# microsoft/GenerativeImage2Text

Measured on AMD Instinct MI355X. Metric: captions/sec whole-node (GIT_BASE 224px bs=64/GPU greedy len=20), higher is better.
Workload: dtype f16; 1 GPU; GIT_BASE 224px bs=64/GPU greedy max_len=20 frames=1; global_batch=64, parallelism=dp1, decode_steps_per_caption=19, seq_len_returned=20, hip_graph=True, contexts_in_flight=4, layernorm_folded=True, library=libgitmi_f16.so, encoder_chains=2, schedule=mixed

## Files before the change

generativeimage2text_amd/csrc/engine.hip:

```cpp
#include "../../include/gitmi.h"
#include "engine_state.h"

#include <algorithm>
#include <cmath>
#include <cstdarg>
#include <cstdio>
#include <cstring>

using namespace gitmi;

#ifdef GITMI_EXPERIMENT
#include "../../include/gitmi_experiment.h"
#define GITMI_EXP_EXPORT extern "C"
#else
#define GITMI_EXP_EXPORT [[maybe_unused]] static
#endif

static thread_local char g_err[1024] = "";
int gitmi::fail(const char* fmt, ...) {
    va_list ap;
    va_start(ap, fmt);
    vsnprintf(g_err, sizeof(g_err), fmt, ap);
    va_end(ap);
    return 1;
// ... 22 lines not shown
static bool gemm_tall_tiles(const gitmi_engine* e, int N) {
    if (!e->pol.shared_device) return false;
    return e->pol.gemm_tall == 1 || (e->pol.gemm_tall == 2 && N >= 2048) || (e->pol.gemm_tall == 3 && N < 2048);
}

static double gemm_flops(int M, int N, int K) { return 2.0 * (double)M * (double)N * (double)K; }
static GemmArgs gemm_args(const void* A, int lda, const void* W, const float* bias, const void* res, int ldr, void* C, int ldc,
                          int M, int N, int K, int act) {
    GemmArgs g{};
    g.A = A; g.W = W; g.bias = bias; g.res = (const float*)res; g.C = C;
    g.M = M; g.N = N; g.K = K; g.lda = lda; g.ldc = ldc; g.ldr = ldr; g.act = act;
    return g;
}
static int gemm_run(gitmi_engine* e, hipStream_t s, GemmArgs g, bool in_f32, bool out_f32, int tag) {
    g.shared = gemm_tall_tiles(e, g.N) ? 1 : 0;
    SpanGuard sp(e, s, tag, gemm_flops(g.M, g.N, g.K));
    HIPCK(launch_gemm(g, in_f32, out_f32, s));
    return 0;
}
static int gemm(gitmi_engine* e, hipStream_t s, const void* A, int lda, const void* W, const float* bias,
                const float* res, int ldr, void* C, int ldc, bool out_f32, int M, int N, int K, int act, int tag) {
    return gemm_run(e, s, gemm_args(A, lda, W, bias, res, ldr, C, ldc, M, N, K, act), e->pol.f32, out_f32, tag);
}
static bool on_p8(const void* A, int lda, const void* W, const void* C, int ldc, int M, int N, int K, bool stream_out) {
    GemmArgs g = gemm_args(A, lda, W, nullptr, nullptr, 0, const_cast<void*>(C), ldc, M, N, K, 0);
    g.out_f16 = stream_out ? 1 : 0;
    return gemm_uses_p8(g, false, false);
}
struct Stream {
    void* x = nullptr; int M = 0, D = 0, tag = 0;
    bool fold = false;
    void* t = nullptr;
    float* xn = nullptr;
    float2* parts[2] = {nullptr, nullptr};
    const float2* part = nullptr; const float* gamma = nullptr; const float* beta = nullptr; float eps = 0.f;
};
static float2* stream_part_out(const Stream& st) { return st.part == st.parts[0] ? st.parts[1] : st.parts[0]; }
static void stream_written(Stream& st, const float2* part, const float* gamma, const float* beta, float eps) {
    st.part = part; st.gamma = gamma; st.beta = beta; st.eps = eps;
}
static int ln_gemm(gitmi_engine* e, hipStream_t s, const Stream& st, const Folded& f, const void* W, const float* bias, void* C,
                   int ldc, int col0, int N, int act) {
    const int D = st.D;
    const size_t woff = (size_t)col0 * D * e->pol.esz;
    C = (char*)C + (size_t)col0 * e->pol.esz;
    if (st.fold) {
        GemmArgs g = gemm_args(st.x, D, (const char*)f.w + woff, f.bias + col0, nullptr, 0, C, ldc, st.M, N, D, act);
        g.ln_part = st.part; g.ln_nparts = D / 256; g.ln_colsum = f.colsum + col0; g.ln_inv_d = 1.0f / (float)D; g.ln_eps = st.eps;
        return gemm_run(e, s, g, false, false, st.tag);
    }
    if (e->pol.stream_f16)
        HIPCK(launch_layernorm_s16(st.x, D, st.gamma, st.beta, st.eps, nullptr, st.t, D, false, st.xn, st.xn ? D : 0, st.M, D, 0, 0, 0, s));
    else
        HIPCK(launch_layernorm((const float*)st.x, D, st.gamma, st.beta, st.eps, nullptr, st.t, D, e->pol.f32, st.xn, st.xn ? D : 0, st.M,
                               D, 0, 0, 0, s));
    return gemm(e, s, st.t, D, (const char*)W + woff, bias + col0, nullptr, 0, C, ldc, e->pol.f32, st.M, N, D, act, st.tag);
}
static int gemm_to_stream(gitmi_engine* e, hipStream_t s, Stream& st, const void* A, int lda, const void* W, const float* bias, int K,
                          bool residual, const float* gamma, const float* beta, float eps) {
    const int D = st.D;
    float2* part = gamma ? stream_part_out(st) : nullptr;
    const void* res = !residual ? nullptr : st.xn && !st.fold ? st.xn : st.x;
    GemmArgs g = gemm_args(A, lda, W, bias, res, residual ? D : 0, st.x, D, st.M, D, K, 0);
    g.out_f16 = e->pol.stream_f16 ? 1 : 0;
    if (st.fold) {
        g.part_out = part;
        if (residual && st.xn) {
            g.res_part = st.part; g.res_nparts = D / 256; g.res_gamma = st.gamma; g.res_beta = st.beta;
            g.res_inv_d = 1.0f / (float)D; g.res_eps = st.eps;
        }
    }
    RCK(gemm_run(e, s, g, e->pol.f32, !e->pol.stream_f16, st.tag));
    stream_written(st, part, gamma, beta, eps);
    return 0;
}
static int attn_full_packed(gitmi_engine* e, const void* qkv, void* out, int width, int heads, int N, int batch, const int* ntok,
                            hipStream_t s) {
    AttnFullArgs a{};
    a.q = qkv;
    a.k = (const char*)qkv + (size_t)width * e->pol.esz;
    a.v = (const char*)qkv + (size_t)2 * width * e->pol.esz;
    a.out = out;
    a.ldq = a.ldk = a.ldv = 3 * width;
    a.ldo = width;
    a.N = N; a.H = heads; a.scale = 0.125f;
    a.ntok = ntok;
    HIPCK(launch_attn_full(a, batch, e->pol.f32, e->pol.attn_impl, s));
    return 0;
}
static int dec_layer_tail(gitmi_engine* e, hipStream_t s, const DecLayerW& L, const void* ctx, float* hf, void* ht, float* y, void* u,
                          int M) {
    const int d = e->cfg.dec_hidden, ffn = e->cfg.dec_ffn;
    RCK(gemm(e, s, ctx, d, L.wo, L.bo, hf, d, y, d, true, M, d, d, 0, TAG_GEMM_OTHER));
    HIPCK(launch_layernorm(y, d, L.lnag, L.lnab, 1e-12f, nullptr, ht, d, e->pol.f32, hf, d, M, d, 0, 0, 0, s));
    RCK(gemm(e, s, ht, d, L.w1, L.b1, nullptr, 0, u, ffn, e->pol.f32, M, ffn, d, 2, TAG_GEMM_OTHER));
    RCK(gemm(e, s, u, ffn, L.w2, L.b2, hf, d, y, d, true, M, d, ffn, 0, TAG_GEMM_OTHER));
    HIPCK(launch_layernorm(y, d, L.lnog, L.lnob, 1e-12f, nullptr, ht, d, e->pol.f32, hf, d, M, d, 0, 0, 0, s));
    return 0;
}

extern "C" int gitmi_abi_version(void) { return GITMI_ABI_VERSION; }
extern "C" int gitmi_operand_dtype(void) {
#ifdef GITMI_OPS_F16
    return GITMI_DTYPE_F16;
#else
    return GITMI_DTYPE_BF16;
#endif
}
extern "C" const char* gitmi_last_error(void) { return g_err; }

extern "C" int gitmi_create(const gitmi_config* cfg, int device, gitmi_engine** out) {
    if (!cfg || !out) return fail("gitmi_create: null argument");
    int ndev = 0;
    if (hipGetDeviceCount(&ndev) != hipSuccess || ndev <= 0)
        return fail("gitmi_create: no HIP device available (this engine has no CPU fallback)");
    if (device < 0 || device >= ndev) return fail("gitmi_create: device %d out of range (%d devices)", device, ndev);
    HIPCK(hipSetDevice(device));
    hipDeviceProp_t prop;
    HIPCK(hipGetDeviceProperties(&prop, device));
    if (strncmp(prop.gcnArchName, "gfx950", 6) != 0)
        return fail("gitmi_create: device %d is %s; this library is built for gfx950 (MI355X) only", device,
                    prop.gcnArchName);
    const gitmi_config& c = *cfg;
    if (c.vit_width % c.vit_heads || c.vit_width / c.vit_heads != 64) return fail("ViT head_dim must be 64");
    if (c.dec_hidden % c.dec_heads || c.dec_hidden / c.dec_heads != 64) return fail("decoder head_dim must be 64");
    if (c.image_size % c.patch) return fail("image_size must be a multiple of patch");
    if (c.max_image_pixels < 0 || c.max_image_tokens < 0) return fail("negative image capacity");
    if (c.vit_width > 1024 || c.dec_hidden > 1024) return fail("hidden sizes above 1024 are not supported");
    if (c.vit_width % 64 || c.dec_hidden % 64 || c.dec_ffn % 64) return fail("hidden sizes must be multiples of 64");
    if (c.max_batch < 1 || c.max_beams < 1 || c.max_beams > 8 || c.max_frames < 1 || c.max_text_len < 2)
        return fail("bad capacity (max_batch>=1, 1<=max_beams<=8, max_frames>=1, max_text_len>=2)");
    if (c.max_text_len > c.max_pos) return fail("max_text_len exceeds max_pos");
    if (c.precision != GITMI_PREC_BF16 && c.precision != GITMI_PREC_F32) return fail("bad precision");

    gitmi_engine* e = new gitmi_engine();
    e->cfg = c;
    e->device = device;
    e->pol.f32 = c.precision == GITMI_PREC_F32;
    e->pol.esz = e->pol.f32 ? 4 : 2;
    e->pol.attn_impl = e->pol.f32 ? 0 : 1;
    init_geometry(e);
    e->pol.stream_f16 = !e->pol.f32;
#ifdef GITMI_OPS_F16
    e->pol.ln_fold = !e->pol.f32 && c.vit_width % 256 == 0 && c.dec_hidden % 256 == 0;
#endif
#ifdef GITMI_EXPERIMENT
    if (const char* env = getenv("GITMI_ATTN_IMPL")) e->pol.attn_impl = e->pol.f32 ? 0 : atoi(env);
    if (const char* env = getenv("GITMI_GRAPH")) e->pol.use_graph = atoi(env) != 0;
    if (const char* env = getenv("GITMI_ATTN_DBG")) e->pol.attn_dbg = atoi(env);
    if (const char* env = getenv("GITMI_ATTN_PW")) e->pol.attn_pw = atoi(env);
    if (const char* env = getenv("GITMI_ATTN_NH")) e->pol.attn_nh = atoi(env);
    if (const char* env = getenv("GITMI_ATTN_STREAM")) e->pol.attn_stream = atoi(env);
    if (const char* env = getenv("GITMI_DECODE_SKIP")) e->pol.decode_skip = atoi(env);
    if (const char* env = getenv("GITMI_GEMM_TALL")) e->pol.gemm_tall = atoi(env);
    if (const char* env = getenv("GITMI_DGEMM_ROWS")) e->pol.dgemm_rows = atoi(env);
    if (const char* env = getenv("GITMI_DGEMM_STRIPS")) e->pol.dgemm_strips = atoi(env);
    if (const char* env = getenv("GITMI_DGEMM_NO_ROW_WALK")) e->pol.dgemm_no_row_walk = atoi(env);
    if (const char* env = getenv("GITMI_DGEMM_DBG")) e->pol.dgemm_dbg = atoi(env);
    if (const char* env = getenv("GITMI_VOCAB_WGS")) e->pol.vocab_wgs = atoi(env);
    if (const char* env = getenv("GITMI_SKINNY")) e->pol.skinny = atoi(env) != 0;
    if (const char* env = getenv("GITMI_STREAM_F16")) e->pol.stream_f16 = !e->pol.f32 && atoi(env) != 0;
    if (const char* env = getenv("GITMI_GEMM_IMPL")) set_gemm_impl(atoi(env));
#endif
    e->pol.ln_fold = e->pol.ln_fold && e->pol.stream_f16;
    e->pol.ln_fold_ready = e->pol.ln_fold;
    *out = e;
    return 0;
}

int CapturedGraph::capture(hipStream_t s, const std::function<int()>& fn) {
    reset();
    HIPCK(hipStreamBeginCapture(s, hipStreamCaptureModeThreadLocal));
    const int rc = fn();
    const hipError_t ce = hipStreamEndCapture(s, &graph);
    if (rc != 0 || ce != hipSuccess) reset();
    RCK(rc);
    HIPCK(ce);
    HIPCK(hipGraphInstantiate(&exec, graph, nullptr, nullptr, 0));
    return 0;
}
static void destroy_graph(gitmi_engine* e) {
    for (CapturedGraph* g : {&e->graph_full, &e->graph_decode, &e->graph_follow}) g->reset();
    e->full_slot.valid = e->follow_slot.valid = false;
}
static void drop_resident(gitmi_engine* e) { e->have_feats = e->have_prefill = false; }
static void set_resident(gitmi_engine* e, int B, int F_eff, int stride = 0) {
    e->cur_B = B; e->cur_F = F_eff; e->cur_Nimg = stride > 0 ? stride : F_eff * e->N;
    e->have_feats = true; e->have_prefill = false;
    e->keyed = e->ragged; e->has_context = false;
    e->res_desc.clear();
}
static void set_context(gitmi_engine* e) { e->keyed = e->has_context = true; }
static const int* key_counts(const gitmi_engine* e) { return e->keyed ? e->rg_ntok : nullptr; }
static void set_prefilled(gitmi_engine* e) { e->have_prefill = true; }
static int settle_residency(gitmi_engine* e, const Request& rq, int rc) {
    if (rc != 0 && rq.frames) drop_resident(e);
    return rc;
}

extern "C" void gitmi_destroy(gitmi_engine* e) {
    if (!e) return;
    hipSetDevice(e->device);
    hipDeviceSynchronize();
    if (e->enc_after) {
        auto& w = e->enc_after->enc_watchers;
        w.erase(std::remove(w.begin(), w.end(), e), w.end());
    }
    for (gitmi_engine* w : e->enc_watchers) w->enc_after = nullptr;
    destroy_graph(e);
    if (e->own_stream) hipStreamDestroy(e->own_stream);
    if (e->fence_in) hipEventDestroy(e->fence_in);
    if (e->fence_out) hipEventDestroy(e->fence_out);
    for (auto ev : e->gev)
        if (ev) hipEventDestroy(ev);
    if (e->enc_done) hipEventDestroy(e->enc_done);
    for (auto ev : e->event_pool) hipEventDestroy(ev);
    for (void* p : e->allocs) hipFree(p);
    for (void* p : e->sc_allocs) hipFree(p);
    hipFree(e->at_out); hipFree(e->at_stats); hipFree(e->ctx_tab); hipFree(e->mem_tab); hipFree(e->feat_tab); hipFree(e->ban_words);
    if (e->ban_stage) hipHostFree(e->ban_stage);
    if (e->ban_staged) hipEventDestroy(e->ban_staged);
    if (e->trie_off) hipFree(e->trie_off);
    if (e->trie_tok) hipFree(e->trie_tok);
    if (e->trie_child) hipFree(e->trie_child);
    delete e;
}

extern "C" int gitmi_set_image_shape(gitmi_engine* e, int H, int W, void* stream) {
    if (!e) return fail("null engine");
    if (!e->finalized) return fail("weights not finalized");
    const gitmi_config& c = e->cfg;
    if (H == 0 && W == 0) {
        if (!e->ragged) {
            e->ragged = true;
            e->H = e->W = e->gh = e->gw = 0;
            e->N = e->Nmax;
            drop_resident(e);
        }
        return 0;
    }
    if (H < c.patch || W < c.patch) return fail("image %dx%d is smaller than one %d-pixel patch", H, W, c.patch);
    const int gh = H / c.patch, gw = W / c.patch;
    if ((size_t)H * W > e->max_pixels)
        return fail("image %dx%d exceeds the max_image_pixels capacity (%zu)", H, W, e->max_pixels);
    if (gh * gw + 1 > e->Nmax)
        return fail("a %dx%d token grid exceeds the max_image_tokens capacity (%d)", gh, gw, e->Nmax);
    if (H == e->H && W == e->W && !e->ragged) return 0;
    e->ragged = false;
    HIPCK(hipSetDevice(e->device));
    if (gh == e->g_nat && gw == e->g_nat) {
        e->pos_cur = e->w.pos;
    } else {
        HIPCK(launch_pos_bicubic(e->w.pos, e->pos_var, e->g_nat, gh, gw, c.vit_width, (hipStream_t)stream));
        e->pos_cur = e->pos_var;
    }
    e->H = H; e->W = W; e->gh = gh; e->gw = gw; e->N = gh * gw + 1;
    drop_resident(e);
    return 0;
}

static Stream vit_stream(gitmi_engine* e, int M) {
    const int D = e->cfg.vit_width;
    const VitLayerW& L = e->w.vit[0];
    Stream st;
    st.x = e->v_x; st.M = M; st.D = D; st.tag = TAG_GEMM_VIT; st.t = e->v_h;
    st.fold = e->pol.ln_fold && on_p8(e->v_x, D, L.qkv_f.w, e->v_qkv, 3 * D, M, 3 * D, D, false) &&
              on_p8(e->v_x, D, L.ffn1_f.w, e->v_u, 4 * D, M, 4 * D, D, false) && on_p8(e->v_ctx, D, L.wo, e->v_x, D, M, D, D, true) &&
              on_p8(e->v_u, 4 * D, L.w2, e->v_x, D, M, D, 4 * D, true);
    if (st.fold) st.parts[0] = st.parts[1] = e->v_part;
    return st;
}
static Stream prefill_stream(gitmi_engine* e, int M) {
    const int d = e->cfg.dec_hidden, ffn = e->cfg.dec_ffn, D = e->cfg.vit_width;
    const DecLayerW& L = e->w.dec[0];
    Stream st;
    st.x = e->p_y; st.M = M; st.D = d; st.tag = TAG_GEMM_OTHER; st.t = e->p_ht; st.xn = e->p_hf;
    st.fold = e->pol.ln_fold && on_p8(e->feats, D, e->w.vp_w, e->p_y, d, M, d, D, true) &&
              on_p8(e->p_y, d, L.qkv_pf.w, e->img_kv[0], 3 * d, M, 3 * d, d, false) &&
              on_p8(e->p_y, d, L.qkv_pf.w, e->img_kv[0], 3 * d, M, 2 * d, d, false) &&
              (e->cfg.dec_layers < 2 || (on_p8(e->p_y, d, L.ffn1_pf.w, e->p_u, ffn, M, ffn, d, false) &&
                                         on_p8(e->p_ctx, d, L.wo, e->p_y, d, M, d, d, true) && on_p8(e->p_u, ffn, L.w2, e->p_y, d, M, d, ffn, true)));
    if (st.fold) { st.parts[0] = e->p_part[0]; st.parts[1] = e->p_part[1]; }
    return st;
}

static int encode_frames_impl(gitmi_engine* e, const float* const* frames, int F, int B, float* feats_out,
                              hipStream_t s, int stride = 0) {
    const gitmi_config& c = e->cfg;
    const int D = c.vit_width, N = e->N;
    const int F_eff = c.num_frames > 0 ? std::min(F, c.num_frames) : F;
    const int Nimg = stride > 0 ? stride : F_eff * N;
    drop_resident(e);
    SpanGuard phase(e, s, TAG_VIT, 0);
    const int BI = F_eff * B;
    const int M = BI * N;
    const int g2 = N - 1;
    const size_t slot = (size_t)3 * e->max_pixels;
    if (e->ragged)
        HIPCK(launch_im2col_ragged(e->frame_stage[0], slot, e->rg_meta, e->patches, e->pol.f32, B, N, c.patch, e->Kp, e->Kp_pad, s));
    else
    for (int fr = 0; fr < F_eff; ++fr)
        HIPCK(launch_im2col(frames[fr], (char*)e->patches + (size_t)fr * B * g2 * e->Kp_pad * e->pol.esz, e->pol.f32, B,
                            e->H, e->W, c.patch, e->Kp, e->Kp_pad, s));
    RCK(gemm(e, s, e->patches, e->Kp_pad, e->w.conv_w, nullptr, nullptr, 0, e->patch_out, D, true, BI * g2, D, e->Kp_pad, 0,
             TAG_GEMM_VIT));
    Stream x = vit_stream(e, M);
    float2* part = stream_part_out(x);
    if (e->ragged)
        HIPCK(launch_vit_assemble_ragged(e->patch_out, e->w.cls, e->w.pos, e->g_nat, e->rg_meta, e->w.lnpre_g, e->w.lnpre_b, 1e-5f, e->v_x,
                                         e->pol.stream_f16, BI, N, c.patch, D, part, s));
    else
    HIPCK(launch_vit_assemble_ln(e->patch_out, e->w.cls, e->pos_cur, e->w.lnpre_g, e->w.lnpre_b, 1e-5f, e->v_x, e->pol.stream_f16, BI, N, D,
                                 part, D / 256, s));
    stream_written(x, part, e->w.vit[0].ln1g, e->w.vit[0].ln1b, 1e-5f);
    for (int l = 0; l < c.vit_layers; ++l) {
        const VitLayerW& L = e->w.vit[l];
        const VitLayerW* Ln = l + 1 < c.vit_layers ? &e->w.vit[l + 1] : nullptr;
        RCK(ln_gemm(e, s, x, L.qkv_f, L.wqkv, L.bqkv, e->v_qkv, 3 * D, 0, 3 * D, 0));
        RCK(attn_full_packed(e, e->v_qkv, e->v_ctx, D, c.vit_heads, N, BI, e->ragged ? e->rg_ntok : nullptr, s));
        RCK(gemm_to_stream(e, s, x, e->v_ctx, D, L.wo, L.bo, D, true, L.ln2g, L.ln2b, 1e-5f));
        RCK(ln_gemm(e, s, x, L.ffn1_f, L.w1, L.b1, e->v_u, 4 * D, 0, 4 * D, 1));
        RCK(gemm_to_stream(e, s, x, e->v_u, 4 * D, L.w2, L.b2, 4 * D, true, Ln ? Ln->ln1g : nullptr, Ln ? Ln->ln1b : nullptr, 1e-5f));
    }
    for (int fr = 0; fr < F_eff; ++fr) {
        const float* te = (c.num_frames > 0 && e->pol.use_temb) ? e->w.temb[fr] : nullptr;
        if (e->pol.stream_f16) {
            const char* xs = (const char*)e->v_x + (size_t)fr * B * N * D * 2;
            HIPCK(launch_layernorm_s16(xs, D, e->w.lnpost_g, e->w.lnpost_b, 1e-5f, te, e->feats, D, false, nullptr, 0, B * N, D, N,
                                       Nimg, fr * N, s));
            if (feats_out)
                HIPCK(launch_layernorm_s16(xs, D, e->w.lnpost_g, e->w.lnpost_b, 1e-5f, te, feats_out, D, true, nullptr, 0, B * N, D,
// ... 153 lines not shown
        v.ban = ban;
        v.part_val = e->part_val; v.part_idx = e->part_idx; v.part_lse = e->part_lse;
        v.logits_out = logits_out; v.ld_logits = ldl;
        {
            SpanGuard sp(e, s, TAG_GEMM_OTHER, gemm_flops(R, c.vocab, d));
            if (!GITMI_SKIPPED(e, 8)) HIPCK(launch_vocab_topm(v, M, s));
        }
        cands->nparts = e->vocab_nparts; cands->slots = vocab_mtop_slots(M);
        if (sampling) RCK(sample_candidates(e, logits_out, ldl, R, cur_len, s, cands, nullptr));
        if (trie) RCK(trie_candidates(e, logits_out, ldl, cur_len, s, cands));
    } else {
        RCK(gemm(e, s, e->d_ht, d, e->w.out_w, e->w.out_b, nullptr, 0, e->logits, e->ldl, true, R, c.vocab, d, 0, TAG_GEMM_OTHER));
        cands->nparts = 1; cands->slots = row_topm_slots(M);
        if (sampling) RCK(sample_candidates(e, e->logits, e->ldl, R, cur_len, s, cands, &ban));
        else if (trie) RCK(trie_candidates(e, e->logits, e->ldl, cur_len, s, cands));
        else if (ids)
            HIPCK(launch_row_topm(e->logits, e->ldl, c.vocab, ids, ld_ids, cur_len, e->plen_dev, beams, suppress_kind,
                                  rep_penalty_of(e), M, R,
                                  e->part_val, e->part_idx, e->part_lse, s, &ban));
        if (logits_out && logits_out != e->logits) HIPCK(launch_copy_f32(e->logits, e->ldl, logits_out, ldl, R, c.vocab, s));
    }
    return 0;
}

static int check_ready(gitmi_engine* e) {
    if (!e) return fail("null engine");
    if (!e->finalized) return fail("weights not finalized (call gitmi_finalize_weights)");
    HIPCK(hipSetDevice(e->device));
    return 0;
}

static int ragged_prepare(gitmi_engine* e, const float* const* frames, int F, int B, hipStream_t s) {
    if (!e->ragged) return 0;
    if (F != 1 || !frames[0]) return fail("ragged input (gitmi_set_image_shape(e, 0, 0)): F must be 1, frames[0] the descriptor buffer");
    drop_resident(e);
    HIPCK(launch_ragged_stage(frames[0], e->frame_stage[0], (size_t)3 * e->max_pixels, e->rg_meta, e->rg_ntok, B, e->cfg.patch,
                              e->max_pixels, e->Nmax, s));
    return 0;
}

static int check_frames(const gitmi_engine* e, const char* who, const float* const* frames, int F, int B) {
    if (!frames || F < 1 || F > e->cfg.max_frames) return fail("%s: F=%d outside [1,%d]", who, F, e->cfg.max_frames);
    if (B < 1 || B > e->cfg.max_batch) return fail("%s: B=%d outside [1,%d]", who, B, e->cfg.max_batch);
    return 0;
}

static int check_resident(const gitmi_engine* e, const char* who, int B) {
    if (!e->have_feats)
        return fail("%s: frames == NULL is a follow-up call, but the engine holds no resident images (encode some with a call "
                    "that takes frames; a change of the image shape or mode, of the temporal embedding or of the LayerNorm "
                    "folding, and a failed call, drop them)", who);
    if (B != e->cur_B) return fail("%s: follow-up call with B=%d, but %d images are resident (B must equal that count)", who, B, e->cur_B);
    return 0;
}

extern "C" int gitmi_encode_frames(gitmi_engine* e, const float* const* frames, int F, int B, float* feats_out,
                                   void* stream) {
    RCK(check_ready(e));
    RCK(check_frames(e, "encode_frames", frames, F, B));
    RCK(ragged_prepare(e, frames, F, B, (hipStream_t)stream));
    return encode_frames_impl(e, frames, F, B, feats_out, (hipStream_t)stream);
}

static EmbedArgs embed_args(gitmi_engine* e, bool on) {
    EmbedArgs em{};
    if (!on) return em;
    em.words = e->w.words_f; em.positions = e->w.positions_f; em.gamma = e->w.emb_lng; em.beta = e->w.emb_lnb; em.eps = 1e-8f;
    em.h_f = e->d_hf; em.h_t = e->d_ht; em.D = e->cfg.dec_hidden; em.vocab = e->cfg.vocab;
    em.frag = (e->pol.skinny && !e->pol.f32) ? 1 : 0;
    return em;
}
static int embed_position(gitmi_engine* e, const int* ids, int ld_ids, int pos, int R, hipStream_t s) {
    const EmbedArgs em = embed_args(e, true);
    HIPCK(launch_embed_ln(ids, ld_ids, pos, em.words, em.positions, em.gamma, em.beta, em.eps, em.h_f, em.h_t, e->pol.f32, R, em.D,
                          em.vocab, em.frag != 0, s));
    return 0;
}

extern "C" int gitmi_prefill(gitmi_engine* e, void* stream) {
    RCK(check_ready(e));
    if (!e->have_feats) return fail("prefill: no encoded frames");
    return prefill_impl(e, (hipStream_t)stream);
}

extern "C" int gitmi_step_logits(gitmi_engine* e, const int64_t* tokens, int R, int t, float* logits_out, void* stream) {
    RCK(check_ready(e));
    if (!e->have_feats) return fail("step_logits: no encoded frames");
    hipStream_t s = (hipStream_t)stream;
    if (!e->have_prefill) RCK(prefill_impl(e, s));
    const int B = e->cur_B;
    if (R < B || R % B) return fail("step_logits: R=%d is not a multiple of the encoded batch %d", R, B);
    const int beams = R / B;
    if (beams > e->cfg.max_beams) return fail("step_logits: %d beams exceed max_beams", beams);
    if (t < 1 || t > e->cfg.max_text_len) return fail("step_logits: t=%d outside [1,%d]", t, e->cfg.max_text_len);
    const gitmi_config& c = e->cfg;
    const int T = c.max_text_len;
    e->img_identity = true;
    HIPCK(launch_load_ids((const long long*)tokens, R, t, e->ss.ids[0], e->ss.kv_src[0], T, s));
    StepCands cands{};
    for (int pos = 0; pos < t; ++pos) {
        SpanGuard step(e, s, TAG_STEP, 0);
        RCK(embed_position(e, e->ss.ids[0], T, pos, R, s));
        RCK(decode_layers_impl(e, e->ss.kv_src[0], T, pos, R, beams, s));
        if (pos == t - 1) RCK(decode_head_impl(e, nullptr, T, t, R, beams, 0, 1, logits_out, c.vocab, s, &cands));
    }
    return 0;
}

static int search_begin_impl(gitmi_engine* e, const Request& rq, int V, hipStream_t s) {
    const gitmi_config& c = e->cfg;
    const gitmi_search* sp = rq.sp;
    const int B = rq.Q, minP = rq.minP, maxP = rq.maxP;
    if (!sp) return fail("search: null config");
    if (sp->kind != GITMI_SEARCH_AUTOREGRESSIVE && sp->kind != GITMI_SEARCH_GENERATOR && sp->kind != GITMI_SEARCH_TRIE)
        return fail("search: bad kind");
    if (sp->kind == GITMI_SEARCH_TRIE) {
        if (sp->beam_size != 1) return fail("search: TrieAutoRegressiveBeamSearch asserts beam_size == 1 (trie_decoder.py:37)");
        if (!e->trie_off) return fail("search: no trie loaded (gitmi_set_trie)");
        if (sp->do_sample) return fail("search: the trie search has no sampling branch");
    }
    if (B < 1 || B > c.max_batch) return fail("search: B=%d outside [1,%d]", B, c.max_batch);
    if (sp->beam_size < 1 || sp->beam_size > c.max_beams) return fail("search: beam_size %d outside [1,%d]", sp->beam_size, c.max_beams);
    if (sp->per_node_beam_size < 1 && sp->kind != GITMI_SEARCH_TRIE) return fail("search: per_node_beam_size must be >= 1");
    if (sp->kind == GITMI_SEARCH_GENERATOR && sp->per_node_beam_size < 2)
        return fail("search: GeneratorWithBeamSearch requires per_node_beam_size > 1 (decoder.py:1078)");
    if (sp->beam_size * sp->per_node_beam_size > 16) return fail("search: beam_size*per_node_beam_size > 16 unsupported");
    if (sp->max_steps > c.max_text_len) return fail("search: max_steps %d exceeds max_text_len %d", sp->max_steps, c.max_text_len);
    if (minP < 1 || maxP > sp->max_steps) return fail("search: prefix lengths [%d,%d] outside [1,max_steps]", minP, maxP);
    if (sp->kind == GITMI_SEARCH_GENERATOR && !(sp->length_penalty > 0)) return fail("search: length_penalty must be > 0");
    if (sp->repetition_penalty != 0 && sp->repetition_penalty != 1.0) {
        if (sp->kind != GITMI_SEARCH_GENERATOR) return fail("search: repetition_penalty belongs to GeneratorWithBeamSearch (decoder.py:1064)");
        if (!(sp->repetition_penalty >= 1.0)) return fail("search: `repetition_penalty` should be >= 1 (decoder.py:1080)");
        if (sp->max_steps > 1024) return fail("search: repetition_penalty supports histories up to 1024 tokens");
    }
    if (sp->num_keep_best < 0 || sp->num_keep_best > SS_NHMAX) return fail("search: num_keep_best %d outside [1,%d]", sp->num_keep_best, SS_NHMAX);
    if (sp->num_keep_best > 1 && sp->kind != GITMI_SEARCH_GENERATOR)
        return fail("search: num_keep_best belongs to GeneratorWithBeamSearch.search (decoder.py:1087)");
    if (sp->do_sample) {
        if (sp->kind != GITMI_SEARCH_GENERATOR) return fail("search: do_sample is implemented for GeneratorWithBeamSearch (decoder.py:1146-1166) only");
        if (sp->temperature < 0) return fail("search: temperature must be > 0");
        if (V > 32768) return fail("search: sampling supports vocabularies up to 32768 tokens");
    }
    SearchState& st = e->ss;
    e->trie_search = sp->kind == GITMI_SEARCH_TRIE;
    st.B = B; st.k = sp->beam_size; st.pn = e->trie_search ? 1 : sp->per_node_beam_size;
    st.T = sp->max_steps;
    st.V = V; st.eos = c.eos; st.kind = e->trie_search ? GITMI_SEARCH_AUTOREGRESSIVE : sp->kind; st.length_penalty = sp->length_penalty;
    st.prefixed = rq.prefixed ? 1 : 0;
    st.nh = keep_best(*sp);
    st.sampled = sp->do_sample ? 1 : 0;
    e->sample = *sp;
    st.start = e->start_dev; st.ld_start = c.max_text_len; st.plen = e->plen_dev;
    e->ss_cur = 0; e->ss_len = minP;
    HIPCK(launch_search_init(st, s));
    if (e->trie_search) HIPCK(launch_fill_i32(e->trie_cursor, 0, B, s));
    return 0;
}

static int search_mtop(const SearchState& st) {
    if (st.sampled) return st.pn;
    return st.kind == GITMI_SEARCH_AUTOREGRESSIVE ? std::max(st.k, st.pn) : st.pn * st.k;
}
static int sample_candidates(gitmi_engine* e, const float* logits, int ldl, int R, int step, hipStream_t s, StepCands* cands,
                             const BanArgs* ban) {
    const gitmi_search& sp = e->sample;
    const float temp = sp.temperature > 0 ? (float)sp.temperature : 1.0f;
    HIPCK(launch_sample_rows(logits, ldl, e->ss.V, R, temp, sp.top_k, (float)sp.top_p, e->ss.pn, sp.seed, step,
                             e->part_val, e->part_idx, e->part_lse, nullptr, e->ss.ids[e->ss_cur], e->ss.T, step,
                             rep_penalty_of(e), row_topm_slots(e->ss.pn), s, ban, e->plen_dev, e->ss.k));
    cands->part_val = e->part_val; cands->part_idx = e->part_idx; cands->part_lse = e->part_lse;
    cands->nparts = 1; cands->slots = row_topm_slots(e->ss.pn);
    return 0;
}

static int trie_candidates(gitmi_engine* e, const float* logits, int ldl, int cur_len, hipStream_t s, StepCands* cands) {
    const SearchState& st = e->ss;
    TrieArgs tr{e->trie_off, e->trie_tok, e->trie_child, e->trie_cursor};
    HIPCK(launch_trie_select(logits, ldl, st.V, st.ids[e->ss_cur], st.T, cur_len, e->plen_dev, st.eos, tr, st.B, e->part_val,
                             e->part_idx, e->part_lse, s));
    cands->part_val = e->part_val; cands->part_idx = e->part_idx; cands->part_lse = e->part_lse;
    cands->nparts = 1; cands->slots = 1;
    return 0;
}

static int search_step_impl(gitmi_engine* e, const StepCands& cands, bool embed, hipStream_t s) {
    const SearchState& st = e->ss;
    const int cur_len = e->ss_len;
    if (cur_len >= st.T) return fail("search_advance: sequence already at max_steps");
    HIPCK(launch_search_step(st, e->ss_cur, cur_len, cands, embed_args(e, embed), e->pol.f32, s));
    e->ss_cur ^= 1;
    e->ss_len = cur_len + 1;
    return 0;
}

static int fill_uniform_sentences(gitmi_engine* e, int B, const long long* prefix_dev, int P, hipStream_t s) {
    HIPCK(launch_fill_start(e->start_dev, e->cfg.max_text_len, prefix_dev, 0, 1, e->cfg.sos, B, P, s));
    HIPCK(launch_fill_i32(e->plen_dev, P, B, s));
    e->img_identity = true;
    return 0;
}

extern "C" int gitmi_set_trie(gitmi_engine* e, int n_nodes, const int32_t* child_off, const int32_t* child_tok,
                              const int32_t* child_node) {
    RCK(check_ready(e));
    HIPCK(hipDeviceSynchronize());
    destroy_graph(e);
    int *n_off = nullptr, *n_tok = nullptr, *n_child = nullptr;
    if (n_nodes > 0) {
        if (!child_off || child_off[0] != 0) return fail("set_trie: child_off must start at 0");
        const int n_edges = child_off[n_nodes];
        for (int n = 0; n < n_nodes; ++n)
            if (child_off[n + 1] < child_off[n]) return fail("set_trie: child_off must be non-decreasing");
        if (n_edges > 0 && (!child_tok || !child_node)) return fail("set_trie: null edge arrays");
        for (int i = 0; i < n_edges; ++i)
            if (child_node[i] < 0 || child_node[i] >= n_nodes) return fail("set_trie: edge %d leads to node %d of %d", i, child_node[i], n_nodes);
        hipError_t err = hipMalloc((void**)&n_off, (size_t)(n_nodes + 1) * sizeof(int));
        if (err == hipSuccess) err = hipMalloc((void**)&n_tok, (size_t)std::max(n_edges, 1) * sizeof(int));
        if (err == hipSuccess) err = hipMalloc((void**)&n_child, (size_t)std::max(n_edges, 1) * sizeof(int));
        if (err == hipSuccess) err = hipMemcpy(n_off, child_off, (size_t)(n_nodes + 1) * sizeof(int), hipMemcpyHostToDevice);
        if (err == hipSuccess && n_edges > 0) err = hipMemcpy(n_tok, child_tok, (size_t)n_edges * sizeof(int), hipMemcpyHostToDevice);
        if (err == hipSuccess && n_edges > 0) err = hipMemcpy(n_child, child_node, (size_t)n_edges * sizeof(int), hipMemcpyHostToDevice);
        if (err != hipSuccess) {
            if (n_off) hipFree(n_off);
            if (n_tok) hipFree(n_tok);
            if (n_child) hipFree(n_child);
            return fail("set_trie: %s (the previous trie is kept)", hipGetErrorString(err));
        }
    }
    if (e->trie_off) { hipFree(e->trie_off); hipFree(e->trie_tok); hipFree(e->trie_child); }
    e->trie_off = n_off; e->trie_tok = n_tok; e->trie_child = n_child;
    return 0;
}

static int search_begin_host(gitmi_engine* e, const char* who, const gitmi_search* sp, int B, const int64_t* start_host, int ld,
                             const int32_t* plen_host, int vocab, void* stream) {
    RCK(check_ready(e));
    if (!start_host) return fail("%s: null start", who);
    if (B < 1 || B > e->cfg.max_batch || ld < 1 || ld > e->cfg.max_text_len) return fail("%s: bad B/P", who);
    if (vocab < 2) return fail("%s: bad vocab", who);
    if (sp && sp->kind == GITMI_SEARCH_SCORE) return fail("%s: GITMI_SEARCH_SCORE is not a search (gitmi_generate_prefixed scores sentences)", who);
    if (sp && sp->kind == GITMI_SEARCH_ATTEND) return fail("%s: GITMI_SEARCH_ATTEND is not a search (gitmi_generate_prefixed returns the attention maps of sentences)", who);
    if (sp && sp->kind == GITMI_SEARCH_CONTEXT) return fail("%s: GITMI_SEARCH_CONTEXT is not a search (gitmi_generate_prefixed puts context tokens into the decoder memory)", who);
    if (sp && sp->kind == GITMI_SEARCH_TREE_SCORE) return fail("%s: GITMI_SEARCH_TREE_SCORE is not a search (gitmi_generate_prefixed scores token trees)", who);
    if (sp && sp->kind == GITMI_SEARCH_KEEP) return fail("%s: GITMI_SEARCH_KEEP is not a search (gitmi_generate_prefixed keeps the memory of resident images)", who);
    if (sp && sp->kind == GITMI_SEARCH_RECALL) return fail("%s: GITMI_SEARCH_RECALL is not a search (gitmi_generate_prefixed recalls kept images)", who);
    if (sp && sp->kind == GITMI_SEARCH_FEATURES) return fail("%s: GITMI_SEARCH_FEATURES is not a search (gitmi_generate_prefixed installs given feature rows)", who);
    if (sp && sp->kind == GITMI_SEARCH_CONSTRAIN) return fail("%s: GITMI_SEARCH_CONSTRAIN is not a search (gitmi_generate_prefixed arms the constraints of the next search call)", who);
    if (e->ban_armed)
        return fail("%s: decoding constraints are armed for %d sentences (GITMI_SEARCH_CONSTRAIN): the seam's caller owns its logits and "
                    "applies its own -- disarm first (a GITMI_SEARCH_CONSTRAIN call with Q == 0)", who, e->ban_armed);
    e->ban_live = false;
    int minP = ld, maxP = ld;
    if (plen_host) {
        maxP = 1;
        for (int b = 0; b < B; ++b) {
            if (plen_host[b] < 1 || plen_host[b] > ld) return fail("%s: prefix length %d of sentence %d outside [1,%d]", who, plen_host[b], b, ld);
            minP = std::min(minP, (int)plen_host[b]); maxP = std::max(maxP, (int)plen_host[b]);
        }
    }
    hipStream_t s = (hipStream_t)stream;
    HIPCK(hipMemcpy2DAsync(e->start_dev, (size_t)e->cfg.max_text_len * sizeof(long long), start_host,
                           (size_t)ld * sizeof(long long), (size_t)ld * sizeof(long long), (size_t)B, hipMemcpyHostToDevice, s));
    if (plen_host) HIPCK(hipMemcpyAsync(e->plen_dev, plen_host, (size_t)B * sizeof(int), hipMemcpyHostToDevice, s));
    HIPCK(hipStreamSynchronize(s));
    if (!plen_host) HIPCK(launch_fill_i32(e->plen_dev, ld, B, s));
    e->img_identity = true;
    Request rq{};
    rq.Q = B; rq.minP = minP; rq.maxP = maxP; rq.prefixed = plen_host != nullptr; rq.sp = sp;
    return search_begin_impl(e, rq, vocab, s);
}

extern "C" int gitmi_search_begin(gitmi_engine* e, const gitmi_search* sp, int B, const int64_t* start_host, int P,
                                  int vocab, void* stream) {
    return search_begin_host(e, "search_begin", sp, B, start_host, P, nullptr, vocab, stream);
}

extern "C" int gitmi_search_rows(gitmi_engine* e, int64_t* tokens_out, int* R, int* t, void* stream) {
    RCK(check_ready(e));
    const SearchState& st = e->ss;
    if (R) *R = st.B * st.k;
    if (t) *t = e->ss_len;
    if (tokens_out) HIPCK(launch_search_rows(st, e->ss_cur, e->ss_len, (long long*)tokens_out, (hipStream_t)stream));
    return 0;
}

extern "C" int gitmi_search_advance(gitmi_engine* e, const float* logits, void* stream) {
    RCK(check_ready(e));
    if (!logits) return fail("search_advance: null logits");
    const SearchState& st = e->ss;
    hipStream_t s = (hipStream_t)stream;
    const int M = search_mtop(st), R = st.B * st.k;
    StepCands cands{e->part_val, e->part_idx, e->part_lse, 1, row_topm_slots(M)};
    if (st.sampled) RCK(sample_candidates(e, logits, st.V, R, e->ss_len, s, &cands, nullptr));
    else if (e->trie_search) RCK(trie_candidates(e, logits, st.V, e->ss_len, s, &cands));
    else
        HIPCK(launch_row_topm(logits, st.V, st.V, st.ids[e->ss_cur], st.T, e->ss_len, e->plen_dev, st.k,
                              st.kind == GITMI_SEARCH_AUTOREGRESSIVE ? 1 : 0, rep_penalty_of(e), M, R, e->part_val,
                              e->part_idx, e->part_lse, s));
    return search_step_impl(e, cands, false, s);
}

extern "C" int gitmi_search_done_count(gitmi_engine* e, int* done_out, void* stream) {
    RCK(check_ready(e));
    if (!done_out) return fail("search_done_count: null argument");
    int h = 0;
    HIPCK(hipMemcpyAsync(&h, e->ss.info, sizeof(int), hipMemcpyDeviceToHost, (hipStream_t)stream));
    HIPCK(hipStreamSynchronize((hipStream_t)stream));
    *done_out = h;
    return 0;
}

extern "C" int gitmi_search_finish(gitmi_engine* e, int64_t* tokens_out, float* logprob_out, int32_t* info_out,
                                   void* stream) {
    RCK(check_ready(e));
    const SearchState& st = e->ss;
    HIPCK(launch_search_finish(st, e->ss_cur, e->ss_len, (long long*)tokens_out, logprob_out, info_out, nullptr,
                               (hipStream_t)stream));
    return 0;
}

GITMI_EXP_EXPORT int gitmi_debug_search_begin_prefixed(gitmi_engine* e, const gitmi_search* sp, int B, const int64_t* start_host,
                                                       int ld, const int32_t* plen_host, int vocab, void* stream) {
    if (!plen_host) return fail("debug_search_begin_prefixed: null prefix lengths");
    return search_begin_host(e, "debug_search_begin_prefixed", sp, B, start_host, ld, plen_host, vocab, stream);
}
GITMI_EXP_EXPORT int gitmi_debug_search_advance_lists(gitmi_engine* e, const float* part_val, const int* part_idx,
                                                      const float* part_lse, int nparts, int slots, int embed, void* stream) {
    RCK(check_ready(e));
    if (!part_val || !part_idx || !part_lse) return fail("debug_search_advance_lists: null argument");
    const SearchState& st = e->ss;
    if (st.B < 1 || st.T < 1) return fail("debug_search_advance_lists: no search has begun");
    if (st.sampled || e->trie_search) return fail("debug_search_advance_lists: the sampling and trie searches select from whole logit rows");
    if (nparts < 1 || nparts > 256) return fail("debug_search_advance_lists: nparts=%d outside [1,256]", nparts);
    if (slots != 1 && slots != 2 && slots != 4 && slots != 8 && slots != 16)
        return fail("debug_search_advance_lists: slots=%d is not one of 1, 2, 4, 8, 16", slots);
    if (slots < search_mtop(st)) return fail("debug_search_advance_lists: slots=%d, but the step reads %d candidates per row", slots, search_mtop(st));
    const StepCands cands{part_val, part_idx, (const float2*)part_lse, nparts, slots};
    return search_step_impl(e, cands, embed != 0, (hipStream_t)stream);
}
GITMI_EXP_EXPORT int gitmi_debug_read_hidden(gitmi_engine* e, int R, float* hf_out, void* ht_out, int* ht_frag, int* ht_dtype,
                                             void* stream) {
    RCK(check_ready(e));
    const gitmi_config& c = e->cfg;
    if (R < 1 || R > c.max_batch * c.max_beams) return fail("debug_read_hidden: R=%d outside the capacity", R);
    if (!hf_out || !ht_out || !ht_frag || !ht_dtype) return fail("debug_read_hidden: null argument");
    hipStream_t s = (hipStream_t)stream;
    const size_t D = (size_t)c.dec_hidden, Rp = (size_t)(R + 15) / 16 * 16;
    HIPCK(hipMemcpyAsync(hf_out, e->d_hf, (size_t)R * D * sizeof(float), hipMemcpyDefault, s));
    HIPCK(hipMemcpyAsync(ht_out, e->d_ht, Rp * D * e->pol.esz, hipMemcpyDefault, s));
    HIPCK(hipStreamSynchronize(s));
    *ht_frag = (e->pol.skinny && !e->pol.f32) ? 1 : 0;
    *ht_dtype = e->pol.f32 ? GITMI_DTYPE_F32 : gitmi_operand_dtype();
    return 0;
}

static int generate_encode(gitmi_engine* e, const Request& rq, hipStream_t s) {
    RCK(encode_frames_impl(e, rq.frames, rq.F, rq.B, nullptr, s));
    return prefill_impl(e, s);
}
static int images_ready(gitmi_engine* e, const Request& rq, hipStream_t s) {
    if (rq.frames) return generate_encode(e, rq, s);
    return e->have_prefill ? 0 : prefill_impl(e, s);
}

static int generate_decode(gitmi_engine* e, const Request& rq, hipStream_t s, bool allow_poll) {
    const gitmi_config& c = e->cfg;
    const gitmi_search* sp = rq.sp;
    RCK(search_begin_impl(e, rq, c.vocab, s));
    const int Q = rq.Q, minP = rq.minP, maxP = rq.maxP, T = sp->max_steps, k = sp->beam_size, R = Q * k;
    const SearchState& st = e->ss;
    const int M = search_mtop(st);
    const int suppress = sp->kind != GITMI_SEARCH_GENERATOR ? 1 : 0;
    {
        SpanGuard phase(e, s, TAG_DECODE, 0);
        RCK(embed_position(e, st.ids[0], T, 0, R, s));
        e->ss_len = 1;
        StepCands cands{e->part_val, e->part_idx, e->part_lse, 1, 1};
        while (e->ss_len < T) {
            const int cur_len = e->ss_len;
            SpanGuard step(e, s, TAG_STEP, 0);
            RCK(decode_layers_impl(e, st.kv_src[e->ss_cur], T, cur_len - 1, R, k, s));
            if (cur_len >= minP)
                RCK(decode_head_impl(e, st.ids[e->ss_cur], T, cur_len, R, k, suppress, M, nullptr, 0, s, &cands));
            RCK(search_step_impl(e, cands, true, s));
            if (allow_poll && e->ss_len > maxP && (e->ss_len - maxP) % 8 == 0 && e->ss_len < T) {
                int h[4];
                HIPCK(hipMemcpyAsync(h, st.info, sizeof(h), hipMemcpyDeviceToHost, s));
                HIPCK(hipStreamSynchronize(s));
                if (h[0] >= Q) break;
            }
        }
    }
    HIPCK(launch_search_finish(st, e->ss_cur, e->ss_len, rq.tokens, rq.logprob, rq.info, rq.sent, s));
    if (e->ragged)
        HIPCK(launch_ragged_report(e->rg_meta, e->img_identity ? nullptr : e->img_of_dev, Q, keep_best(*sp), rq.logprob, rq.info,
                                   nullptr, s));
    const double kv = (double)Q * c.dec_layers * 2.0 * ((double)e->cur_Nimg + k * 0.5 * (minP + T)) * c.dec_hidden * e->pol.esz;
    e->last_decode_step_bytes = e->w.dec_weight_bytes + kv;
    return 0;
}

static int generate_body(gitmi_engine* e, const Request& rq, hipStream_t s, bool allow_poll) {
    SpanGuard total(e, s, 99, 0);
    RCK(images_ready(e, rq, s));
    return generate_decode(e, rq, s, allow_poll);
}

static GraphKey graph_key_of(const gitmi_engine* e, const Request& rq, int F_eff) {
    const gitmi_search& sp = *rq.sp;
    const bool resident = rq.frames == nullptr;
    return {rq.B, rq.Q, F_eff, rq.minP, sp.kind, sp.beam_size, sp.per_node_beam_size, sp.max_steps, e->H, e->W,
            rq.prefixed ? 1 : 0, e->img_identity ? 1 : 0, e->pol.use_temb ? 1 : 0, resident ? 1 : 0,
            resident ? e->cur_Nimg : 0, resident && e->keyed ? 1 : 0, sp.length_penalty,
            sp.do_sample, sp.top_k, keep_best(sp), sp.top_p, sp.temperature, sp.repetition_penalty, sp.seed, e->ban_live ? 1 : 0};
}

static int replay(gitmi_engine* e, const Request& rq, hipStream_t x, const CapturedGraph* enc, const CapturedGraph* dec) {
    const bool timed = e->profile_mode == 2;
    if (timed) {
        for (auto& ev : e->gev)
            if (!ev) HIPCK(hipEventCreate(&ev));
        HIPCK(hipEventRecord(e->gev[enc ? 0 : 1], x));
    } else if (enc && e->enc_after && e->enc_after->enc_done) {
        HIPCK(hipStreamWaitEvent(x, e->enc_after->enc_done, 0));
    }
    if (enc) {
        HIPCK(enc->launch(x));
        if (timed) HIPCK(hipEventRecord(e->gev[1], x));
        else if (e->enc_done && !e->enc_watchers.empty()) HIPCK(hipEventRecord(e->enc_done, x));
    }
    if (dec) HIPCK(dec->launch(x));
    if (!timed) return 0;
    HIPCK(hipEventRecord(e->gev[2], x));
    HIPCK(hipStreamSynchronize(x));
    float a = 0, b = 0;
    if (enc) HIPCK(hipEventElapsedTime(&a, e->gev[0], e->gev[1]));
    HIPCK(hipEventElapsedTime(&b, e->gev[1], e->gev[2]));
    e->split_encode_ms += a; e->split_decode_ms += b; e->split_calls += 1; e->split_steps += rq.sp->max_steps - 1;
    return 0;
}

static int generate_graphed(gitmi_engine* e, const Request& rq, hipStream_t s) {
    const gitmi_config& c = e->cfg;
    const bool resident = rq.frames == nullptr;
    hipStream_t x = s ? s : e->own_stream;
    if (x != s) {
        HIPCK(hipEventRecord(e->fence_in, s));
        HIPCK(hipStreamWaitEvent(x, e->fence_in, 0));
    }
    const size_t frame_bytes = (size_t)rq.B * 3 * e->H * e->W * sizeof(float);
    const int F_eff = resident ? e->cur_F : c.num_frames > 0 ? std::min(rq.F, c.num_frames) : rq.F;
    if (!e->ragged && !resident)
    for (int f = 0; f < F_eff; ++f)
        HIPCK(hipMemcpyAsync(e->frame_stage[f], rq.frames[f], frame_bytes, hipMemcpyDeviceToDevice, x));
    Request own = rq;
    if (!resident) { own.frames = e->frame_stage.data(); own.F = F_eff; }
    own.tokens = e->out_tokens; own.logprob = e->out_lp; own.info = e->out_info; own.sent = e->out_sent;
    const GraphKey key = graph_key_of(e, rq, F_eff);
    const CapturedGraph *enc = nullptr, *dec = nullptr;
    if (resident) {
        RCK(images_ready(e, rq, x));
        if (!e->follow_slot.valid || !(key == e->follow_slot.key)) {
            e->follow_slot.valid = false;
            RCK(e->graph_follow.capture(x, [&] { return generate_decode(e, own, x, false); }));
            e->follow_slot = {key, true};
        }
        dec = &e->graph_follow;
    } else {
        const bool split = e->profile_mode == 2 || e->enc_after != nullptr || !e->enc_watchers.empty();
        if (!e->full_slot.valid || !(key == e->full_slot.key) || split != e->graph_is_split) {
            e->full_slot.valid = false;
            e->graph_decode.reset();
            if (!split) {
                RCK(e->graph_full.capture(x, [&] { return generate_body(e, own, x, false); }));
            } else {
                RCK(e->graph_full.capture(x, [&] { return generate_encode(e, own, x); }));
                RCK(e->graph_decode.capture(x, [&] { return generate_decode(e, own, x, false); }));
            }
            e->full_slot = {key, true}; e->graph_is_split = split;
        } else {
            set_resident(e, rq.B, F_eff);
            set_prefilled(e);
        }
        enc = &e->graph_full;
        if (split) dec = &e->graph_decode;
    }
    RCK(replay(e, rq, x, enc, dec));
    const size_t nout = (size_t)rq.Q * (size_t)keep_best(*rq.sp);
    HIPCK(hipMemcpyAsync(rq.tokens, e->out_tokens, nout * rq.sp->max_steps * sizeof(long long), hipMemcpyDefault, x));
    HIPCK(hipMemcpyAsync(rq.logprob, e->out_lp, nout * sizeof(float), hipMemcpyDefault, x));
    HIPCK(hipMemcpyAsync(rq.info, e->out_info, 4 * sizeof(int), hipMemcpyDefault, x));
    if (rq.sent != e->out_sent) HIPCK(hipMemcpyAsync(rq.sent, e->out_sent, (size_t)rq.Q * 2 * sizeof(int), hipMemcpyDefault, x));
    if (x != s) {
        HIPCK(hipEventRecord(e->fence_out, x));
        HIPCK(hipStreamWaitEvent(s, e->fence_out, 0));
    }
    return 0;
}

static int generate_run(gitmi_engine* e, const Request& rq, hipStream_t s, bool constrained) {
    const bool long_budget = rq.sp->max_steps - rq.minP > 32;
    const bool graph = e->pol.use_graph && !e->profiling && !long_budget;
    if (constrained) e->ban_armed = 0;
    e->ban_live = constrained;
    const int rc = settle_residency(e, rq, graph ? generate_graphed(e, rq, s) : generate_body(e, rq, s, long_budget && !e->profiling));
    e->ban_live = false;
    return rc;
}

static int constrain_check(const gitmi_engine* e, const char* who, const gitmi_search* sp, int Q, bool* constrained);

extern "C" int gitmi_generate(gitmi_engine* e, const float* const* frames, int F, int B, const int64_t* prefix, int P,
                              const gitmi_search* sp, int64_t* tokens_out, float* logprob_out, int32_t* info_out,
                              void* stream) {
    RCK(check_ready(e));
    const gitmi_config& c = e->cfg;
    if (sp && sp->kind == GITMI_SEARCH_SCORE) return fail("generate: GITMI_SEARCH_SCORE scores given sentences: call gitmi_generate_prefixed");
    if (sp && sp->kind == GITMI_SEARCH_ATTEND) return fail("generate: GITMI_SEARCH_ATTEND maps given sentences: call gitmi_generate_prefixed");
    if (sp && sp->kind == GITMI_SEARCH_CONTEXT) return fail("generate: GITMI_SEARCH_CONTEXT takes context segments: call gitmi_generate_prefixed");
    if (sp && sp->kind == GITMI_SEARCH_TREE_SCORE) return fail("generate: GITMI_SEARCH_TREE_SCORE scores given token trees: call gitmi_generate_prefixed");
    if (sp && sp->kind == GITMI_SEARCH_KEEP) return fail("generate: GITMI_SEARCH_KEEP keeps the memory of resident images: call gitmi_generate_prefixed");
    if (sp && sp->kind == GITMI_SEARCH_RECALL) return fail("generate: GITMI_SEARCH_RECALL recalls kept images: call gitmi_generate_prefixed");
    if (sp && sp->kind == GITMI_SEARCH_FEATURES) return fail("generate: GITMI_SEARCH_FEATURES installs given feature rows: call gitmi_generate_prefixed");
    if (sp && sp->kind == GITMI_SEARCH_CONSTRAIN) return fail("generate: GITMI_SEARCH_CONSTRAIN arms decoding constraints: call gitmi_generate_prefixed");
    if (!frames) RCK(check_resident(e, "generate", B));
    if (!sp || !tokens_out || !logprob_out || !info_out) return fail("generate: null argument");
    if (frames) RCK(check_frames(e, "generate", frames, F, B));
    if (!prefix) P = 1;
    if (P < 1 || P > c.max_text_len) return fail("generate: prefix length %d outside [1,%d]", P, c.max_text_len);
    if (sp->max_steps < P || sp->max_steps > c.max_text_len) return fail("generate: max_steps %d outside [P,%d]", sp->max_steps, c.max_text_len);
    bool constrained = false;
    RCK(constrain_check(e, "generate", sp, B, &constrained));
    hipStream_t s = (hipStream_t)stream;
    if (frames) RCK(ragged_prepare(e, frames, F, B, s));
    RCK(fill_uniform_sentences(e, B, (const long long*)prefix, P, s));
    const Request rq{frames, F, B, B, P, P, false, sp, (long long*)tokens_out, logprob_out, info_out, e->out_sent};
    return generate_run(e, rq, s, constrained);
}

static int tree_max_depth(const gitmi_config& c) { return std::min((int)c.max_text_len, (int)c.max_pos); }
constexpr int TREE_MAX_ROWS = 65535 * 64;
static void score_free(gitmi_engine* e) {
    for (void* p : e->sc_allocs) hipFree(p);
    e->sc_allocs.clear();
    e->sc_rows = 0;
    e->tr_out_n = 0;
}
static int score_alloc(gitmi_engine* e, size_t rows_needed, size_t tree_out = 0) {
    size_t rows = (size_t)round_up((int)rows_needed, 128);
    if (e->sc_rows >= rows && e->tr_out_n >= tree_out) return 0;
    rows = std::max(rows, e->sc_rows);
    tree_out = std::max(tree_out, e->tr_out_n);
    score_free(e);
    const gitmi_config& c = e->cfg;
    const int d = c.dec_hidden;
    const size_t Qmax = (size_t)c.max_batch * c.max_beams;
    const size_t esz = e->pol.esz;
    auto alloc = [&](auto** p, size_t bytes) -> bool {
        void* q = nullptr;
        if (hipMalloc(&q, bytes) != hipSuccess) return false;
        e->sc_allocs.push_back(q);
        *reinterpret_cast<void**>(p) = q;
        return true;
    };
    const bool ok = alloc(&e->sc_hf, rows * d * 4) && alloc(&e->sc_y, rows * d * 4) && alloc(&e->sc_ht, rows * d * esz) &&
                    alloc(&e->sc_qkv, rows * 3 * d * esz) && alloc(&e->sc_ctx, rows * d * esz) &&
                    alloc(&e->sc_u, rows * c.dec_ffn * esz) &&
                    alloc(&e->sc_part, rows * (size_t)(e->pol.f32 ? 1 : score_head_tiles(c.vocab)) * sizeof(float4)) &&
                    alloc(&e->sc_zt, rows * 4) && alloc(&e->sc_tgt, rows * 4) && alloc(&e->sc_lens, Qmax * 4) &&
                    alloc(&e->sc_img, Qmax * 4) && alloc(&e->sc_bad, Qmax * 4) && alloc(&e->sc_info, 16) &&
                    alloc(&e->sc_out, Qmax * (size_t)c.max_text_len * sizeof(float2)) &&
                    (!tree_out || (alloc(&e->tr_nodes, rows * 4 * sizeof(int)) && alloc(&e->tr_out, tree_out * sizeof(float2))));
    if (!ok) {
        score_free(e);
        (void)hipGetLastError();
        return fail("score: out of device memory for the workspaces of %zu text rows", rows);
    }
    e->sc_rows = rows;
    e->tr_out_n = tree_out;
    return 0;
}

static int attend_alloc(gitmi_engine* e, size_t floats, size_t stat_rows) {
    if (e->at_floats < floats) {
        hipFree(e->at_out);
        e->at_out = nullptr; e->at_floats = 0;
        if (hipMalloc(&e->at_out, floats * sizeof(float)) != hipSuccess) {
            (void)hipGetLastError();
            return fail("attend: out of device memory for the %zu floats of the maps", floats);
        }
        e->at_floats = floats;
    }
    if (e->at_stat_rows < stat_rows) {
        hipFree(e->at_stats);
        e->at_stats = nullptr; e->at_stat_rows = 0;
        if (hipMalloc(&e->at_stats, stat_rows * sizeof(float2)) != hipSuccess) {
            (void)hipGetLastError();
            return fail("attend: out of device memory for the softmax statistics of %zu rows", stat_rows);
        }
        e->at_stat_rows = stat_rows;
    }
    return 0;
}
static int call_Nimg(const gitmi_engine* e, const float* const* frames, int F) {
    if (!frames) return e->cur_Nimg;
    return (e->cfg.num_frames > 0 ? std::min(F, (int)e->cfg.num_frames) : F) * e->N;
}

static int score_head_impl(gitmi_engine* e, int M, hipStream_t s, int* ntiles, const TreeNodes* tree = nullptr, int Lp = 0) {
    const gitmi_config& c = e->cfg;
    const int d = c.dec_hidden, V = c.vocab;
    *ntiles = 1;
    if (e->pol.f32) {
        const int chunk = round_up(c.max_batch * c.max_beams, 64);
        for (int r0 = 0; r0 < M; r0 += chunk) {
            const int rows = std::min(chunk, M - r0);
            RCK(gemm(e, s, (const float*)e->sc_ht + (size_t)r0 * d, d, e->w.out_w, e->w.out_b, nullptr, 0, e->logits, e->ldl, true, rows,
                     V, d, 0, TAG_GEMM_OTHER));
            HIPCK(launch_score_rowstats(e->logits, e->ldl, V, e->sc_tgt, r0, rows, e->sc_part, e->sc_zt, s));
            if (tree) HIPCK(launch_tree_gather_logits(e->logits, e->ldl, r0, rows, *tree, Lp, M, e->sc_zt, s));
        }
    } else {
        SpanGuard sp(e, s, TAG_GEMM_OTHER, gemm_flops(M, V, d));
        *ntiles = score_head_tiles(V);
        HIPCK(launch_score_head(e->sc_ht, d, e->w.out_w, e->w.out_b, e->sc_tgt, M, V, d, e->sc_part, e->sc_zt, s));
        if (tree) HIPCK(launch_tree_gather_dot(e->sc_ht, d, e->w.out_w, e->w.out_b, *tree, Lp, M, d, e->sc_zt, s));
    }
    return 0;
}
static int text_pass_impl(gitmi_engine* e, const Request& rq, const long long* tokens, int ld, hipStream_t s) {
    const gitmi_config& c = e->cfg;
    const int d = c.dec_hidden, V = c.vocab, Q = rq.Q, L = c.dec_layers;
    const bool attend = rq.sp->kind == GITMI_SEARCH_ATTEND, tree = rq.sp->kind == GITMI_SEARCH_TREE_SCORE;
    RCK(images_ready(e, rq, s));
    const int Lp = round_up(rq.maxP, 16), M = Q * Lp;
    const int Nk = e->cur_Nimg, Kc = Nk + ld;
    void* const out = attend ? (void*)e->at_out : tree ? (void*)e->tr_out : (void*)e->sc_out;
    const size_t out_bytes = attend ? (size_t)Q * ld * L * Kc * sizeof(float) : (size_t)Q * ld * sizeof(float2);
    auto zero_outputs = [&]() -> int {
        HIPCK(hipMemsetAsync(out, 0, out_bytes, s));
        HIPCK(hipMemsetAsync(e->sc_bad, 0, (size_t)Q * sizeof(int), s));
        return 0;
    };
    SpanGuard phase(e, s, TAG_DECODE, 0);
    if (attend || tree) RCK(zero_outputs());
    const size_t R = tree ? e->sc_rows : 0;
    const TreeNodes nodes = tree ? TreeNodes{e->tr_nodes, e->tr_nodes + R, e->tr_nodes + 2 * R, e->tr_nodes + 3 * R} : TreeNodes{};
    if (tree) HIPCK(launch_tree_structure(tokens, ld, Q, Lp, e->sc_lens, V, tree_max_depth(c), nodes, e->sc_bad, s));
    HIPCK(launch_score_embed_ln(tokens, ld, Q, Lp, e->w.words_f, e->w.positions_f, e->w.emb_lng, e->w.emb_lnb, 1e-8f, e->sc_hf, e->sc_ht,
                                e->pol.f32, d, V, c.max_pos, s, tree ? &nodes : nullptr));
    const int* ntok = key_counts(e);
    for (int l = 0; l < L; ++l) {
        const DecLayerW& W = e->w.dec[l];
        RCK(gemm(e, s, e->sc_ht, d, W.wqkv, W.bqkv, nullptr, 0, e->sc_qkv, 3 * d, e->pol.f32, M, 3 * d, d, 0, TAG_GEMM_OTHER));
        HIPCK(launch_score_attn(e->sc_qkv, e->img_kv[l], e->sc_img, e->sc_ctx, Q, c.dec_heads, d, Nk, Lp, 0.125f, e->pol.f32, s, ntok,
                                attend ? e->at_stats : nullptr, tree ? nodes.end : nullptr));
        if (attend)
            HIPCK(launch_score_attn_map(e->sc_qkv, e->img_kv[l], e->sc_img, ntok, e->at_stats, e->sc_lens, e->at_out + (size_t)l * Kc,
                                        (size_t)ld * L * Kc, (size_t)L * Kc, ld, Q, c.dec_heads, Nk, Lp, 0.125f, e->pol.f32, e->sc_bad, s));
        if (!attend || l + 1 < L) RCK(dec_layer_tail(e, s, W, e->sc_ctx, e->sc_hf, e->sc_ht, e->sc_y, e->sc_u, M));
    }
    if (int ntiles = 1; tree) {
        HIPCK(hipMemsetAsync(e->sc_tgt, 0xff, (size_t)M * sizeof(int), s));
        RCK(score_head_impl(e, M, s, &ntiles, &nodes, Lp));
        HIPCK(launch_tree_combine(e->sc_part, ntiles, e->sc_zt, nodes, M, Lp, ld, V, e->tr_out, e->sc_bad, s));
    } else if (!attend) {
        HIPCK(launch_score_targets(tokens, ld, Lp, e->sc_lens, V, M, e->sc_tgt, s));
        RCK(score_head_impl(e, M, s, &ntiles));
        RCK(zero_outputs());
        HIPCK(launch_score_combine(e->sc_part, ntiles, e->sc_zt, e->sc_tgt, M, Lp, ld, V, e->sc_out, e->sc_bad, s));
    }
    if (e->ragged) HIPCK(launch_ragged_report(e->rg_meta, e->sc_img, Q, 0, nullptr, nullptr, e->sc_bad, s));
    HIPCK(launch_score_info(e->sc_bad, Q, ld, e->sc_info, s, attend ? Kc : 0, attend ? L : 0));
    HIPCK(hipMemcpyAsync(rq.logprob, out, out_bytes, hipMemcpyDefault, s));
    HIPCK(hipMemcpyAsync(rq.info, e->sc_info, 4 * sizeof(int), hipMemcpyDefault, s));
    return 0;
}

struct SentenceSpan { int minP, maxP; bool ident; };
static int read_sentences(gitmi_engine* e, const char* who, const int32_t* plen, const int32_t* image_of, int ld, int B, int Q,
                          int Qmax, const char* cap, SentenceSpan* span) {
    if (Q < 1 || Q > Qmax) return fail("%s: Q=%d sentences outside [1,%d] (%s)", who, Q, Qmax, cap);
    if (!image_of && Q != B) return fail("%s: without image_of, Q must equal B", who);
    *span = {1 << 30, 0, true};
    e->plen_host.assign(plen, plen + Q);
    e->img_of_host.resize(Q);
    for (int q = 0; q < Q; ++q) {
        const int p = plen[q];
        if (p < 1 || p > ld) return fail("%s: length %d of sentence %d outside [1,%d]", who, p, q, ld);
// ... 603 lines not shown
```

generativeimage2text_amd/csrc/engine_state.h:

```cpp
#pragma once
#include "../../include/gitmi.h"
#include "abi_common.h"
#include "launchers.h"

#include <hip/hip_runtime.h>

#include <functional>
#include <map>
#include <string>
#include <tuple>
#include <vector>

static inline int round_up(int x, int m) { return (x + m - 1) / m * m; }
static inline int keep_best(const gitmi_search& sp) { return sp.num_keep_best > 1 ? sp.num_keep_best : 1; }

struct HostTensor {
    std::vector<float> data;
    std::vector<int64_t> shape;
    float amax = 0.f;
    size_t numel() const { size_t n = 1; for (auto s : shape) n *= (size_t)s; return n; }
};

struct Folded { void* w = nullptr; float* bias = nullptr; float* colsum = nullptr; };

struct VitLayerW {
    void *wqkv = nullptr, *wo = nullptr, *w1 = nullptr, *w2 = nullptr;
    float *bqkv = nullptr, *bo = nullptr, *b1 = nullptr, *b2 = nullptr;
    float *ln1g = nullptr, *ln1b = nullptr, *ln2g = nullptr, *ln2b = nullptr;
    Folded qkv_f;
    Folded ffn1_f;
};
struct DecLayerW {
    void *wqkv = nullptr, *wo = nullptr, *w1 = nullptr, *w2 = nullptr;
    float *bqkv = nullptr, *bo = nullptr, *b1 = nullptr, *b2 = nullptr;
    float *lnag = nullptr, *lnab = nullptr, *lnog = nullptr, *lnob = nullptr;
    Folded qkv_f;
    Folded ffn1_f;
    void *wo_p = nullptr, *w2_p = nullptr;
    Folded qkv_pf, ffn1_pf;
};

struct TimedSpan { hipEvent_t a, b; int tag; double flops; };
enum { TAG_VIT = 0, TAG_PREFILL = 1, TAG_DECODE = 2, TAG_GEMM_VIT = 10, TAG_GEMM_OTHER = 11, TAG_STEP = 20 };

struct GraphKey {
    int B, Q, F, P, kind, k, pn, T, H, W, prefixed, ident, temb, resident, Nimg, keyed; double lp;
    int smp, top_k, nh; double top_p, temp, rp; unsigned long long seed;
    int constrained;
    auto fields() const {
        return std::tie(B, Q, F, P, kind, k, pn, T, H, W, prefixed, ident, temb, resident, Nimg, keyed, lp, smp, top_k, nh, top_p, temp,
                        rp, seed, constrained);
    }
    bool operator==(const GraphKey& o) const { return fields() == o.fields(); }
};
struct GraphSlot { GraphKey key{}; bool valid = false; };

struct CapturedGraph {
    hipGraph_t graph = nullptr;
    hipGraphExec_t exec = nullptr;
    void reset() {
        if (exec) hipGraphExecDestroy(exec);
        if (graph) hipGraphDestroy(graph);
        exec = nullptr, graph = nullptr;
    }
    int capture(hipStream_t s, const std::function<int()>& fn);
    hipError_t launch(hipStream_t s) const { return hipGraphLaunch(exec, s); }
};

struct Request {
    const float* const* frames;
    int F, B, Q, minP, maxP;
    bool prefixed;
    const gitmi_search* sp;
    long long* tokens; float* logprob; int32_t* info;
    int32_t* sent;
};

struct ModelWeights {
    void* conv_w = nullptr;
    float *cls = nullptr, *pos = nullptr, *lnpre_g = nullptr, *lnpre_b = nullptr, *lnpost_g = nullptr, *lnpost_b = nullptr;
    std::vector<VitLayerW> vit;
    std::vector<float*> temb;
    void* vp_w = nullptr;
    float *vp_b = nullptr, *vp_lng = nullptr, *vp_lnb = nullptr;
    float *words_f = nullptr, *positions_f = nullptr, *emb_lng = nullptr, *emb_lnb = nullptr;
    std::vector<DecLayerW> dec;
    void* out_w = nullptr;
    float* out_b = nullptr;
    Folded out_f;
    double dec_weight_bytes = 0;
};

struct Policy {
    bool f32 = false;
    size_t esz = 2;
    int attn_impl = 1;
    bool stream_f16 = false;
    bool ln_fold = false;
    bool ln_fold_ready = false;
    bool skinny = true;
    bool use_graph = true;
    bool use_temb = true;
    bool shared_device = false;
    int attn_dbg = 0, dgemm_dbg = 0;
    int attn_pw = 0;
    int attn_nh = 0;
    int attn_stream = -1;
    int dgemm_no_row_walk = -1;
    int dgemm_strips = -1;
    int vocab_wgs = -1;
    int gemm_tall = 1;
    int dgemm_rows = 0;
    int decode_skip = 0;
};

struct gitmi_engine {
    gitmi_config cfg{};
    ModelWeights w;
    Policy pol;
    int device = 0;
    bool finalized = false;
    gitmi_engine* parent = nullptr;

    std::map<std::string, HostTensor> host_w;
    std::vector<void*> allocs;

    int N = 0, gh = 0, gw = 0, H = 0, W = 0, Kp = 0, Kp_pad = 0;
    int N_nat = 0, g_nat = 0, Nmax = 0;
    size_t max_pixels = 0;
    float* pos_var = nullptr;
    const float* pos_cur = nullptr;
    bool ragged = false;
    int4* rg_meta = nullptr;
    int* rg_ntok = nullptr;
    bool keyed = false;
    bool has_context = false;
    int* ctx_tab = nullptr;
    size_t ctx_tab_ints = 0;
    gitmi::MemoryEntry* mem_tab = nullptr;
    size_t mem_tab_n = 0;
    std::vector<int4> res_desc;
    gitmi::FeaturePiece* feat_tab = nullptr;
    unsigned int* ban_words = nullptr;
    int* ban_stage = nullptr;
    hipEvent_t ban_staged = nullptr;
    int ban_armed = 0;
    bool ban_live = false;

    void *patches = nullptr, *v_h = nullptr, *v_qkv = nullptr, *v_ctx = nullptr, *v_u = nullptr;
    float *patch_out = nullptr, *v_x = nullptr;
    void* feats = nullptr;
    float *p_y = nullptr, *p_hf = nullptr;
    void *p_ht = nullptr, *p_ctx = nullptr, *p_u = nullptr;
    std::vector<void*> img_kv;
    std::vector<void*> img_kh, img_vh;
    float *d_y = nullptr, *d_hf = nullptr, *logits = nullptr;
    void *d_ht = nullptr, *d_qkv = nullptr, *d_ctx = nullptr, *d_u = nullptr;
    std::vector<void*> txt_k, txt_v;
    int ldl = 0;
    float *xa_f = nullptr, *xo_f = nullptr;
    void *xa_b = nullptr, *xo_b = nullptr;
    float2 *stats_a = nullptr, *stats_o = nullptr;
    float* part_val = nullptr; int* part_idx = nullptr; float2* part_lse = nullptr;
    int vocab_cols = 128, vocab_nparts = 1;
    gitmi::SearchState ss{};
    int ss_cur = 0, ss_len = 0;
    long long* start_dev = nullptr;
    int *plen_dev = nullptr, *img_of_dev = nullptr;
    bool img_identity = true;
    int *trie_off = nullptr, *trie_tok = nullptr, *trie_child = nullptr, *trie_cursor = nullptr;
    bool trie_search = false;
    gitmi_search sample{};
    std::vector<int> plen_host, img_of_host;

    int cur_B = 0, cur_F = 0, cur_Nimg = 0;
    bool have_feats = false, have_prefill = false;

    int profile_mode = 0;
    bool profiling = false;
    float2 *v_part = nullptr, *p_part[2] = {nullptr, nullptr};
    hipEvent_t gev[3] = {nullptr, nullptr, nullptr};
    gitmi_engine* enc_after = nullptr;
    std::vector<gitmi_engine*> enc_watchers;
    hipEvent_t enc_done = nullptr;
    double split_encode_ms = 0, split_decode_ms = 0;
    int split_calls = 0, split_steps = 0;
    std::vector<TimedSpan> spans;
    std::vector<hipEvent_t> event_pool;
    size_t event_next = 0;
    double last_decode_step_bytes = 0;

    CapturedGraph graph_full, graph_decode, graph_follow;
    GraphSlot full_slot, follow_slot;
    bool graph_is_split = false;
    std::vector<float*> frame_stage;
    long long* out_tokens = nullptr;
    float* out_lp = nullptr;
    int* out_info = nullptr;
    int* out_sent = nullptr;
    hipStream_t own_stream = nullptr;
    hipEvent_t fence_in = nullptr, fence_out = nullptr;

    size_t sc_rows = 0;
    std::vector<void*> sc_allocs;
    float *sc_hf = nullptr, *sc_y = nullptr, *sc_zt = nullptr;
    void *sc_ht = nullptr, *sc_qkv = nullptr, *sc_ctx = nullptr, *sc_u = nullptr;
    float4* sc_part = nullptr;
    int *sc_tgt = nullptr, *sc_lens = nullptr, *sc_img = nullptr, *sc_bad = nullptr, *sc_info = nullptr;
    float2* sc_out = nullptr;
    size_t tr_out_n = 0;
    int* tr_nodes = nullptr;
    float2* tr_out = nullptr;
    size_t at_floats = 0, at_stat_rows = 0;
    float* at_out = nullptr;
    float2* at_stats = nullptr;
};

namespace gitmi {
void init_geometry(gitmi_engine* e);
}
```

generativeimage2text_amd/csrc/engine_weights.hip:

```cpp
#include "engine_state.h"

#include <algorithm>
#include <cmath>
#include <cstring>

using namespace gitmi;

static int dev_alloc(gitmi_engine* e, void** p, size_t bytes) {
    if (bytes == 0) bytes = 16;
    HIPCK(hipMalloc(p, bytes));
    e->allocs.push_back(*p);
    return 0;
}
template <typename T> static int dev_alloc_t(gitmi_engine* e, T** p, size_t count) {
    return dev_alloc(e, reinterpret_cast<void**>(p), count * sizeof(T));
}

static float half_to_float(uint16_t h) {
    const uint32_t sign = (uint32_t)(h & 0x8000) << 16;
    uint32_t exp = (h >> 10) & 0x1f, man = h & 0x3ff, out;
    if (exp == 0) {
        if (man == 0) out = sign;
        else {
            exp = 127 - 15 + 1;
// ... 33 lines not shown
    float amax = 0.f;
    for (size_t i = 0; i < n; ++i) {
        if (!std::isfinite(t.data[i])) return fail("gitmi_load_tensor: '%s' holds a non-finite value at element %zu", key, i);
        amax = std::max(amax, std::fabs(t.data[i]));
    }
    t.amax = amax;
    e->host_w[k] = std::move(t);
    return 0;
}

static int get_w(gitmi_engine* e, const std::string& key, std::initializer_list<int64_t> shape, const HostTensor** out) {
    auto it = e->host_w.find(key);
    if (it == e->host_w.end()) return fail("missing weight '%s'", key.c_str());
    size_t want = 1;
    for (auto s : shape) want *= (size_t)s;
    if (it->second.numel() != want) return fail("weight '%s' has %zu elements, expected %zu", key.c_str(), it->second.numel(), want);
    *out = &it->second;
    return 0;
}
static int up_f32(gitmi_engine* e, const std::string& key, std::initializer_list<int64_t> shape, float** dst) {
    const HostTensor* t;
    RCK(get_w(e, key, shape, &t));
    RCK(dev_alloc_t(e, dst, t->numel()));
    HIPCK(hipMemcpy(*dst, t->data.data(), t->numel() * 4, hipMemcpyHostToDevice));
    return 0;
}
static int operand_range_check(gitmi_engine* e, const char* what, float amax) {
#ifdef GITMI_OPS_F16
    if (!e->pol.f32 && amax > 65504.f)
        return fail("'%s': max |w| = %g is outside the fp16 operand range (65504): load this checkpoint with precision "
                    "\"bf16\" or \"f32\"", what, (double)amax);
#endif
    (void)e; (void)what; (void)amax;
    return 0;
}
static int up_mat(gitmi_engine* e, const std::string& key, int64_t rows, int K, int Kpad, void** dst) {
    const HostTensor* t;
    RCK(get_w(e, key, {rows, (int64_t)K}, &t));
    RCK(operand_range_check(e, key.c_str(), t->amax));
    RCK(dev_alloc(e, dst, (size_t)rows * Kpad * e->pol.esz));
    float* tmp = nullptr;
    HIPCK(hipMalloc((void**)&tmp, t->numel() * 4));
    hipError_t err = hipMemcpy(tmp, t->data.data(), t->numel() * 4, hipMemcpyHostToDevice);
    if (err == hipSuccess) err = launch_convert_pad(tmp, *dst, e->pol.f32, (size_t)rows, K, Kpad, 0);
    if (err == hipSuccess) err = hipDeviceSynchronize();
    hipFree(tmp);
    HIPCK(err);
    return 0;
}

void gitmi::init_geometry(gitmi_engine* e) {
    const gitmi_config& c = e->cfg;
    e->g_nat = e->gh = e->gw = c.image_size / c.patch;
    e->N_nat = e->N = e->g_nat * e->g_nat + 1;
    e->H = e->W = c.image_size;
    e->Nmax = std::max(e->N_nat, c.max_image_tokens);
    e->max_pixels = std::max((size_t)c.image_size * c.image_size, (size_t)c.max_image_pixels);
    e->Kp = 3 * c.patch * c.patch;
    e->Kp_pad = round_up(e->Kp, 64);
    e->pos_cur = e->w.pos;
}

static int alloc_workspaces(gitmi_engine* e) {
    const gitmi_config& c = e->cfg;
    const size_t esz = e->pol.esz;
    const int D = c.vit_width, d = c.dec_hidden;
    const size_t Mv = (size_t)c.max_batch * c.max_frames * e->Nmax;
    const size_t Mp = (size_t)c.max_batch * c.max_frames * e->Nmax;
    const size_t R = (size_t)round_up(c.max_batch * c.max_beams, 64);
    const int T = c.max_text_len;
    RCK(dev_alloc(e, &e->patches, (size_t)c.max_batch * c.max_frames * (e->Nmax - 1) * e->Kp_pad * esz));
    RCK(dev_alloc_t(e, &e->patch_out, (size_t)c.max_batch * c.max_frames * (e->Nmax - 1) * D));
    RCK(dev_alloc_t(e, &e->pos_var, (size_t)e->Nmax * D));
    RCK(dev_alloc_t(e, &e->v_x, Mv * D));
    RCK(dev_alloc(e, &e->v_h, Mv * D * esz));
    RCK(dev_alloc(e, &e->v_qkv, Mv * 3 * D * esz));
    RCK(dev_alloc(e, &e->v_ctx, Mv * D * esz));
    RCK(dev_alloc(e, &e->v_u, Mv * 4 * D * esz));
    RCK(dev_alloc(e, &e->feats, Mp * D * esz));
    if (e->pol.ln_fold_ready) {
        RCK(dev_alloc_t(e, &e->v_part, Mv * 4));
        RCK(dev_alloc_t(e, &e->p_part[0], Mp * 4));
        RCK(dev_alloc_t(e, &e->p_part[1], Mp * 4));
        HIPCK(hipMemset(e->v_part, 0, Mv * 4 * sizeof(float2)));
        HIPCK(hipMemset(e->p_part[0], 0, Mp * 4 * sizeof(float2)));
        HIPCK(hipMemset(e->p_part[1], 0, Mp * 4 * sizeof(float2)));
    }
    RCK(dev_alloc_t(e, &e->p_y, Mp * d));
    RCK(dev_alloc_t(e, &e->p_hf, Mp * d));
    RCK(dev_alloc(e, &e->p_ht, Mp * d * esz));
    RCK(dev_alloc(e, &e->p_ctx, Mp * d * esz));
    RCK(dev_alloc(e, &e->p_u, Mp * c.dec_ffn * esz));
    e->img_kv.resize(c.dec_layers);
    e->img_kh.resize(c.dec_layers);
    e->img_vh.resize(c.dec_layers);
    e->txt_k.resize(c.dec_layers);
    e->txt_v.resize(c.dec_layers);
    for (int l = 0; l < c.dec_layers; ++l) {
        RCK(dev_alloc(e, &e->img_kv[l], Mp * 3 * d * esz));
        const size_t Mkv = (size_t)c.max_batch * round_up(c.max_frames * e->Nmax, 32);
        RCK(dev_alloc(e, &e->img_kh[l], Mkv * d * esz));
        RCK(dev_alloc(e, &e->img_vh[l], Mkv * d * esz));
        RCK(dev_alloc(e, &e->txt_k[l], R * T * d * esz));
        RCK(dev_alloc(e, &e->txt_v[l], R * T * d * esz));
    }
    RCK(dev_alloc_t(e, &e->d_y, R * d));
    RCK(dev_alloc_t(e, &e->d_hf, R * d));
    RCK(dev_alloc(e, &e->d_ht, R * d * esz));
    RCK(dev_alloc(e, &e->d_qkv, R * 3 * d * esz));
    RCK(dev_alloc(e, &e->d_ctx, R * d * esz));
    RCK(dev_alloc(e, &e->d_u, R * c.dec_ffn * esz));
    RCK(dev_alloc_t(e, &e->xa_f, R * d));
    RCK(dev_alloc_t(e, &e->xo_f, R * d));
    RCK(dev_alloc(e, &e->xa_b, R * d * 2));
    RCK(dev_alloc(e, &e->xo_b, R * d * 2));
    RCK(dev_alloc_t(e, &e->stats_a, R * (size_t)(d / 16)));
    RCK(dev_alloc_t(e, &e->stats_o, R * (size_t)(d / 16)));
    e->ldl = round_up(c.vocab, 8);
    RCK(dev_alloc_t(e, &e->logits, R * e->ldl));
    e->vocab_cols = 128;
    e->vocab_nparts = (e->pol.skinny && !e->pol.f32) ? vocab_parts(c.vocab, e->vocab_cols) : 1;
    RCK(dev_alloc_t(e, &e->part_val, R * (size_t)e->vocab_nparts * 16));
    RCK(dev_alloc_t(e, &e->part_idx, R * (size_t)e->vocab_nparts * 16));
    RCK(dev_alloc_t(e, &e->part_lse, R * (size_t)e->vocab_nparts));
    SearchState& s = e->ss;
    for (int i = 0; i < 2; ++i) {
        RCK(dev_alloc_t(e, &s.ids[i], R * T));
        RCK(dev_alloc_t(e, &s.kv_src[i], R * T));
        RCK(dev_alloc_t(e, &s.score[i], R));
    }
    RCK(dev_alloc_t(e, &s.done, (size_t)c.max_batch));
    RCK(dev_alloc_t(e, &s.hyp_n, (size_t)c.max_batch));
    RCK(dev_alloc_t(e, &s.hyp_cnt, (size_t)c.max_batch));
    RCK(dev_alloc_t(e, &s.hyp_worst, (size_t)c.max_batch));
    RCK(dev_alloc_t(e, &s.hyp_score, (size_t)c.max_batch * SS_NHMAX));
    RCK(dev_alloc_t(e, &s.hyp_len, (size_t)c.max_batch * SS_NHMAX));
    RCK(dev_alloc_t(e, &s.hyp_seq, (size_t)c.max_batch * SS_NHMAX));
    RCK(dev_alloc_t(e, &s.hyp_tok, (size_t)c.max_batch * SS_NHMAX * T));
    RCK(dev_alloc_t(e, &s.stop, (size_t)c.max_batch));
    RCK(dev_alloc_t(e, &s.early, (size_t)c.max_batch));
    RCK(dev_alloc_t(e, &s.info, 4));
    RCK(dev_alloc_t(e, &s.len_norm, (size_t)T + 1));
    RCK(dev_alloc_t(e, &e->start_dev, (size_t)c.max_batch * T));
    RCK(dev_alloc_t(e, &e->plen_dev, (size_t)c.max_batch));
    RCK(dev_alloc_t(e, &e->img_of_dev, (size_t)c.max_batch));
    RCK(dev_alloc_t(e, &e->trie_cursor, (size_t)c.max_batch));
    RCK(dev_alloc_t(e, &e->out_tokens, (size_t)c.max_batch * SS_NHMAX * T));
    RCK(dev_alloc_t(e, &e->out_lp, (size_t)c.max_batch * SS_NHMAX));
    RCK(dev_alloc_t(e, &e->out_info, 4));
    RCK(dev_alloc_t(e, &e->out_sent, (size_t)c.max_batch * 2));
    HIPCK(hipStreamCreateWithFlags(&e->own_stream, hipStreamNonBlocking));
    HIPCK(hipEventCreateWithFlags(&e->fence_in, hipEventDisableTiming));
    HIPCK(hipEventCreateWithFlags(&e->fence_out, hipEventDisableTiming));
    e->frame_stage.resize(c.max_frames);
    for (int f = 0; f < c.max_frames; ++f)
        RCK(dev_alloc_t(e, &e->frame_stage[f], (size_t)c.max_batch * 3 * e->max_pixels));
    RCK(dev_alloc_t(e, &e->rg_meta, (size_t)c.max_batch));
    RCK(dev_alloc_t(e, &e->rg_ntok, (size_t)c.max_batch));
    return 0;
}

#ifdef GITMI_OPS_F16
static inline float bf16_round(float f) { return (float)(_Float16)f; }
#else
static inline float bf16_round(float f) {
    uint32_t u;
    memcpy(&u, &f, 4);
    if ((u & 0x7f800000u) == 0x7f800000u) return f;
    u += 0x7fffu + ((u >> 16) & 1u);
    u &= 0xffff0000u;
    memcpy(&f, &u, 4);
    return f;
}
#endif
static int fold_layernorm(gitmi_engine* e, const std::vector<float>& W, const std::vector<float>& bias,
                          const std::vector<float>& gamma, const std::vector<float>& beta, int64_t rows, int K, bool frag,
                          Folded* out) {
    std::vector<float> wf((size_t)rows * K), b2((size_t)rows), c2((size_t)rows);
    float amax = 0.f;
    for (int64_t n = 0; n < rows; ++n) {
        double sum = 0.0, cst = bias[n];
        const float* w = &W[(size_t)n * K];
        float* o = &wf[(size_t)n * K];
        for (int k = 0; k < K; ++k) {
            amax = std::max(amax, std::fabs(w[k] * gamma[k]));
            o[k] = bf16_round(w[k] * gamma[k]);
            sum += (double)o[k];
            cst += (double)beta[k] * (double)w[k];
        }
        c2[n] = (float)sum;
        b2[n] = (float)cst;
    }
    RCK(operand_range_check(e, "a matrix with the LayerNorm gain in front of it folded in (W . gamma)", amax));
    const int64_t rows_pad = (rows + 127) / 128 * 128;
    RCK(dev_alloc(e, &out->w, (size_t)rows_pad * K * 2));
    float* tmp = nullptr;
    void* tmp_b = nullptr;
    HIPCK(hipMalloc((void**)&tmp, wf.size() * 4));
    hipError_t err = hipSuccess;
    if (frag) err = hipMalloc(&tmp_b, wf.size() * 2);
    if (err == hipSuccess) err = hipMemcpy(tmp, wf.data(), wf.size() * 4, hipMemcpyHostToDevice);
    if (err == hipSuccess) err = launch_convert_pad(tmp, frag ? tmp_b : out->w, false, (size_t)rows, K, K, 0);
    if (err == hipSuccess && frag) err = launch_frag_pack(tmp_b, out->w, (int)rows, (int)rows_pad, K, 0);
    if (err == hipSuccess) err = hipDeviceSynchronize();
    hipFree(tmp);
    if (tmp_b) hipFree(tmp_b);
    HIPCK(err);
    b2.resize((size_t)rows_pad, 0.f);
    c2.resize((size_t)rows_pad, 0.f);
    RCK(dev_alloc_t(e, &out->bias, (size_t)rows_pad));
    RCK(dev_alloc_t(e, &out->colsum, (size_t)rows_pad));
    HIPCK(hipMemcpy(out->bias, b2.data(), (size_t)rows_pad * 4, hipMemcpyHostToDevice));
    HIPCK(hipMemcpy(out->colsum, c2.data(), (size_t)rows_pad * 4, hipMemcpyHostToDevice));
    return 0;
}
static int pack_frag(gitmi_engine* e, const void* src, int64_t rows, int K, void** dst) {
    const int64_t rows_pad = (rows + 15) / 16 * 16;
    RCK(dev_alloc(e, dst, (size_t)rows_pad * K * 2));
    HIPCK(launch_frag_pack(src, *dst, (int)rows, (int)rows_pad, K, 0));
    HIPCK(hipDeviceSynchronize());
    return 0;
}
static int fold_named(gitmi_engine* e, const std::string& ln, const std::string& dense, int64_t rows, int K, bool frag, Folded* out) {
    const HostTensor *g, *b, *w, *bi;
    RCK(get_w(e, ln + "weight", {K}, &g));
    RCK(get_w(e, ln + "bias", {K}, &b));
    RCK(get_w(e, dense + "weight", {rows, K}, &w));
    RCK(get_w(e, dense + "bias", {rows}, &bi));
    return fold_layernorm(e, w->data, bi->data, g->data, b->data, rows, K, frag, out);
}
static std::string vit_layer_key(int i) { return "image_encoder.transformer.resblocks." + std::to_string(i) + "."; }
static std::string dec_layer_key(int i) { return "textual.transformer.encoder.layer." + std::to_string(i) + "."; }
static int concat_qkv(gitmi_engine* e, const std::string& pre, int d) {
    HostTensor w, b;
    w.shape = {3 * d, d};
    b.shape = {3 * d};
    for (const char* name : {"query", "key", "value"}) {
        const HostTensor *tw, *tb;
        RCK(get_w(e, pre + "attention.self." + name + ".weight", {d, d}, &tw));
        RCK(operand_range_check(e, (pre + "attention.self." + name + ".weight").c_str(), tw->amax));
        RCK(get_w(e, pre + "attention.self." + name + ".bias", {d}, &tb));
        w.data.insert(w.data.end(), tw->data.begin(), tw->data.end());
        b.data.insert(b.data.end(), tb->data.begin(), tb->data.end());
        w.amax = std::max(w.amax, tw->amax);
    }
    e->host_w[pre + "attention.self.qkv.weight"] = std::move(w);
    e->host_w[pre + "attention.self.qkv.bias"] = std::move(b);
    return 0;
}

static int fold_decoder(gitmi_engine* e) {
    const gitmi_config& c = e->cfg;
    const int d = c.dec_hidden, f = c.dec_ffn;
    for (int i = 0; i < c.dec_layers; ++i) {
        const std::string pre = dec_layer_key(i);
        DecLayerW& L = e->w.dec[i];
        if (i > 0) {
            RCK(fold_named(e, dec_layer_key(i - 1) + "output.LayerNorm.", pre + "attention.self.qkv.", 3 * d, d, true, &L.qkv_f));
        } else {
            RCK(pack_frag(e, L.wqkv, 3 * d, d, &L.qkv_f.w));
            L.qkv_f.bias = L.bqkv;
        }
        RCK(pack_frag(e, L.wo, d, d, &L.wo_p));
        RCK(pack_frag(e, L.w2, d, f, &L.w2_p));
        RCK(fold_named(e, pre + "attention.output.LayerNorm.", pre + "intermediate.dense.", f, d, true, &L.ffn1_f));
    }
    return fold_named(e, dec_layer_key(c.dec_layers - 1) + "output.LayerNorm.", "textual.output.", c.vocab, d, true, &e->w.out_f);
}

static int fold_encoder_prefill(gitmi_engine* e) {
    const gitmi_config& c = e->cfg;
    const int D = c.vit_width, d = c.dec_hidden, f = c.dec_ffn;
    for (int i = 0; i < c.vit_layers; ++i) {
        const std::string pre = vit_layer_key(i);
        RCK(fold_named(e, pre + "ln_1.", pre + "attn.in_proj_", 3 * D, D, false, &e->w.vit[i].qkv_f));
        RCK(fold_named(e, pre + "ln_2.", pre + "mlp.c_fc.", 4 * D, D, false, &e->w.vit[i].ffn1_f));
    }
    for (int i = 0; i < c.dec_layers; ++i) {
        const std::string pre = dec_layer_key(i);
        DecLayerW& L = e->w.dec[i];
        const std::string ln = i == 0 ? "textual.visual_projection.1." : dec_layer_key(i - 1) + "output.LayerNorm.";
        RCK(fold_named(e, ln, pre + "attention.self.qkv.", 3 * d, d, false, &L.qkv_pf));
        if (i + 1 == c.dec_layers) break;
        RCK(fold_named(e, pre + "attention.output.LayerNorm.", pre + "intermediate.dense.", f, d, false, &L.ffn1_pf));
    }
    return 0;
}

extern "C" int gitmi_finalize_weights(gitmi_engine* e) {
    if (!e) return fail("null engine");
    if (e->finalized) return 0;
    HIPCK(hipSetDevice(e->device));
    const gitmi_config& c = e->cfg;
    const int D = c.vit_width, F4 = 4 * D, d = c.dec_hidden, f = c.dec_ffn, V = c.vocab;
    const int64_t p = c.patch;
    {
        const HostTensor* t;
        RCK(get_w(e, "image_encoder.conv1.weight", {D, 3, p, p}, &t));
        e->host_w["image_encoder.conv1.weight"].shape = {D, (int64_t)e->Kp};
        RCK(up_mat(e, "image_encoder.conv1.weight", D, e->Kp, e->Kp_pad, &e->w.conv_w));
    }
    RCK(up_f32(e, "image_encoder.class_embedding", {D}, &e->w.cls));
    RCK(up_f32(e, "image_encoder.positional_embedding", {e->N_nat, D}, &e->w.pos));
    e->pos_cur = e->w.pos;
    RCK(up_f32(e, "image_encoder.ln_pre.weight", {D}, &e->w.lnpre_g));
    RCK(up_f32(e, "image_encoder.ln_pre.bias", {D}, &e->w.lnpre_b));
    RCK(up_f32(e, "image_encoder.ln_post.weight", {D}, &e->w.lnpost_g));
    RCK(up_f32(e, "image_encoder.ln_post.bias", {D}, &e->w.lnpost_b));
    e->w.vit.resize(c.vit_layers);
// ... 81 lines not shown
```

generativeimage2text_amd/csrc/gitmi_common.h:

```cpp
#pragma once
#include <hip/hip_runtime.h>
#include <stdint.h>

typedef unsigned short bf16_t;
typedef __attribute__((ext_vector_type(8))) __bf16 bf16x8_t;
typedef __attribute__((ext_vector_type(4))) float f32x4_t;
typedef __attribute__((ext_vector_type(4))) unsigned int u32x4_t;

#define GITMI_WAVE 64

typedef _Float16 f16_t;
typedef __attribute__((ext_vector_type(2))) _Float16 f16x2_t;
typedef __attribute__((ext_vector_type(8))) _Float16 f16x8_t;
typedef __attribute__((ext_vector_type(2))) __bf16 bf16x2_t;
#ifdef GITMI_OPS_F16
#define GITMI_OPERAND_NAME "f16"
__device__ __forceinline__ float bf2f(bf16_t h) { return (float)__builtin_bit_cast(_Float16, h); }
__device__ __forceinline__ bf16_t f2bf(float f) {
    const _Float16 b = (_Float16)f;
    return __builtin_bit_cast(bf16_t, b);
}
__device__ __forceinline__ uint32_t pack2bf(float lo, float hi) {
    const f16x2_t v = {(_Float16)lo, (_Float16)hi};
    return __builtin_bit_cast(uint32_t, v);
}
__device__ __forceinline__ void unpack2op(uint32_t u, float& lo, float& hi) {
    const f16x2_t v = __builtin_bit_cast(f16x2_t, u);
    lo = (float)v[0];
    hi = (float)v[1];
}
__device__ __forceinline__ f32x4_t mfma16(bf16x8_t a, bf16x8_t b, f32x4_t c) {
    return __builtin_amdgcn_mfma_f32_16x16x32_f16(__builtin_bit_cast(f16x8_t, a), __builtin_bit_cast(f16x8_t, b), c, 0, 0, 0);
}
#else
#define GITMI_OPERAND_NAME "bf16"
__device__ __forceinline__ float bf2f(bf16_t h) { return __uint_as_float(((uint32_t)h) << 16); }
__device__ __forceinline__ bf16_t f2bf(float f) {
    const __bf16 b = (__bf16)f;
    return __builtin_bit_cast(bf16_t, b);
}
__device__ __forceinline__ uint32_t pack2bf(float lo, float hi) {
    const bf16x2_t v = {(__bf16)lo, (__bf16)hi};
    return __builtin_bit_cast(uint32_t, v);
}
__device__ __forceinline__ void unpack2op(uint32_t u, float& lo, float& hi) {
    lo = __uint_as_float(u << 16);
    hi = __uint_as_float(u & 0xffff0000u);
}
__device__ __forceinline__ f32x4_t mfma16(bf16x8_t a, bf16x8_t b, f32x4_t c) {
    return __builtin_amdgcn_mfma_f32_16x16x32_bf16(a, b, c, 0, 0, 0);
}
#endif

__device__ __forceinline__ uint32_t pack2h(float lo, float hi) {
    const f16x2_t v = {(_Float16)lo, (_Float16)hi};
    return __builtin_bit_cast(uint32_t, v);
}
__device__ __forceinline__ void unpack2h(uint32_t u, float& lo, float& hi) {
    const f16x2_t v = __builtin_bit_cast(f16x2_t, u);
    lo = (float)v[0];
    hi = (float)v[1];
}
__device__ __forceinline__ f32x4_t ld4s(const float* p) { return *reinterpret_cast<const f32x4_t*>(p); }
__device__ __forceinline__ f32x4_t ld4s(const f16_t* p) {
    const uint2 u = *reinterpret_cast<const uint2*>(p);
    float a, b, c, d;
    unpack2h(u.x, a, b);
    unpack2h(u.y, c, d);
    return f32x4_t{a, b, c, d};
}
__device__ __forceinline__ void st4s(float* p, f32x4_t v) { *reinterpret_cast<f32x4_t*>(p) = v; }
__device__ __forceinline__ void st4s(f16_t* p, f32x4_t v) {
    uint2 u;
    u.x = pack2h(v[0], v[1]);
    u.y = pack2h(v[2], v[3]);
    *reinterpret_cast<uint2*>(p) = u;
}

template <typename T> __device__ __forceinline__ float ld(const T* p);
template <> __device__ __forceinline__ float ld<float>(const float* p) { return *p; }
template <> __device__ __forceinline__ float ld<bf16_t>(const bf16_t* p) { return bf2f(*p); }
template <typename T> __device__ __forceinline__ void st(T* p, float v);
template <> __device__ __forceinline__ void st<float>(float* p, float v) { *p = v; }
template <> __device__ __forceinline__ void st<bf16_t>(bf16_t* p, float v) { *p = f2bf(v); }
template <> __device__ __forceinline__ float ld<f16_t>(const f16_t* p) { return (float)*p; }
template <> __device__ __forceinline__ void st<f16_t>(f16_t* p, float v) { *p = (f16_t)v; }

__device__ __forceinline__ void ld8(const bf16_t* p, float (&v)[8]) {
    u32x4_t r = *reinterpret_cast<const u32x4_t*>(p);
#pragma unroll
    for (int i = 0; i < 4; ++i) unpack2op(r[i], v[2 * i], v[2 * i + 1]);
}
__device__ __forceinline__ void ld8(const float* p, float (&v)[8]) {
    f32x4_t a = *reinterpret_cast<const f32x4_t*>(p);
    f32x4_t b = *reinterpret_cast<const f32x4_t*>(p + 4);
#pragma unroll
    for (int i = 0; i < 4; ++i) { v[i] = a[i]; v[4 + i] = b[i]; }
}
__device__ __forceinline__ void st8(bf16_t* p, const float (&v)[8]) {
    u32x4_t r;
#pragma unroll
    for (int i = 0; i < 4; ++i) r[i] = pack2bf(v[2 * i], v[2 * i + 1]);
    *reinterpret_cast<u32x4_t*>(p) = r;
}
__device__ __forceinline__ void st8(float* p, const float (&v)[8]) {
    f32x4_t a, b;
#pragma unroll
    for (int i = 0; i < 4; ++i) { a[i] = v[i]; b[i] = v[4 + i]; }
    *reinterpret_cast<f32x4_t*>(p) = a;
    *reinterpret_cast<f32x4_t*>(p + 4) = b;
}

__device__ __forceinline__ float wave_sum(float v) {
#pragma unroll
    for (int o = 32; o > 0; o >>= 1) v += __shfl_xor(v, o, 64);
    return v;
}
__device__ __forceinline__ float wave_max(float v) {
#pragma unroll
    for (int o = 32; o > 0; o >>= 1) v = fmaxf(v, __shfl_xor(v, o, 64));
    return v;
}

__device__ __host__ __forceinline__ size_t frag_offset(int row, int k, int ksteps) {
    return (((size_t)(row >> 4) * ksteps + (k >> 5)) * 64 + (size_t)(((k & 31) >> 3) * 16 + (row & 15))) * 8 + (k & 7);
}
__device__ __forceinline__ size_t frag_tile(int rt, int ks, int ksteps, int lane) {
    return (((size_t)rt * ksteps + ks) * 64 + lane) * 8;
}

__device__ __forceinline__ float rep_penalize(float x, float rp) { return x < 0.f ? x * rp : x / rp; }
constexpr int HIST_SLOTS = 2048;
__device__ __forceinline__ unsigned int hist_hash(int tok) { return ((unsigned int)tok * 2654435761u) >> 21; }
__device__ __forceinline__ void hist_insert(int* tbl, int tok) {
    unsigned int h = hist_hash(tok);
    for (;;) {
        const int old = atomicCAS(&tbl[h], -1, tok);
        if (old == -1 || old == tok) return;
        h = (h + 1) & (HIST_SLOTS - 1);
    }
}
__device__ __forceinline__ bool hist_contains(const int* tbl, int tok) {
    unsigned int h = hist_hash(tok);
    for (;;) {
        const int v = tbl[h];
        if (v == tok) return true;
        if (v == -1) return false;
        h = (h + 1) & (HIST_SLOTS - 1);
    }
}

#define GITMI_ACT_NONE 0
#define GITMI_ACT_QUICKGELU 1
#define GITMI_ACT_GELU_ERF 2

__device__ __forceinline__ float fast_exp(float x) { return __builtin_amdgcn_exp2f(x * 1.4426950408889634f); }
__device__ __forceinline__ float fast_rcp(float x) { return __builtin_amdgcn_rcpf(x); }

__device__ __forceinline__ float quick_gelu(float x) { return x * fast_rcp(1.0f + fast_exp(-1.702f * x)); }

__device__ __forceinline__ float gelu_erf(float x) {
    const float z = x * 0.70710678118654752440f;
    const float az = fabsf(z);
    const float t = fast_rcp(1.0f + 0.3275911f * az);
    float poly = 1.061405429f;
    poly = poly * t - 1.453152027f;
    poly = poly * t + 1.421413741f;
    poly = poly * t - 0.284496736f;
    poly = poly * t + 0.254829592f;
    poly *= t;
    const float e = 1.0f - poly * fast_exp(-az * az);
    return 0.5f * x * (1.0f + copysignf(e, z));
}

template <int ACT> __device__ __forceinline__ float apply_act_t(float x) {
    if constexpr (ACT == GITMI_ACT_QUICKGELU) return quick_gelu(x);
    else if constexpr (ACT == GITMI_ACT_GELU_ERF) return gelu_erf(x);
    else return x;
}
__device__ __forceinline__ float apply_act(float x, int act) {
    if (act == GITMI_ACT_QUICKGELU) return quick_gelu(x);
    if (act == GITMI_ACT_GELU_ERF) return gelu_erf(x);
    return x;
}
```

generativeimage2text_amd/csrc/kernels_norm.hip:

```cpp
#include "gitmi_common.h"
#include "launchers.h"

namespace gitmi {

struct RowMap {
    int n_in, n_out, off;
};
__device__ __forceinline__ size_t map_row(const RowMap& m, int row) {
    return (size_t)(row / m.n_in) * m.n_out + m.off + row % m.n_in;
}

constexpr int LN_MAXV = 16;

template <typename TOut, typename TS = float>
__global__ __launch_bounds__(256) void layernorm_kernel(const TS* __restrict__ x, int ldx,
                                                        const float* __restrict__ gamma,
                                                        const float* __restrict__ beta, float eps,
                                                        const float* __restrict__ add_after,
                                                        TOut* __restrict__ y_t, int ld_t,
                                                        TS* __restrict__ y_f, int ld_f, int rows, int D,
                                                        RowMap map) {
    const int lane = threadIdx.x & 63;
    const int row = blockIdx.x * 4 + (threadIdx.x >> 6);
    if (row >= rows) return;
// ... 287 lines not shown
__global__ void im2col_ragged_kernel(const float* __restrict__ stage, size_t slot, const int4* __restrict__ meta,
                                     TOut* __restrict__ out, int B, int Nmax, int p, int K, int Kpad) {
    const size_t total = (size_t)B * (Nmax - 1) * Kpad;
    for (size_t i = blockIdx.x * (size_t)blockDim.x + threadIdx.x; i < total; i += (size_t)gridDim.x * blockDim.x) {
        const int k = (int)(i % Kpad);
        const size_t prow = i / Kpad;
        const int t = (int)(prow % (Nmax - 1)), b = (int)(prow / (Nmax - 1));
        const int4 m = meta[b];
        const int gh = m.x / p, gw = m.y / p;
        float val = 0.f;
        if (k < K && t < gh * gw) {
            const int kx = k % p, ky = (k / p) % p, c = k / (p * p);
            const int gx = t % gw, gy = t / gw;
            val = stage[(size_t)b * slot + ((size_t)c * m.x + gy * p + ky) * m.y + gx * p + kx];
        }
        st<TOut>(out + i, val);
    }
}

template <typename TS>
__global__ __launch_bounds__(256) void vit_assemble_ragged_kernel(const float* __restrict__ patch_out,
                                                                  const float* __restrict__ cls,
                                                                  const float* __restrict__ pos, int g,
                                                                  const int4* __restrict__ meta,
                                                                  const float* __restrict__ gamma,
                                                                  const float* __restrict__ beta, float eps,
                                                                  TS* __restrict__ X, int B, int Nmax, int p, int D,
                                                                  float2* __restrict__ part) {
    const int lane = threadIdx.x & 63;
    const int row = blockIdx.x * 4 + (threadIdx.x >> 6);
    if (row >= B * Nmax) return;
    const int b = row / Nmax, n = row % Nmax;
    const int4 m = meta[b];
    if (n >= m.z) {
#pragma unroll
        for (int i = 0; i < LN_MAXV; ++i) {
            const int c = lane + 64 * i;
            if (c < D) st<TS>(X + (size_t)row * D + c, 0.f);
        }
        if (part && lane < 4) part[(size_t)row * 4 + lane] = float2{0.f, 0.f};
        return;
    }
    const int gh = m.x / p, gw = m.y / p;
    const float* src = n == 0 ? cls : patch_out + ((size_t)b * (Nmax - 1) + (n - 1)) * D;
    const bool native = n == 0 || (gh == g && gw == g);
    const float sy = (float)g / (float)gh, sx = (float)g / (float)gw;
    const int oy = native ? 0 : (n - 1) / gw, ox = native ? 0 : (n - 1) % gw;
    const float fy = ((float)oy + 0.5f) * sy - 0.5f, fx = ((float)ox + 0.5f) * sx - 0.5f;
    const float y0f = floorf(fy), x0f = floorf(fx);
    float wy[4], wx[4];
    cubic_taps(fy - y0f, wy);
    cubic_taps(fx - x0f, wx);
    const int y0 = (int)y0f, x0 = (int)x0f;
    float v[LN_MAXV];
    float s = 0.f;
#pragma unroll
    for (int i = 0; i < LN_MAXV; ++i) {
        const int c = lane + 64 * i;
        float pv = 0.f;
        if (c < D) {
            if (native) {
                pv = pos[(size_t)n * D + c];
            } else {
                float acc = 0.f;
#pragma unroll
                for (int a = 0; a < 4; ++a) {
                    int yy = y0 - 1 + a;
                    yy = yy < 0 ? 0 : (yy > g - 1 ? g - 1 : yy);
                    float rw = 0.f;
#pragma unroll
                    for (int bb = 0; bb < 4; ++bb) {
                        int xx = x0 - 1 + bb;
                        xx = xx < 0 ? 0 : (xx > g - 1 ? g - 1 : xx);
                        rw += wx[bb] * pos[((size_t)1 + (size_t)yy * g + xx) * D + c];
                    }
                    acc += wy[a] * rw;
                }
                pv = acc;
            }
        }
        v[i] = c < D ? src[c] + pv : 0.f;
        s += v[i];
    }
    const float mean = wave_sum(s) / (float)D;
    float q = 0.f;
#pragma unroll
    for (int i = 0; i < LN_MAXV; ++i) {
        const int c = lane + 64 * i;
        const float d = c < D ? v[i] - mean : 0.f;
        q += d * d;
    }
    const float rstd = rsqrtf(wave_sum(q) / (float)D + eps);
#pragma unroll
    for (int i = 0; i < LN_MAXV; ++i) {
        const int c = lane + 64 * i;
        if (c < D) st<TS>(X + (size_t)row * D + c, (v[i] - mean) * rstd * gamma[c] + beta[c]);
    }
    if (part) {
        float sx2 = 0.f, sq = 0.f;
#pragma unroll
        for (int i = 0; i < LN_MAXV; ++i) {
            const int c = lane + 64 * i;
            if (c < D) {
                const float o = (float)(TS)((v[i] - mean) * rstd * gamma[c] + beta[c]);
                sx2 += o;
                sq = fmaf(o, o, sq);
            }
        }
        sx2 = wave_sum(sx2);
        sq = wave_sum(sq);
        if (lane < 4) part[(size_t)row * 4 + lane] = lane == 0 ? float2{sx2, sq} : float2{0.f, 0.f};
    }
}

__global__ __launch_bounds__(256) void zero_pad_rows_kernel(char* __restrict__ x, size_t bytes, const int* __restrict__ ntok,
                                                            int B, int Nmax) {
    const int lane = threadIdx.x & 63;
    const int row = blockIdx.x * 4 + (threadIdx.x >> 6);
    if (row >= B * Nmax || row % Nmax < ntok[row / Nmax]) return;
    uint4* r = reinterpret_cast<uint4*>(x + (size_t)row * bytes);
    for (size_t i = lane; i < bytes / 16; i += 64) r[i] = make_uint4(0u, 0u, 0u, 0u);
}

__global__ __launch_bounds__(256) void ragged_report_kernel(const int4* __restrict__ meta, const int* __restrict__ image_of, int Q,
                                                            int nout_per, float* __restrict__ logprob, int* __restrict__ info,
                                                            int* __restrict__ bad) {
    __shared__ int s_n;
    if (threadIdx.x == 0) s_n = 0;
    __syncthreads();
    int n = 0;
    for (int q = threadIdx.x; q < Q; q += blockDim.x) {
        const int im = image_of ? image_of[q] : q;
        if (meta[im].w) {
            ++n;
            if (logprob)
                for (int j = 0; j < nout_per; ++j) logprob[(size_t)q * nout_per + j] = __builtin_nanf("");
            if (bad) bad[q] = 1;
        }
    }
    atomicAdd(&s_n, n);
    __syncthreads();
    if (threadIdx.x == 0 && info && s_n) info[3] += s_n;
}

template <typename TOut>
__global__ __launch_bounds__(256) void embed_ln_kernel(const int* __restrict__ ids, int ld_ids, int pos,
                                                       const float* __restrict__ words,
                                                       const float* __restrict__ positions,
                                                       const float* __restrict__ gamma,
                                                       const float* __restrict__ beta, float eps,
                                                       float* __restrict__ h_f, TOut* __restrict__ h_t, int R,
                                                       int D, int vocab, int frag) {
    __shared__ float s_part[8];
    const int tid = threadIdx.x, lane = tid & 63, wave = tid >> 6;
    const int row = blockIdx.x;
    int tok = ids[(size_t)row * ld_ids + pos];
    tok = tok < 0 ? 0 : (tok >= vocab ? vocab - 1 : tok);
    const int c = tid * 4;
    const bool on = c < D;
    f32x4_t a = {0.f, 0.f, 0.f, 0.f}, g4 = a, b4 = a;
    if (on) {
        const f32x4_t w4 = *reinterpret_cast<const f32x4_t*>(words + (size_t)tok * D + c);
        const f32x4_t p4 = *reinterpret_cast<const f32x4_t*>(positions + (size_t)pos * D + c);
        g4 = *reinterpret_cast<const f32x4_t*>(gamma + c);
        b4 = *reinterpret_cast<const f32x4_t*>(beta + c);
#pragma unroll
        for (int r = 0; r < 4; ++r) a[r] = w4[r] + p4[r];
    }
    float sum = wave_sum(a[0] + a[1] + a[2] + a[3]);
    if (lane == 0) s_part[wave] = sum;
    __syncthreads();
    const float mean = (s_part[0] + s_part[1] + s_part[2] + s_part[3]) / (float)D;
    float q = 0.f;
    if (on) {
#pragma unroll
        for (int r = 0; r < 4; ++r) { const float d = a[r] - mean; q += d * d; }
    }
    q = wave_sum(q);
    if (lane == 0) s_part[4 + wave] = q;
    __syncthreads();
    const float rstd = rsqrtf((s_part[4] + s_part[5] + s_part[6] + s_part[7]) / (float)D + eps);
    if (on) {
        float o[4];
#pragma unroll
        for (int r = 0; r < 4; ++r) o[r] = (a[r] - mean) * rstd * g4[r] + b4[r];
        *reinterpret_cast<f32x4_t*>(h_f + (size_t)row * D + c) = f32x4_t{o[0], o[1], o[2], o[3]};
        if constexpr (sizeof(TOut) == 4) {
            *reinterpret_cast<f32x4_t*>(h_t + (size_t)row * D + c) = f32x4_t{o[0], o[1], o[2], o[3]};
        } else {
            uint2 t;
            t.x = pack2bf(o[0], o[1]);
            t.y = pack2bf(o[2], o[3]);
            const size_t off = frag ? frag_offset(row, c, D >> 5) : (size_t)row * D + c;
            *reinterpret_cast<uint2*>(h_t + off) = t;
        }
    }
}

template <typename TOut>
__global__ __launch_bounds__(256) void context_embed_kernel(const long long* __restrict__ tokens, int ld,
                                                            const int4* __restrict__ seg, int Q, const int* __restrict__ cnt,
                                                            const float* __restrict__ words, const float* __restrict__ positions,
                                                            const float* __restrict__ gamma, const float* __restrict__ beta,
                                                            float eps, TOut* __restrict__ feats, float* __restrict__ feats_f,
                                                            int* __restrict__ ntok, int B, int n_img, int stride, int D, int vocab,
                                                            int max_pos) {
    const int lane = threadIdx.x & 63;
    const int item = blockIdx.x * 4 + (threadIdx.x >> 6);
    const int n_ctx = Q * ld;
    if (item >= n_ctx + B * stride) return;
    constexpr int NCH = 2;
    if (item >= n_ctx) {
        const int r = item - n_ctx, b = r / stride, t = r - b * stride;
        const int nt = n_img + cnt[b];
        if (t == 0 && lane == 0) ntok[b] = nt;
        if (t < nt) return;
        const float z[8] = {0.f, 0.f, 0.f, 0.f, 0.f, 0.f, 0.f, 0.f};
#pragma unroll
        for (int i = 0; i < NCH; ++i) {
            const int c = (lane + 64 * i) * 8;
            if (c < D) {
                st8(feats + (size_t)r * D + c, z);
                if (feats_f) st8(feats_f + (size_t)r * D + c, z);
            }
        }
        return;
    }
    const int q = item / ld, p = item - q * ld;
    const int4 sg = seg[q];
    if (p >= sg.z || sg.x < 0 || sg.x >= B || sg.y < 0 || n_img + sg.y + sg.z > stride) return;
    const long long t = tokens[(size_t)q * ld + p];
    const int tok = t < 0 ? 0 : (t >= vocab ? vocab - 1 : (int)t);
    const int pos = p < max_pos ? p : max_pos - 1;
    const float* wr = words + (size_t)tok * D;
    const float* pr = positions + (size_t)pos * D;
    float v[NCH][8];
    float s = 0.f;
#pragma unroll
    for (int i = 0; i < NCH; ++i) {
        const int c = (lane + 64 * i) * 8;
        if (c < D) {
            float w8[8], p8[8];
            ld8(wr + c, w8);
            ld8(pr + c, p8);
#pragma unroll
            for (int j = 0; j < 8; ++j) { v[i][j] = w8[j] + p8[j]; s += v[i][j]; }
        } else {
#pragma unroll
            for (int j = 0; j < 8; ++j) v[i][j] = 0.f;
        }
    }
    const float mean = wave_sum(s) / (float)D;
    float sq = 0.f;
#pragma unroll
    for (int i = 0; i < NCH; ++i) {
        if ((lane + 64 * i) * 8 < D) {
#pragma unroll
            for (int j = 0; j < 8; ++j) { const float d = v[i][j] - mean; sq += d * d; }
        }
    }
    const float rstd = rsqrtf(wave_sum(sq) / (float)D + eps);
    const size_t orow = (size_t)sg.x * stride + n_img + sg.y + p;
#pragma unroll
    for (int i = 0; i < NCH; ++i) {
        const int c = (lane + 64 * i) * 8;
        if (c < D) {
            float g8[8], b8[8], o[8];
            ld8(gamma + c, g8);
            ld8(beta + c, b8);
#pragma unroll
            for (int j = 0; j < 8; ++j) o[j] = (v[i][j] - mean) * rstd * g8[j] + b8[j];
            st8(feats + orow * D + c, o);
            if (feats_f) st8(feats_f + orow * D + c, o);
        }
    }
}

template <typename TOut>
__global__ void convert_pad_kernel(const float* __restrict__ src, TOut* __restrict__ dst, size_t rows, int K,
                                   int Kpad) {
    const size_t total = rows * (size_t)Kpad;
    for (size_t i = blockIdx.x * (size_t)blockDim.x + threadIdx.x; i < total; i += (size_t)gridDim.x * blockDim.x) {
        const int k = (int)(i % Kpad);
        const size_t r = i / Kpad;
        st<TOut>(dst + i, k < K ? src[r * K + k] : 0.f);
    }
}

template <typename TIn, typename TOut>
__global__ void convert_any_kernel(const TIn* __restrict__ src, TOut* __restrict__ dst, size_t n) {
    for (size_t i = blockIdx.x * (size_t)blockDim.x + threadIdx.x; i < n; i += (size_t)gridDim.x * blockDim.x)
        st<TOut>(dst + i, ld<TIn>(src + i));
}

__global__ void chain_input_kernel(const float* __restrict__ x, bf16_t* __restrict__ xb, float2* __restrict__ stats, int R, int d) {
    const int strips = d >> 4;
    for (int i = blockIdx.x * blockDim.x + threadIdx.x; i < R * strips; i += gridDim.x * blockDim.x) {
        const int r = i / strips, sp = i % strips;
        float sum = 0.f, sq = 0.f;
        for (int c = 0; c < 16; ++c) {
            const float v = x[(size_t)r * d + sp * 16 + c];
            sum += v; sq += v * v;
            xb[frag_offset(r, sp * 16 + c, d >> 5)] = f2bf(v);
        }
        stats[(size_t)sp * R + r] = float2{sum, sq};
    }
}

__global__ void copy_f32_kernel(const float* __restrict__ src, int lds, float* __restrict__ dst, int ldd,
                                int rows, int cols) {
    const size_t total = (size_t)rows * cols;
    for (size_t i = blockIdx.x * (size_t)blockDim.x + threadIdx.x; i < total; i += (size_t)gridDim.x * blockDim.x) {
        const size_t r = i / cols, c = i % cols;
        dst[r * ldd + c] = src[r * lds + c];
    }
}

__global__ void frag_pack_kernel(const bf16_t* __restrict__ src, bf16_t* __restrict__ dst, int rows, int rows_out, int K) {
    const int ksteps = K >> 5;
    const size_t total = (size_t)rows_out * (K >> 3);
    for (size_t i = blockIdx.x * (size_t)blockDim.x + threadIdx.x; i < total; i += (size_t)gridDim.x * blockDim.x) {
        const size_t tile = i >> 6;
        const int lane = (int)(i & 63);
        const int rt = (int)(tile / ksteps), ks = (int)(tile % ksteps);
        const int row = rt * 16 + (lane & 15), k = ks * 32 + (lane >> 4) * 8;
        u32x4_t v = {0u, 0u, 0u, 0u};
        if (row < rows) v = *reinterpret_cast<const u32x4_t*>(src + (size_t)row * K + k);
        *reinterpret_cast<u32x4_t*>(dst + i * 8) = v;
    }
}

__global__ void fill_i32_kernel(int* __restrict__ dst, int value, int n) {
    for (int i = blockIdx.x * blockDim.x + threadIdx.x; i < n; i += gridDim.x * blockDim.x) dst[i] = value;
}

static inline int grid_for(size_t total, int block) {
    size_t g = (total + block - 1) / block;
    return (int)(g > 8192 ? 8192 : (g == 0 ? 1 : g));
}

hipError_t launch_layernorm(const float* x, int ldx, const float* gamma, const float* beta, float eps,
                            const float* add_after, void* y_t, int ld_t, bool t_is_f32, float* y_f, int ld_f,
                            int rows, int D, int map_n_in, int map_n_out, int map_off, hipStream_t s) {
    if (rows <= 0) return hipSuccess;
    if (D > 64 * LN_MAXV || (D & 3) || (ldx & 3) || (ld_t & 3) || (y_f && (ld_f & 3))) return hipErrorInvalidValue;
    RowMap m{map_n_in > 0 ? map_n_in : rows, map_n_in > 0 ? map_n_out : rows, map_off};
    dim3 grid((rows + 3) / 4), block(256);
    if (t_is_f32)
        hipLaunchKernelGGL(layernorm_kernel<float>, grid, block, 0, s, x, ldx, gamma, beta, eps, add_after,
                           (float*)y_t, ld_t, y_f, ld_f, rows, D, m);
    else if (y_t && launch_layernorm_wide<float>(x, ldx, gamma, beta, eps, add_after, (bf16_t*)y_t, ld_t, y_f, ld_f, rows, D, m, s))
        ;
    else
        hipLaunchKernelGGL(layernorm_kernel<bf16_t>, grid, block, 0, s, x, ldx, gamma, beta, eps, add_after,
                           (bf16_t*)y_t, ld_t, y_f, ld_f, rows, D, m);
    return hipGetLastError();
}

hipError_t launch_im2col(const float* img, void* out, bool out_f32, int B, int H, int W, int p, int K, int Kpad,
                         hipStream_t s) {
    const int gh = H / p, gw = W / p;
    const size_t total = (size_t)B * gh * gw * Kpad;
    if (out_f32)
        hipLaunchKernelGGL(im2col_kernel<float>, dim3(grid_for(total, 256)), dim3(256), 0, s, img, (float*)out, B,
                           3, H, W, p, gh, gw, K, Kpad);
    else if (p == 16 && K == 3 * 256 && Kpad == K && (W & 3) == 0 && ((uintptr_t)img & 15) == 0)
        hipLaunchKernelGGL(im2col_p16_kernel, dim3(grid_for(total / 8, 256)), dim3(256), 0, s, img, (bf16_t*)out, B, 3, H, W,
                           gh, gw, Kpad);
    else
        hipLaunchKernelGGL(im2col_kernel<bf16_t>, dim3(grid_for(total, 256)), dim3(256), 0, s, img, (bf16_t*)out,
                           B, 3, H, W, p, gh, gw, K, Kpad);
    return hipGetLastError();
}

hipError_t launch_pos_bicubic(const float* pos, float* out, int g, int gh, int gw, int D, hipStream_t s) {
    const size_t total = ((size_t)gh * gw + 1) * D;
    hipLaunchKernelGGL(pos_bicubic_kernel, dim3(grid_for(total, 256)), dim3(256), 0, s, pos, out, g, gh, gw, D);
    return hipGetLastError();
}

hipError_t launch_ragged_stage(const float* src, float* dst, size_t slot, int4* meta, int* ntok, int B, int p, size_t max_pixels,
                               int Nmax, hipStream_t s) {
    if (B <= 0 || p <= 0 || Nmax < 2) return hipErrorInvalidValue;
    const dim3 grid(64, B);
    if (slot % 4 == 0 && ((uintptr_t)src & 15) == 0 && ((uintptr_t)dst & 15) == 0)
        hipLaunchKernelGGL(ragged_stage_kernel<true>, grid, dim3(256), 0, s, src, dst, slot, meta, ntok, B, p, (long long)max_pixels, Nmax);
    else
        hipLaunchKernelGGL(ragged_stage_kernel<false>, grid, dim3(256), 0, s, src, dst, slot, meta, ntok, B, p, (long long)max_pixels, Nmax);
    return hipGetLastError();
}

hipError_t launch_im2col_ragged(const float* stage, size_t slot, const int4* meta, void* out, bool out_f32, int B, int Nmax,
                                int p, int K, int Kpad, hipStream_t s) {
    const size_t total = (size_t)B * (Nmax - 1) * Kpad;
    if (out_f32)
        hipLaunchKernelGGL(im2col_ragged_kernel<float>, dim3(grid_for(total, 256)), dim3(256), 0, s, stage, slot, meta, (float*)out,
                           B, Nmax, p, K, Kpad);
    else
        hipLaunchKernelGGL(im2col_ragged_kernel<bf16_t>, dim3(grid_for(total, 256)), dim3(256), 0, s, stage, slot, meta,
                           (bf16_t*)out, B, Nmax, p, K, Kpad);
    return hipGetLastError();
}

hipError_t launch_vit_assemble_ragged(const float* patch_out, const float* cls, const float* pos, int g, const int4* meta,
                                      const float* gamma, const float* beta, float eps, void* X, bool x_f16, int B, int Nmax,
                                      int p, int D, float2* part, hipStream_t s) {
    if (D > 64 * LN_MAXV || (part && !x_f16)) return hipErrorInvalidValue;
    if (x_f16)
        hipLaunchKernelGGL(vit_assemble_ragged_kernel<f16_t>, dim3((B * Nmax + 3) / 4), dim3(256), 0, s, patch_out, cls, pos, g,
                           meta, gamma, beta, eps, (f16_t*)X, B, Nmax, p, D, part);
    else
        hipLaunchKernelGGL(vit_assemble_ragged_kernel<float>, dim3((B * Nmax + 3) / 4), dim3(256), 0, s, patch_out, cls, pos, g,
                           meta, gamma, beta, eps, (float*)X, B, Nmax, p, D, (float2*)nullptr);
    return hipGetLastError();
}

hipError_t launch_zero_pad_rows(void* x, bool is_f32, int ld, const int* ntok, int B, int Nmax, hipStream_t s) {
    const size_t bytes = (size_t)ld * (is_f32 ? 4 : 2);
    if (bytes % 16 || ((uintptr_t)x & 15)) return hipErrorInvalidValue;
    hipLaunchKernelGGL(zero_pad_rows_kernel, dim3((B * Nmax + 3) / 4), dim3(256), 0, s, (char*)x, bytes, ntok, B, Nmax);
    return hipGetLastError();
}

hipError_t launch_ragged_report(const int4* meta, const int* image_of, int Q, int nout_per, float* logprob, int* info, int* bad,
                                hipStream_t s) {
    hipLaunchKernelGGL(ragged_report_kernel, dim3(1), dim3(256), 0, s, meta, image_of, Q, nout_per, logprob, info, bad);
    return hipGetLastError();
}

hipError_t launch_vit_assemble_ln(const float* patch_out, const float* cls, const float* pos, const float* gamma,
                                  const float* beta, float eps, void* X, bool x_f16, int B, int N, int D, float2* part,
                                  int nparts, hipStream_t s) {
    if (D > 64 * LN_MAXV || (part && (!x_f16 || nparts < 1 || nparts > 64))) return hipErrorInvalidValue;
    if (x_f16)
        hipLaunchKernelGGL(vit_assemble_ln_kernel<f16_t>, dim3((B * N + 3) / 4), dim3(256), 0, s, patch_out, cls, pos, gamma,
                           beta, eps, (f16_t*)X, B, N, D, part, nparts);
    else
        hipLaunchKernelGGL(vit_assemble_ln_kernel<float>, dim3((B * N + 3) / 4), dim3(256), 0, s, patch_out, cls, pos, gamma,
                           beta, eps, (float*)X, B, N, D, (float2*)nullptr, 0);
    return hipGetLastError();
}

hipError_t launch_layernorm_s16(const void* x, int ldx, const float* gamma, const float* beta, float eps,
                                const float* add_after, void* y_t, int ld_t, bool t_is_f32, void* y_s, int ld_s,
                                int rows, int D, int map_n_in, int map_n_out, int map_off, hipStream_t s) {
    if (rows <= 0) return hipSuccess;
    if (D > 64 * LN_MAXV || (D & 3) || (ldx & 3) || (ld_t & 3) || (y_s && (ld_s & 3))) return hipErrorInvalidValue;
    RowMap m{map_n_in > 0 ? map_n_in : rows, map_n_in > 0 ? map_n_out : rows, map_off};
    dim3 grid((rows + 3) / 4), block(256);
    if (t_is_f32) {
        if (!(y_t && launch_layernorm_wide<f16_t, float>((const f16_t*)x, ldx, gamma, beta, eps, add_after, (float*)y_t, ld_t, (f16_t*)y_s,
                                                         ld_s, rows, D, m, s)))
            hipLaunchKernelGGL((layernorm_kernel<float, f16_t>), grid, block, 0, s, (const f16_t*)x, ldx, gamma, beta, eps,
                               add_after, (float*)y_t, ld_t, (f16_t*)y_s, ld_s, rows, D, m);
    } else if (y_t && launch_layernorm_wide<f16_t>((const f16_t*)x, ldx, gamma, beta, eps, add_after, (bf16_t*)y_t, ld_t, (f16_t*)y_s, ld_s,
                                                 rows, D, m, s))
        ;
    else
        hipLaunchKernelGGL((layernorm_kernel<bf16_t, f16_t>), grid, block, 0, s, (const f16_t*)x, ldx, gamma, beta, eps,
                           add_after, (bf16_t*)y_t, ld_t, (f16_t*)y_s, ld_s, rows, D, m);
    return hipGetLastError();
}

hipError_t launch_embed_ln(const int* ids, int ld_ids, int pos, const float* words, const float* positions,
                           const float* gamma, const float* beta, float eps, float* h_f, void* h_t, bool t_is_f32,
                           int R, int D, int vocab, bool frag, hipStream_t s) {
    if (D > 1024 || (D & 3) || (frag && (t_is_f32 || (D & 31)))) return hipErrorInvalidValue;
    dim3 grid(R), block(256);
    if (t_is_f32)
        hipLaunchKernelGGL(embed_ln_kernel<float>, grid, block, 0, s, ids, ld_ids, pos, words, positions, gamma,
                           beta, eps, h_f, (float*)h_t, R, D, vocab, 0);
    else
        hipLaunchKernelGGL(embed_ln_kernel<bf16_t>, grid, block, 0, s, ids, ld_ids, pos, words, positions, gamma,
                           beta, eps, h_f, (bf16_t*)h_t, R, D, vocab, frag ? 1 : 0);
    return hipGetLastError();
}

hipError_t launch_context_embed(const long long* tokens, int ld, const int4* seg, int Q, const int* cnt, const float* words,
                                const float* positions, const float* gamma, const float* beta, float eps, void* feats, bool t_is_f32,
                                float* feats_f, int* ntok, int B, int n_img, int stride, int D, int vocab, int max_pos, hipStream_t s) {
    if (D > 1024 || (D & 7) || Q < 1 || ld < 1 || B < 1 || n_img < 0 || stride < n_img || vocab < 1 || max_pos < 1 ||
        ((uintptr_t)feats & 15) || ((uintptr_t)feats_f & 15))
        return hipErrorInvalidValue;
    const size_t items = (size_t)Q * ld + (size_t)B * stride;
    if (items > (size_t)1 << 30) return hipErrorInvalidValue;
    const dim3 grid((unsigned)((items + 3) / 4)), block(256);
    if (t_is_f32)
        hipLaunchKernelGGL(context_embed_kernel<float>, grid, block, 0, s, tokens, ld, seg, Q, cnt, words, positions, gamma, beta, eps,
                           (float*)feats, feats_f, ntok, B, n_img, stride, D, vocab, max_pos);
    else
        hipLaunchKernelGGL(context_embed_kernel<bf16_t>, grid, block, 0, s, tokens, ld, seg, Q, cnt, words, positions, gamma, beta, eps,
                           (bf16_t*)feats, feats_f, ntok, B, n_img, stride, D, vocab, max_pos);
    return hipGetLastError();
}

hipError_t launch_frag_pack(const void* src_bf16, void* dst_bf16, int rows, int rows_out, int K, hipStream_t s) {
    if (K % 32 || rows_out % 16 || rows_out < rows) return hipErrorInvalidValue;
    const size_t total = (size_t)rows_out * (K >> 3);
    hipLaunchKernelGGL(frag_pack_kernel, dim3(grid_for(total, 256)), dim3(256), 0, s, (const bf16_t*)src_bf16,
                       (bf16_t*)dst_bf16, rows, rows_out, K);
    return hipGetLastError();
}

hipError_t launch_convert_pad(const float* src, void* dst, bool dst_f32, size_t rows, int K, int Kpad,
                              hipStream_t s) {
    const size_t total = rows * (size_t)Kpad;
    if (total == 0) return hipSuccess;
    if (dst_f32)
        hipLaunchKernelGGL(convert_pad_kernel<float>, dim3(grid_for(total, 256)), dim3(256), 0, s, src, (float*)dst,
                           rows, K, Kpad);
    else
        hipLaunchKernelGGL(convert_pad_kernel<bf16_t>, dim3(grid_for(total, 256)), dim3(256), 0, s, src,
                           (bf16_t*)dst, rows, K, Kpad);
    return hipGetLastError();
}

hipError_t launch_convert(const void* src, bool src_f32, void* dst, bool dst_f32, size_t n, hipStream_t s) {
    if (n == 0) return hipSuccess;
    const dim3 g(grid_for(n, 256)), b(256);
    if (src_f32 && dst_f32) hipLaunchKernelGGL((convert_any_kernel<float, float>), g, b, 0, s, (const float*)src, (float*)dst, n);
    else if (src_f32) hipLaunchKernelGGL((convert_any_kernel<float, bf16_t>), g, b, 0, s, (const float*)src, (bf16_t*)dst, n);
    else if (dst_f32) hipLaunchKernelGGL((convert_any_kernel<bf16_t, float>), g, b, 0, s, (const bf16_t*)src, (float*)dst, n);
    else hipLaunchKernelGGL((convert_any_kernel<bf16_t, bf16_t>), g, b, 0, s, (const bf16_t*)src, (bf16_t*)dst, n);
    return hipGetLastError();
}
// ... 23 lines not shown
```

generativeimage2text_amd/csrc/kernels_search.hip:

```cpp
#include "gitmi_common.h"
#include "launchers.h"
#include "ban_rules.h"

namespace gitmi {

template <int NT>
__device__ __forceinline__ void ban_fill_ngram(const BanRow& br, const int* hist, int t, int* tbl) {
    for (int i = threadIdx.x; i < HIST_SLOTS; i += NT) tbl[i] = -1;
    __syncthreads();
    for (int i = threadIdx.x; i <= ban_ngram_last(br, t); i += NT)
        if (ban_ngram_hit(br, hist, t, i)) hist_insert(tbl, hist[i + br.n - 1]);
    __syncthreads();
}
__device__ __forceinline__ bool ban_test(const BanRow& br, const int* tbl, int c) {
    return ban_static(br, c) || (br.n > 0 && hist_contains(tbl, c));
}

template <int MMAX, int NT, bool BAN = false>
__global__ __launch_bounds__(NT) void row_topm_kernel(const float* __restrict__ logits, int ldl, int V,
                                                       const int* __restrict__ ids, int ld_ids, int cur_len,
                                                       const int* __restrict__ plen, int beams, int suppress_kind,
                                                       float rep_penalty, float* __restrict__ part_val,
                                                       int* __restrict__ part_idx, float2* __restrict__ part_lse, BanArgs ban) {
    constexpr int NW = NT / 64;
// ... 599 lines not shown
                                slot = 0;
                                for (int i = 1; i < nh; ++i)
                                    if (s_hscore[i] < s_hscore[slot] || (s_hscore[i] == s_hscore[slot] && s_hseq[i] < s_hseq[slot])) slot = i;
                                double w = sc;
                                for (int i = 0; i < nh; ++i)
                                    if (i != slot && s_hscore[i] < w) w = s_hscore[i];
                                hyp_worst = w;
                            }
                            s_hscore[slot] = sc; s_hseq[slot] = hyp_cnt;
                            h_score[slot] = sc;
                            h_len[slot] = cur_len;
                            h_seq[slot] = hyp_cnt++;
                            s_add_slot[s_nadd] = slot; s_add_row[s_nadd] = b * k + n_beam[c];
                            ++s_nadd;
                        }
                    } else {
                        sel_score[nb] = n_score[c]; sel_word[nb] = word; sel_src[nb] = b * k + n_beam[c];
                        ++nb;
                    }
                }
                if (hyp_n != s_hyp_n) st.hyp_n[b] = hyp_n;
                if (hyp_cnt != s_hyp_cnt) st.hyp_cnt[b] = hyp_cnt;
                if (hyp_worst != s_hyp_worst) st.hyp_worst[b] = hyp_worst;
            }
            if (nb < k) {
                const int pad_row = st.prefixed ? b * k : 0;
                for (int j = 0; j < k; ++j) { sel_score[j] = 0.f; sel_word[j] = st.eos; sel_src[j] = pad_row; }
            }
        }
        if (b == 0) st.info[2] += 1;
    }
    __syncthreads();

    for (int a = 0; a < s_nadd; ++a) {
        int* ht = st.hyp_tok + ((size_t)b * st.nh + s_add_slot[a]) * T;
        for (int s = tid; s < cur_len; s += 256) ht[s] = ids_at(st, src, s_add_row[a], s);
    }
    for (int idx = tid; idx < k * cur_len; idx += 256) {
        const int j = idx / cur_len, s = idx - j * cur_len;
        const int r = b * k + j, rs = sel_src[j];
        st.ids[dst][(size_t)r * T + s] = st.ids[src][(size_t)rs * T + s];
        st.kv_src[dst][(size_t)r * T + s] = st.kv_src[src][(size_t)rs * T + s];
    }
    if (tid < k) {
        const int r = b * k + tid;
        st.ids[dst][(size_t)r * T + cur_len] = sel_word[tid];
        st.kv_src[dst][(size_t)r * T + cur_len] = r;
        st.score[dst][r] = sel_score[tid];
    }

    if (em.words == nullptr || cur_len + 1 >= T) return;
    const int D = em.D;
    if (k == 1) {
        const int r = b;
        int tok = sel_word[0];
        tok = tok < 0 ? 0 : (tok >= em.vocab ? em.vocab - 1 : tok);
        const int c = tid * 4;
        const bool on = c < D;
        f32x4_t a = {0.f, 0.f, 0.f, 0.f}, g4 = a, b4 = a;
        if (on) {
            const f32x4_t w4 = *reinterpret_cast<const f32x4_t*>(em.words + (size_t)tok * D + c);
            const f32x4_t p4 = *reinterpret_cast<const f32x4_t*>(em.positions + (size_t)cur_len * D + c);
            g4 = *reinterpret_cast<const f32x4_t*>(em.gamma + c);
            b4 = *reinterpret_cast<const f32x4_t*>(em.beta + c);
#pragma unroll
            for (int q = 0; q < 4; ++q) a[q] = w4[q] + p4[q];
        }
        const float sum = wave_sum(a[0] + a[1] + a[2] + a[3]);
        if (lane == 0) s_part[wave] = sum;
        __syncthreads();
        const float mean = (s_part[0] + s_part[1] + s_part[2] + s_part[3]) / (float)D;
        float q2 = 0.f;
        if (on) {
#pragma unroll
            for (int q = 0; q < 4; ++q) { const float d = a[q] - mean; q2 += d * d; }
        }
        q2 = wave_sum(q2);
        if (lane == 0) s_part[4 + wave] = q2;
        __syncthreads();
        const float rstd = rsqrtf((s_part[4] + s_part[5] + s_part[6] + s_part[7]) / (float)D + em.eps);
        if (on) {
            float o[4];
#pragma unroll
            for (int q = 0; q < 4; ++q) o[q] = (a[q] - mean) * rstd * g4[q] + b4[q];
            *reinterpret_cast<f32x4_t*>(em.h_f + (size_t)r * D + c) = f32x4_t{o[0], o[1], o[2], o[3]};
            TOut* ht = reinterpret_cast<TOut*>(em.h_t);
            if constexpr (sizeof(TOut) == 4) {
                *reinterpret_cast<f32x4_t*>(ht + (size_t)r * D + c) = f32x4_t{o[0], o[1], o[2], o[3]};
            } else {
                uint2 t;
                t.x = pack2bf(o[0], o[1]);
                t.y = pack2bf(o[2], o[3]);
                const size_t off = em.frag ? frag_offset(r, c, D >> 5) : (size_t)r * D + c;
                *reinterpret_cast<uint2*>(ht + off) = t;
            }
        }
        return;
    }
    for (int j = wave; j < k; j += 4) {
        const int r = b * k + j;
        int tok = sel_word[j];
        tok = tok < 0 ? 0 : (tok >= em.vocab ? em.vocab - 1 : tok);
        f32x4_t a[4], g4[4], b4[4];
#pragma unroll
        for (int i = 0; i < 4; ++i) {
            const int c = (lane + 64 * i) * 4;
            a[i] = g4[i] = b4[i] = f32x4_t{0.f, 0.f, 0.f, 0.f};
            if (c < D) {
                const f32x4_t w4 = *reinterpret_cast<const f32x4_t*>(em.words + (size_t)tok * D + c);
                const f32x4_t p4 = *reinterpret_cast<const f32x4_t*>(em.positions + (size_t)cur_len * D + c);
                g4[i] = *reinterpret_cast<const f32x4_t*>(em.gamma + c);
                b4[i] = *reinterpret_cast<const f32x4_t*>(em.beta + c);
#pragma unroll
                for (int q = 0; q < 4; ++q) a[i][q] = w4[q] + p4[q];
            }
        }
        float part[4];
#pragma unroll
        for (int i = 0; i < 4; ++i) part[i] = wave_sum(a[i][0] + a[i][1] + a[i][2] + a[i][3]);
        const float mean = (part[0] + part[1] + part[2] + part[3]) / (float)D;
#pragma unroll
        for (int i = 0; i < 4; ++i) {
            float q2 = 0.f;
            if ((lane + 64 * i) * 4 < D) {
#pragma unroll
                for (int q = 0; q < 4; ++q) { const float d = a[i][q] - mean; q2 += d * d; }
            }
            part[i] = wave_sum(q2);
        }
        const float rstd = rsqrtf((part[0] + part[1] + part[2] + part[3]) / (float)D + em.eps);
#pragma unroll
        for (int i = 0; i < 4; ++i) {
            const int c = (lane + 64 * i) * 4;
            if (c < D) {
                float o[4];
#pragma unroll
                for (int q = 0; q < 4; ++q) o[q] = (a[i][q] - mean) * rstd * g4[i][q] + b4[i][q];
                *reinterpret_cast<f32x4_t*>(em.h_f + (size_t)r * D + c) = f32x4_t{o[0], o[1], o[2], o[3]};
                TOut* ht = reinterpret_cast<TOut*>(em.h_t);
                if constexpr (sizeof(TOut) == 4) {
                    *reinterpret_cast<f32x4_t*>(ht + (size_t)r * D + c) = f32x4_t{o[0], o[1], o[2], o[3]};
                } else {
                    uint2 t;
                    t.x = pack2bf(o[0], o[1]);
                    t.y = pack2bf(o[2], o[3]);
                    const size_t off = em.frag ? frag_offset(r, c, D >> 5) : (size_t)r * D + c;
                    *reinterpret_cast<uint2*>(ht + off) = t;
                }
            }
        }
    }
}

__global__ void search_init_kernel(SearchState st) {
    const int R = st.B * st.k;
    for (int i = blockIdx.x * blockDim.x + threadIdx.x; i < R * st.T; i += gridDim.x * blockDim.x) {
        const int r = i / st.T, s = i % st.T;
        const int b = r / st.k;
        st.ids[0][i] = s < st.plen[b] ? (int)st.start[(size_t)b * st.ld_start + s] : st.eos;
        st.kv_src[0][i] = r;
    }
    if (blockIdx.x == 0) {
        for (int r = threadIdx.x; r < R; r += blockDim.x) {
            st.score[0][r] = (st.kind == 1 && r % st.k > 0) ? -1e9f : 0.f;
        }
        for (int b = threadIdx.x; b < st.B; b += blockDim.x) {
            st.done[b] = 0; st.hyp_n[b] = 0; st.hyp_cnt[b] = 0; st.hyp_worst[b] = 1e9; st.stop[b] = 0; st.early[b] = 0;
        }
        if (threadIdx.x < 4) st.info[threadIdx.x] = 0;
        for (int len = threadIdx.x; len <= st.T; len += blockDim.x) st.len_norm[len] = length_norm(len, st.length_penalty);
    }
}

__global__ void search_finish_kernel(SearchState st, int cur, int cur_len, long long* __restrict__ tokens_out,
                                     float* __restrict__ logprob_out, int* __restrict__ info_out,
                                     int* __restrict__ sent_out) {
    __shared__ int s_max_stop, s_all_stop, s_all_early;
    if (threadIdx.x == 0) { s_max_stop = 0; s_all_stop = 1; s_all_early = 1; }
    __syncthreads();
    for (int b = threadIdx.x; b < st.B; b += blockDim.x) {
        const int nout = st.kind == 0 ? 1 : st.nh;
        long long* out = tokens_out + (size_t)b * nout * st.T;
        int L = st.T, early = 0;
        if (st.kind == 0) {
            const int r = b * st.k;
            const int stop = st.stop[b];
            L = stop > 0 ? stop : cur_len;
            early = st.k == 1 ? st.early[b] : 0;
            int non_eos = 0, any_eos = 0;
            for (int s = 0; s < st.T; ++s) {
                const int tok = s < L ? st.ids[cur][(size_t)r * st.T + s] : st.eos;
                out[s] = tok;
                if (s < L) { if (tok != st.eos) ++non_eos; else any_eos = 1; }
            }
            int nv = non_eos + any_eos - st.plen[b];
            nv = nv < 1 ? 1 : nv;
            logprob_out[b] = st.score[cur][r] / (float)nv;
            if (sent_out) sent_out[2 * b + 1] = early;
            if (stop > 0) atomicMax(&s_max_stop, stop); else s_all_stop = 0;
            if (!early) s_all_early = 0;
        } else {
            const int nh = st.nh, have = st.hyp_n[b];
            const double* h_score = st.hyp_score + (size_t)b * nh;
            const int* h_seq = st.hyp_seq + (size_t)b * nh;
            unsigned taken = 0u;
            for (int i = 0; i < nh; ++i) {
                int best = -1;
                for (int j = 0; j < have; ++j) {
                    if ((taken >> j) & 1u) continue;
                    if (best < 0 || h_score[j] > h_score[best] || (h_score[j] == h_score[best] && h_seq[j] < h_seq[best])) best = j;
                }
                const int n = best >= 0 ? st.hyp_len[(size_t)b * nh + best] : 0;
                const int* ht = st.hyp_tok + ((size_t)b * nh + (best >= 0 ? best : 0)) * st.T;
                for (int s = 0; s < st.T; ++s) out[(size_t)i * st.T + s] = s < n ? ht[s] : st.eos;
                logprob_out[(size_t)b * nh + i] = best >= 0 ? (float)h_score[best] : -1e5f;
                if (best >= 0) taken |= 1u << best;
            }
            if (sent_out) sent_out[2 * b + 1] = 0;
        }
        if (sent_out) sent_out[2 * b] = L;
    }
    __syncthreads();
    if (threadIdx.x == 0) {
        info_out[0] = st.kind == 0 ? (s_all_stop ? s_max_stop : cur_len) : st.T;
        info_out[1] = (st.kind == 0 && st.k == 1) ? s_all_early : 0;
        info_out[2] = st.info[2];
        const int nout = st.kind == 0 ? 1 : st.nh;
        int bad = 0;
        for (int i = 0; i < st.B * nout; ++i) bad += !isfinite(logprob_out[i]);
        info_out[3] = bad;
    }
}

__global__ void search_rows_kernel(SearchState st, int cur, int cur_len, long long* __restrict__ out) {
    const int R = st.B * st.k;
    for (int i = blockIdx.x * blockDim.x + threadIdx.x; i < R * cur_len; i += gridDim.x * blockDim.x) {
        const int r = i / cur_len, s = i % cur_len;
        out[i] = st.ids[cur][(size_t)r * st.T + s];
    }
}

__global__ void load_ids_kernel(const long long* __restrict__ tokens, int R, int t, int* __restrict__ ids,
                                int* __restrict__ kv_src, int ld) {
    for (int i = blockIdx.x * blockDim.x + threadIdx.x; i < R * ld; i += gridDim.x * blockDim.x) {
        const int r = i / ld, s = i % ld;
        ids[i] = s < t ? (int)tokens[(size_t)r * t + s] : 0;
        kv_src[i] = r;
    }
}

__global__ void fill_start_kernel(long long* __restrict__ start, int ld, const long long* __restrict__ prefix, int ldp,
                                  int shared, int sos, int B, int P) {
    for (int i = blockIdx.x * blockDim.x + threadIdx.x; i < B * P; i += gridDim.x * blockDim.x) {
        const int b = i / P, s = i % P;
        start[(size_t)b * ld + s] = prefix ? prefix[(shared ? 0 : (size_t)b * ldp) + s] : (long long)sos;
    }
}

hipError_t launch_fill_start(long long* start, int ld, const long long* prefix, int ldp, int shared, int sos, int B, int P,
                             hipStream_t s) {
    hipLaunchKernelGGL(fill_start_kernel, dim3(8), dim3(256), 0, s, start, ld, prefix, ldp, shared, sos, B, P);
    return hipGetLastError();
}

hipError_t launch_load_ids(const long long* tokens, int R, int t, int* ids, int* kv_src, int ld, hipStream_t s) {
    hipLaunchKernelGGL(load_ids_kernel, dim3(64), dim3(256), 0, s, tokens, R, t, ids, kv_src, ld);
    return hipGetLastError();
}

int row_topm_slots(int M) { return M <= 1 ? 1 : M <= 2 ? 2 : M <= 4 ? 4 : M <= 8 ? 8 : 16; }

hipError_t launch_row_topm(const float* logits, int ldl, int V, const int* ids, int ld_ids, int cur_len,
                           const int* plen, int beams, int suppress_kind, float rep_penalty, int M, int R,
                           float* part_val, int* part_idx, float2* part_lse, hipStream_t s, const BanArgs* ban) {
    if (M < 1 || M > 16) return hipErrorInvalidValue;
    const bool banned = ban && ban->set_of && ids;
    if (banned && (!plen || cur_len > HIST_SLOTS / 2)) return hipErrorInvalidValue;
    const BanArgs ba = banned ? *ban : BanArgs{};
    if (rep_penalty != 0.f && rep_penalty != 1.f && ids && cur_len > HIST_SLOTS / 2) return hipErrorInvalidValue;
#define GITMI_TOPM_B(MM, NTT, BB)                                                                                           \
    hipLaunchKernelGGL((row_topm_kernel<MM, NTT, BB>), dim3(R), dim3(NTT), 0, s, logits, ldl, V, ids, ld_ids, cur_len, plen, \
                       beams, suppress_kind, rep_penalty, part_val, part_idx, part_lse, ba)
#define GITMI_TOPM(MM, NTT)                           \
    do {                                              \
        if (banned) GITMI_TOPM_B(MM, NTT, true);      \
        else GITMI_TOPM_B(MM, NTT, false);            \
    } while (0)
    if (M <= 1) GITMI_TOPM(1, 1024);
    else if (M <= 2) GITMI_TOPM(2, 1024);
    else if (M <= 4) GITMI_TOPM(4, 1024);
    else if (M <= 8) GITMI_TOPM(8, 512);
    else GITMI_TOPM(16, 256);
#undef GITMI_TOPM
#undef GITMI_TOPM_B
    return hipGetLastError();
}

hipError_t launch_sample_rows(const float* logits, int ldl, int V, int R, float temperature, int top_k, float top_p,
                              int ndraw, unsigned long long seed, int step, float* part_val, int* part_idx,
                              float2* part_lse, float* filtered_out, const int* ids, int ld_ids, int cur_len,
                              float rep_penalty, int stride, hipStream_t s, const BanArgs* ban, const int* plen, int beams) {
    if (R <= 0) return hipSuccess;
    const bool banned = ban && ban->set_of && ids;
    if (banned && (!plen || beams < 1 || cur_len > HIST_SLOTS / 2)) return hipErrorInvalidValue;
    const BanArgs ba = banned ? *ban : BanArgs{};
    if (stride < ndraw) return hipErrorInvalidValue;
    if (rep_penalty != 0.f && rep_penalty != 1.f && ids && cur_len > HIST_SLOTS / 2) return hipErrorInvalidValue;
    if (V > SMP_NT * SMP_PER || V < 2 || ndraw < 1 || ndraw > SS_CMAX || !(temperature > 0.f)) return hipErrorInvalidValue;
#define GITMI_SAMPLE(BB)                                                                                                        \
    hipLaunchKernelGGL(sample_rows_kernel<BB>, dim3(R), dim3(SMP_NT), 0, s, logits, ldl, V, 1.0f / temperature, top_k, top_p, ndraw, \
                       (unsigned int)(seed & 0xffffffffu), (unsigned int)(seed >> 32), step, part_val, part_idx, part_lse,         \
                       filtered_out, ids, ld_ids, cur_len, rep_penalty, stride, ba, plen, beams)
    if (banned) GITMI_SAMPLE(true);
    else GITMI_SAMPLE(false);
#undef GITMI_SAMPLE
    return hipGetLastError();
}

hipError_t launch_trie_select(const float* logits, int ldl, int V, const int* ids, int ld_ids, int cur_len, const int* plen,
                              int eos, const TrieArgs& tr, int B, float* part_val, int* part_idx, float2* part_lse,
                              hipStream_t s) {
    if (B <= 0) return hipSuccess;
    if (!tr.child_off || !tr.child_tok || !tr.child_node || !tr.cursor || V < 2) return hipErrorInvalidValue;
    hipLaunchKernelGGL(trie_select_kernel, dim3(B), dim3(TRIE_NT), 0, s, logits, ldl, V, ids, ld_ids, cur_len, plen, eos, tr,
                       part_val, part_idx, part_lse);
    return hipGetLastError();
}

hipError_t launch_search_step(const SearchState& st, int src, int cur_len, const StepCands& in, const EmbedArgs& em,
                              bool t_is_f32, hipStream_t s) {
    if (st.k > SS_KMAX || in.slots < 1 || in.slots > SS_CMAX || in.nparts < 1 || in.nparts > 256) return hipErrorInvalidValue;
    if (st.k * st.pn > SS_CMAX) return hipErrorInvalidValue;
    if (em.words && (em.D > 1024 || (em.D & 3))) return hipErrorInvalidValue;
#define GITMI_SSTEP(SL)                                                                                               \
    do {                                                                                                                \
        if (t_is_f32) hipLaunchKernelGGL((search_step_kernel<float, SL>), dim3(st.B), dim3(256), 0, s, st, src, cur_len, in, em); \
        else hipLaunchKernelGGL((search_step_kernel<bf16_t, SL>), dim3(st.B), dim3(256), 0, s, st, src, cur_len, in, em);          \
    } while (0)
    switch (in.slots) {
        case 1: GITMI_SSTEP(1); break;
        case 2: GITMI_SSTEP(2); break;
        case 4: GITMI_SSTEP(4); break;
        case 8: GITMI_SSTEP(8); break;
        case 16: GITMI_SSTEP(16); break;
        default: return hipErrorInvalidValue;
    }
#undef GITMI_SSTEP
    return hipGetLastError();
}
hipError_t launch_search_init(const SearchState& st, hipStream_t s) {
    hipLaunchKernelGGL(search_init_kernel, dim3(16), dim3(256), 0, s, st);
    return hipGetLastError();
}
hipError_t launch_search_finish(const SearchState& st, int cur, int cur_len, long long* tokens_out,
                                float* logprob_out, int* info_out, int* sent_out, hipStream_t s) {
    hipLaunchKernelGGL(search_finish_kernel, dim3(1), dim3(256), 0, s, st, cur, cur_len, tokens_out, logprob_out,
                       info_out, sent_out);
    return hipGetLastError();
}
hipError_t launch_search_rows(const SearchState& st, int cur, int cur_len, long long* out, hipStream_t s) {
    hipLaunchKernelGGL(search_rows_kernel, dim3(64), dim3(256), 0, s, st, cur, cur_len, out);
    return hipGetLastError();
}

}
```

generativeimage2text_amd/csrc/launchers.h:

```cpp
#pragma once
#include <hip/hip_runtime.h>
#include <stddef.h>

namespace gitmi {

struct GemmArgs {
    const void* A; const void* W; const float* bias; const float* res; void* C;
    int M, N, K;
    int lda, ldc, ldr;
    int act;
    int tiles_n, nwg;
    int ng;
    int dbg;
    int out_f16;
    int shared;
    const float2* ln_part; int ln_nparts; const float* ln_colsum; float ln_inv_d, ln_eps;
    float2* part_out;
    const float2* res_part; int res_nparts; const float* res_gamma; const float* res_beta; float res_inv_d, res_eps;
};
bool gemm_uses_p8(const GemmArgs& g, bool in_f32, bool out_f32);
hipError_t launch_gemm(const GemmArgs& g, bool in_f32, bool out_f32, hipStream_t s);
hipError_t launch_gemm_p8(GemmArgs g, bool out_f32, hipStream_t s);
bool gemm_p8_supports(const GemmArgs& g);
int gemm_p8_cost(const GemmArgs& g, int bm);
bool set_gemm_impl(int impl);

struct DGemmArgs {
    const unsigned short* A; const unsigned short* W;
    const float* bias;
    const float* colsum;
    const float2* stats_in;
    int strips_in; float inv_d, eps_in;
    void* C;
    int c_frag;
    const float* res_x;
    const float2* res_stats; int res_strips; const float* res_gamma; const float* res_beta; float res_inv_d, res_eps;
    float* x_out; unsigned short* xb_out; float2* stats_out;
    int M, N, K, lda, ldc, act;
    int dbg;
    int rows_per_wg;
    int strips_per_wg;
    int no_row_walk;
};
hipError_t launch_dgemm(const DGemmArgs& g, hipStream_t s);
struct DLn { const float2* stats; int strips; float inv_d, eps; const float* gamma; const float* beta; };
inline DGemmArgs dgemm_ln(const void* A, const void* W, const float* bias, const float* colsum, const DLn* ln, void* C, int c_frag,
                          int act, int M, int N, int K) {
    DGemmArgs g{};
    g.A = (const unsigned short*)A; g.lda = K; g.W = (const unsigned short*)W; g.bias = bias;
    if (ln) { g.colsum = colsum; g.stats_in = ln->stats; g.strips_in = ln->strips; g.inv_d = ln->inv_d; g.eps_in = ln->eps; }
    g.C = C; g.ldc = N; g.c_frag = c_frag; g.act = act; g.M = M; g.N = N; g.K = K;
    return g;
}
inline DGemmArgs dgemm_to_stream(const void* A, const void* W, const float* bias, const float* res_x, const DLn* res_ln, float* x_out,
                                 void* xb_out, float2* stats_out, int M, int N, int K) {
    DGemmArgs g{};
    g.A = (const unsigned short*)A; g.lda = K; g.W = (const unsigned short*)W; g.bias = bias; g.res_x = res_x;
    if (res_ln) {
        g.res_stats = res_ln->stats; g.res_strips = res_ln->strips; g.res_gamma = res_ln->gamma; g.res_beta = res_ln->beta;
        g.res_inv_d = res_ln->inv_d; g.res_eps = res_ln->eps;
    }
    g.x_out = x_out; g.xb_out = (unsigned short*)xb_out; g.stats_out = stats_out; g.M = M; g.N = N; g.K = K;
    return g;
}

struct BanArgs {
    const unsigned int* words; const int* set_of; const int* min_new; const int* ngram;
    int W, eos;
};

struct VocabArgs {
    const unsigned short* A; int lda; const unsigned short* W; const float* bias; const float* colsum;
    const float2* stats_in; int strips_in; float inv_d, eps_in;
    int M, N, K, cols_per_wg;
    const int* ids; int ld_ids, cur_len; const int* plen; int beams, suppress_kind;
    float rep_penalty;
    float* part_val; int* part_idx; float2* part_lse;
    float* logits_out; int ld_logits;
    int max_wgs;
    int nblk;
    BanArgs ban;
};
hipError_t launch_vocab_topm(const VocabArgs& g, int mtop, hipStream_t s);
int vocab_parts(int V, int cols_per_wg);
int vocab_mtop_slots(int mtop);

hipError_t launch_layernorm(const float* x, int ldx, const float* gamma, const float* beta, float eps,
                            const float* add_after, void* y_t, int ld_t, bool t_is_f32, float* y_f, int ld_f,
                            int rows, int D, int map_n_in, int map_n_out, int map_off, hipStream_t s);
hipError_t launch_im2col(const float* img, void* out, bool out_f32, int B, int H, int W, int p, int K, int Kpad,
                         hipStream_t s);
hipError_t launch_pos_bicubic(const float* pos, float* out, int g, int gh, int gw, int D, hipStream_t s);
hipError_t launch_ragged_stage(const float* src, float* dst, size_t slot, int4* meta, int* ntok, int B, int p, size_t max_pixels,
                               int Nmax, hipStream_t s);
hipError_t launch_im2col_ragged(const float* stage, size_t slot, const int4* meta, void* out, bool out_f32, int B, int Nmax,
                                int p, int K, int Kpad, hipStream_t s);
hipError_t launch_vit_assemble_ragged(const float* patch_out, const float* cls, const float* pos, int g, const int4* meta,
                                      const float* gamma, const float* beta, float eps, void* X, bool x_f16, int B, int Nmax,
                                      int p, int D, float2* part, hipStream_t s);
hipError_t launch_zero_pad_rows(void* x, bool is_f32, int ld, const int* ntok, int B, int Nmax, hipStream_t s);
hipError_t launch_ragged_report(const int4* meta, const int* image_of, int Q, int nout_per, float* logprob, int* info,
                                int* bad, hipStream_t s);
hipError_t launch_vit_assemble_ln(const float* patch_out, const float* cls, const float* pos, const float* gamma,
                                  const float* beta, float eps, void* X, bool x_f16, int B, int N, int D, float2* part,
                                  int nparts, hipStream_t s);
hipError_t launch_layernorm_s16(const void* x, int ldx, const float* gamma, const float* beta, float eps,
                                const float* add_after, void* y_t, int ld_t, bool t_is_f32, void* y_s, int ld_s,
                                int rows, int D, int map_n_in, int map_n_out, int map_off, hipStream_t s);
hipError_t launch_embed_ln(const int* ids, int ld_ids, int pos, const float* words, const float* positions,
                           const float* gamma, const float* beta, float eps, float* h_f, void* h_t, bool t_is_f32,
                           int R, int D, int vocab, bool frag, hipStream_t s);
hipError_t launch_context_embed(const long long* tokens, int ld, const int4* seg, int Q, const int* cnt, const float* words,
                                const float* positions, const float* gamma, const float* beta, float eps, void* feats, bool t_is_f32,
                                float* feats_f, int* ntok, int B, int n_img, int stride, int D, int vocab, int max_pos, hipStream_t s);
hipError_t launch_frag_pack(const void* src_bf16, void* dst_bf16, int rows, int rows_out, int K, hipStream_t s);
hipError_t launch_convert_pad(const float* src, void* dst, bool dst_f32, size_t rows, int K, int Kpad,
                              hipStream_t s);
hipError_t launch_convert(const void* src, bool src_f32, void* dst, bool dst_f32, size_t n, hipStream_t s);
hipError_t launch_chain_input(const float* x, void* xb_frag, float2* stats, int R, int d, hipStream_t s);
hipError_t launch_copy_f32(const float* src, int lds, float* dst, int ldd, int rows, int cols, hipStream_t s);
hipError_t launch_fill_i32(int* dst, int value, int n, hipStream_t s);

constexpr int MEMORY_MAX_LAYERS = 31;
constexpr int MEMORY_HEADER_BYTES = 256, MEMORY_HEADER_WORDS = 16;
constexpr int MEMORY_MAGIC = 0x4d495447;
enum { MEMW_MAGIC = 0, MEMW_VERSION = 1, MEMW_FP0 = 2, MEMW_FP_END = 9, MEMW_N = 9, MEMW_IMG_ROWS = 10, MEMW_CTX_ROWS = 11,
       MEMW_F = 12, MEMW_H = 13, MEMW_W = 14, MEMW_REJECTED = 15 };
struct MemoryEntry {
    int image, slot, n, rsv;
    int hdr[MEMORY_HEADER_WORDS + 4];
};
struct MemoryArgs {
    void* feats;
    void* kv[MEMORY_MAX_LAYERS];
    int layers, stride;
    int feat_row, kv_row, kv_ld, kv_col;
    size_t slot_bytes, feat_plane, kv_plane;
    int* ntok; int4* meta;
};
hipError_t launch_memory_pack(const MemoryArgs& a, void* store, const MemoryEntry* tab, int entries, int max_n, hipStream_t s);
hipError_t launch_memory_unpack(const MemoryArgs& a, const void* store, const MemoryEntry* tab, int entries, hipStream_t s);

struct FeaturePiece { int image, dst0, src0, rows; const float* temb; };
struct FeatureArgs {
    void* feats;
    const void* src;
    const FeaturePiece* pieces; int pieces_n;
    const int* count;
    int stride, D;
    int* ntok; int4* meta;
};
hipError_t launch_feature_install(const FeatureArgs& a, int B, bool src16, bool dst16, hipStream_t s);

struct AttnFullArgs {
    const void* q; const void* k; const void* v; void* out;
    int ldq, ldk, ldv, ldo;
    int N, H;
    float scale;
    const int* ntok;
};
hipError_t launch_attn_full(const AttnFullArgs& a, int B, bool is_f32, int impl, hipStream_t s);

struct AttnDecodeArgs {
    const void* qkv; const void* img_k; const void* img_v; void* txt_k; void* txt_v; void* out;
    const int* kv_src;
    const int* img_of;
    int ld_src;
    int d;
    int N_img, T_max, pos, beams;
    int N_pad;
    int out_frag;
    float scale;
    int dbg;
    int pairs_per_wg;
    int stream_wgs;
    int waves_per_pair;
    int n_pairs;
    const int* ntok;
    const unsigned short* x; const unsigned short* w; const float* bias; const float* colsum;
    const float2* stats_in; int strips_in; float inv_d, eps_in;
    int M;
};
hipError_t launch_kv_repack(const void* qkv, void* kh, void* vh, int B, int N, int H, int d, hipStream_t s);
hipError_t launch_attn_decode(const AttnDecodeArgs& a, int B, int H, hipStream_t s);
hipError_t launch_kv_repack_frag(const void* qkv, void* kf, void* vt, int B, int N, int N_pad, int H, int d, hipStream_t s);
hipError_t launch_attn_decode_mfma(const AttnDecodeArgs& a, int B, int H, hipStream_t s);
int attn_decode_pairs_per_wg(const AttnDecodeArgs& a, int B, int H);
bool attn_decode_qkv_form(const AttnDecodeArgs& a, int B, int H);
inline void attn_decode_set_qkv(AttnDecodeArgs& a, const DGemmArgs& g) {
    a.x = g.A; a.w = g.W; a.bias = g.bias; a.colsum = g.colsum;
    a.stats_in = g.stats_in; a.strips_in = g.strips_in; a.inv_d = g.inv_d; a.eps_in = g.eps_in; a.M = g.M;
}
hipError_t launch_attn_decode_qkv(const AttnDecodeArgs& a, int B, int H, hipStream_t s);

constexpr int SS_NHMAX = 8;
struct SearchState {
    int B, k, pn, T, V, eos, kind;
    int prefixed;
    int sampled;
    double length_penalty;
    double* len_norm;
    const long long* start;
    int ld_start;
    const int* plen;
    int* ids[2];
    int* kv_src[2];
    float* score[2];
    int* done;
    int nh;
    int* hyp_n;
    int* hyp_cnt;
    double* hyp_worst;
    double* hyp_score;
    int* hyp_len;
    int* hyp_seq;
    int* hyp_tok;
    int* stop;
    int* early;
    int* info;
};
struct StepCands {
    const float* part_val; const int* part_idx; const float2* part_lse;
    int nparts, slots;
};
struct EmbedArgs {
    const float* words; const float* positions; const float* gamma; const float* beta; float eps;
    float* h_f; void* h_t; int D, vocab;
    int frag;
};
int row_topm_slots(int M);
hipError_t launch_sample_rows(const float* logits, int ldl, int V, int R, float temperature, int top_k, float top_p,
                              int ndraw, unsigned long long seed, int step, float* part_val, int* part_idx,
                              float2* part_lse, float* filtered_out, const int* ids, int ld_ids, int cur_len,
                              float rep_penalty, int stride, hipStream_t s,
                              const BanArgs* ban = nullptr, const int* plen = nullptr, int beams = 1);
struct TrieArgs {
    const int* child_off; const int* child_tok; const int* child_node;
    int* cursor;
};
hipError_t launch_trie_select(const float* logits, int ldl, int V, const int* ids, int ld_ids, int cur_len, const int* plen,
                              int eos, const TrieArgs& tr, int B, float* part_val, int* part_idx, float2* part_lse,
                              hipStream_t s);
hipError_t launch_row_topm(const float* logits, int ldl, int V, const int* ids, int ld_ids, int cur_len,
                           const int* plen, int beams, int suppress_kind, float rep_penalty, int M, int R,
                           float* part_val, int* part_idx, float2* part_lse, hipStream_t s, const BanArgs* ban = nullptr);
hipError_t launch_search_step(const SearchState& st, int src, int cur_len, const StepCands& in, const EmbedArgs& em,
                              bool t_is_f32, hipStream_t s);
hipError_t launch_search_init(const SearchState& st, hipStream_t s);
hipError_t launch_search_finish(const SearchState& st, int cur, int cur_len, long long* tokens_out,
                                float* logprob_out, int* info_out, int* sent_out, hipStream_t s);
hipError_t launch_search_rows(const SearchState& st, int cur, int cur_len, long long* out, hipStream_t s);
hipError_t launch_fill_start(long long* start, int ld, const long long* prefix, int ldp, int shared, int sos, int B, int P,
                             hipStream_t s);
hipError_t launch_load_ids(const long long* tokens, int R, int t, int* ids, int* kv_src, int ld, hipStream_t s);

struct TreeNodes {
    int* tok;
    int* depth;
    int* parent;
    int* end;
};
hipError_t launch_score_embed_ln(const long long* tokens, int ld, int Q, int Lp, const float* words, const float* positions,
                                 const float* gamma, const float* beta, float eps, float* h_f, void* h_t, bool t_is_f32,
                                 int D, int vocab, int max_pos, hipStream_t s, const TreeNodes* tree = nullptr);
hipError_t launch_score_attn(const void* qkv, const void* img_kv, const int* image_of, void* out, int Q, int H, int d,
                             int N_img, int Lp, float scale, bool is_f32, hipStream_t s, const int* ntok = nullptr,
                             float2* stats = nullptr, const int* node_end = nullptr);
hipError_t launch_score_attn_map(const void* qkv, const void* img_kv, const int* image_of, const int* ntok, const float2* stats,
                                 const int* lens, float* out, size_t out_sq, size_t out_sj, int Tc, int Q, int H, int N_img,
                                 int Lp, float scale, bool is_f32, int* bad, hipStream_t s);
int score_head_tiles(int V);
hipError_t launch_score_head(const void* A, int lda, const void* W, const float* bias, const int* tgt, int M, int V, int K,
                             float4* part, float* zt, hipStream_t s);
hipError_t launch_score_rowstats(const float* logits, int ldl, int V, const int* tgt, int row_off, int rows, float4* part,
                                 float* zt, hipStream_t s);
hipError_t launch_score_targets(const long long* tokens, int ld, int Lp, const int* lens, int V, int M, int* tgt,
                                hipStream_t s);
hipError_t launch_score_combine(const float4* part, int ntiles, const float* zt, const int* tgt, int M, int Lp, int ld, int V,
                                float2* out, int* bad, hipStream_t s);
hipError_t launch_score_info(const int* bad, int Q, int ld, int* info, hipStream_t s, int i1 = 0, int i2 = 0);
hipError_t launch_tree_structure(const long long* packed, int ld, int Q, int Lp, const int* lens, int V, int max_depth,
                                 const TreeNodes& nd, int* bad, hipStream_t s);
hipError_t launch_tree_gather_dot(const void* A, int lda, const void* W, const float* bias, const TreeNodes& nd, int Lp, int M,
                                  int K, float* zt, hipStream_t s);
hipError_t launch_tree_gather_logits(const float* logits, int ldl, int row_off, int rows, const TreeNodes& nd, int Lp, int M,
                                     float* zt, hipStream_t s);
hipError_t launch_tree_combine(const float4* part, int ntiles, const float* zt, const TreeNodes& nd, int M, int Lp, int ld, int V,
                               float2* out, int* bad, hipStream_t s);

hipError_t launch_preprocess(const unsigned char* rgb, int H, int W, int crop, unsigned char* tmp, float* out, hipStream_t s);
hipError_t launch_preprocess_batch(const unsigned char* rgb, const long long* desc, int n, int crop, unsigned char* tmp, float* out,
                                   hipStream_t s);
size_t preprocess_batch_workspace(const long long* desc, int n, int crop);
hipError_t launch_resize_crop_norm(const uint8_t* rgb, int H, int W, int nh, int nw, int top, int left, int ch, int cw,
                                   uint8_t* tmp, float* out, hipStream_t s);

}
```

Before: 11770 captions/s.

## Patch graph node pointers in place of staging copies; fuse decode-open init

Instead of copying input frames into fixed staging buffers and copying results out of staging buffers around each graph replay, the engine records the im2col and search_finish kernel nodes and updates their pointer arguments with hipGraphExecKernelNodeSetParams. It also adds a decode_open kernel that merges fill_start, search_init and the first embed+layernorm into one launch for plain (non-trie, unconstrained) calls. The goal is to cut device-to-device memcpys and a few small launches per call. In exchange it adds per-call graph parameter patching and pointer-attribute queries, and it falls back to recapture when patching fails or frame alignment changes.

```diff
diff --git a/generativeimage2text_amd/csrc/engine.hip b/generativeimage2text_amd/csrc/engine.hip
--- a/generativeimage2text_amd/csrc/engine.hip
+++ b/generativeimage2text_amd/csrc/engine.hip
@@ -198,6 +198,7 @@
     if (const char* env = getenv("GITMI_ATTN_NH")) e->pol.attn_nh = atoi(env);
     if (const char* env = getenv("GITMI_ATTN_STREAM")) e->pol.attn_stream = atoi(env);
     if (const char* env = getenv("GITMI_DECODE_SKIP")) e->pol.decode_skip = atoi(env);
+    if (const char* env = getenv("GITMI_DECODE_OPEN")) e->pol.decode_open = atoi(env) != 0;
     if (const char* env = getenv("GITMI_GEMM_TALL")) e->pol.gemm_tall = atoi(env);
     if (const char* env = getenv("GITMI_DGEMM_ROWS")) e->pol.dgemm_rows = atoi(env);
     if (const char* env = getenv("GITMI_DGEMM_STRIPS")) e->pol.dgemm_strips = atoi(env);
@@ -223,6 +224,54 @@
     RCK(rc);
     HIPCK(ce);
     HIPCK(hipGraphInstantiate(&exec, graph, nullptr, nullptr, 0));
+    return 0;
+}
+hipError_t PatchedNode::set(hipGraphExec_t exec, const void* const* v) {
+    if (std::equal(v, v + n, vals)) return hipSuccess;
+    std::copy(v, v + n, vals);
+    for (int i = 0; i < n; ++i) args[first + i] = (void*)&vals[i];
+    params.kernelParams = args.data();
+    return hipGraphExecKernelNodeSetParams(exec, node, &params);
+}
+int CapturedGraph::bind(const gitmi_engine* e, const Request& rq, int F_in, bool with_results) {
+    frames_in.clear(); results.clear(); opens.clear();
+    size_t n_nodes = 0;
+    HIPCK(hipGraphGetNodes(graph, nullptr, &n_nodes));
+    std::vector<hipGraphNode_t> nodes(n_nodes);
+    HIPCK(hipGraphGetNodes(graph, nodes.data(), &n_nodes));
+    auto find = [&](const void* func, int nargs, int first, int n, const void* const* v, std::vector<PatchedNode>* into) {
+        for (hipGraphNode_t node : nodes) {
+            hipGraphNodeType type;
+            if (hipGraphNodeGetType(node, &type) != hipSuccess || type != hipGraphNodeTypeKernel) continue;
+            PatchedNode p;
+            if (hipGraphKernelNodeGetParams(node, &p.params) != hipSuccess || p.params.func != func || !p.params.kernelParams) continue;
+            bool same = true;
+            for (int i = 0; i < n; ++i) same = same && *(const void* const*)p.params.kernelParams[first + i] == v[i];
+            for (const PatchedNode& q : *into) same = same && q.node != node;
+            if (!same) continue;
+            p.node = node; p.first = first; p.n = n;
+            p.args.assign(p.params.kernelParams, p.params.kernelParams + nargs);
+            std::copy(v, v + n, p.vals);
+            into->push_back(std::move(p));
+            return true;
+        }
+        return false;
+    };
+    for (int f = 0; f < F_in; ++f) {
+        int nargs = 0;
+        const void* img = rq.frames[f];
+        const void* func = im2col_kernel_func(rq.frames[f], e->pol.f32, e->W, e->cfg.patch, e->Kp, e->Kp_pad, &nargs);
+        if (!find(func, nargs, 0, 1, &img, &frames_in))
+            return fail("graph: the captured encode holds no im2col launch that reads frame %d", f);
+    }
+    if (with_results) {
+        const void* out[4] = {rq.tokens, rq.logprob, rq.info, rq.sent};
+        if (!find(search_finish_kernel_func(), SEARCH_FINISH_NARGS, SEARCH_FINISH_OUT_ARG, 4, out, &results))
+            return fail("graph: the captured decode holds no search_finish launch that writes the call's results");
+        const void* prefix = rq.open_prefix;
+        if (rq.plain && !find(decode_open_kernel_func(e->pol.f32), DECODE_OPEN_NARGS, DECODE_OPEN_PREFIX_ARG, 1, &prefix, &opens))
+            return fail("graph: the captured decode of a plain call holds no decode_open launch");
+    }
     return 0;
 }
 static void destroy_graph(gitmi_engine* e) {
@@ -682,6 +731,10 @@
     e->sample = *sp;
     st.start = e->start_dev; st.ld_start = c.max_text_len; st.plen = e->plen_dev;
     e->ss_cur = 0; e->ss_len = minP;
+    if (rq.plain) {
+        HIPCK(launch_decode_open(st, e->start_dev, e->plen_dev, rq.open_prefix, c.sos, minP, embed_args(e, true), e->pol.f32, s));
+        return 0;
+    }
     HIPCK(launch_search_init(st, s));
     if (e->trie_search) HIPCK(launch_fill_i32(e->trie_cursor, 0, B, s));
     return 0;
@@ -903,7 +956,7 @@
     const int suppress = sp->kind != GITMI_SEARCH_GENERATOR ? 1 : 0;
     {
         SpanGuard phase(e, s, TAG_DECODE, 0);
-        RCK(embed_position(e, st.ids[0], T, 0, R, s));
+        if (!rq.plain) RCK(embed_position(e, st.ids[0], T, 0, R, s));
         e->ss_len = 1;
         StepCands cands{e->part_val, e->part_idx, e->part_lse, 1, 1};
         while (e->ss_len < T) {
@@ -970,6 +1023,21 @@
     return 0;
 }
 
+static bool on_device(const gitmi_engine* e, const void* p) {
+    if (p == e->out_sent) return true;
+    hipPointerAttribute_t at{};
+    if (hipPointerGetAttributes(&at, p) == hipSuccess) return at.type == hipMemoryTypeDevice;
+    (void)hipGetLastError();
+    return false;
+}
+
+static hipError_t patch_decode(CapturedGraph& g, const Request& rq, const void* const* results) {
+    const hipError_t err = g.results[0].set(g.exec, results);
+    if (err != hipSuccess || !rq.plain) return err;
+    const void* prefix = rq.open_prefix;
+    return g.opens[0].set(g.exec, &prefix);
+}
+
 static int generate_graphed(gitmi_engine* e, const Request& rq, hipStream_t s) {
     const gitmi_config& c = e->cfg;
     const bool resident = rq.frames == nullptr;
@@ -978,34 +1046,51 @@
         HIPCK(hipEventRecord(e->fence_in, s));
         HIPCK(hipStreamWaitEvent(x, e->fence_in, 0));
     }
-    const size_t frame_bytes = (size_t)rq.B * 3 * e->H * e->W * sizeof(float);
     const int F_eff = resident ? e->cur_F : c.num_frames > 0 ? std::min(rq.F, c.num_frames) : rq.F;
-    if (!e->ragged && !resident)
-    for (int f = 0; f < F_eff; ++f)
-        HIPCK(hipMemcpyAsync(e->frame_stage[f], rq.frames[f], frame_bytes, hipMemcpyDeviceToDevice, x));
+    const int F_in = e->ragged || resident ? 0 : F_eff;
+    const bool staged = e->ragged || !(on_device(e, rq.tokens) && on_device(e, rq.logprob) && on_device(e, rq.info) && on_device(e, rq.sent));
     Request own = rq;
-    if (!resident) { own.frames = e->frame_stage.data(); own.F = F_eff; }
-    own.tokens = e->out_tokens; own.logprob = e->out_lp; own.info = e->out_info; own.sent = e->out_sent;
+    if (e->ragged && !resident) own.frames = e->frame_stage.data();
+    if (!resident) own.F = F_eff;
+    if (staged) { own.tokens = e->out_tokens; own.logprob = e->out_lp; own.info = e->out_info; own.sent = e->out_sent; }
+    const void* const results[4] = {own.tokens, own.logprob, own.info, own.sent};
     const GraphKey key = graph_key_of(e, rq, F_eff);
     const CapturedGraph *enc = nullptr, *dec = nullptr;
     if (resident) {
         RCK(images_ready(e, rq, x));
-        if (!e->follow_slot.valid || !(key == e->follow_slot.key)) {
+        bool capture = !e->follow_slot.valid || !(key == e->follow_slot.key);
+        if (!capture && patch_decode(e->graph_follow, own, results) != hipSuccess) { (void)hipGetLastError(); capture = true; }
+        if (capture) {
             e->follow_slot.valid = false;
             RCK(e->graph_follow.capture(x, [&] { return generate_decode(e, own, x, false); }));
+            RCK(e->graph_follow.bind(e, own, 0, true));
             e->follow_slot = {key, true};
         }
         dec = &e->graph_follow;
     } else {
         const bool split = e->profile_mode == 2 || e->enc_after != nullptr || !e->enc_watchers.empty();
-        if (!e->full_slot.valid || !(key == e->full_slot.key) || split != e->graph_is_split) {
+        bool capture = !e->full_slot.valid || !(key == e->full_slot.key) || split != e->graph_is_split;
+        if (!capture) {
+            CapturedGraph& fin = split ? e->graph_decode : e->graph_full;
+            for (int f = 0; f < F_in && !capture; ++f) {
+                PatchedNode& n = e->graph_full.frames_in[f];
+                const void* img = own.frames[f];
+                capture = (((uintptr_t)img ^ (uintptr_t)n.vals[0]) & 15) != 0 || n.set(e->graph_full.exec, &img) != hipSuccess;
+            }
+            capture = capture || patch_decode(fin, own, results) != hipSuccess;
+            if (capture) (void)hipGetLastError();
+        }
+        if (capture) {
             e->full_slot.valid = false;
             e->graph_decode.reset();
             if (!split) {
                 RCK(e->graph_full.capture(x, [&] { return generate_body(e, own, x, false); }));
+                RCK(e->graph_full.bind(e, own, F_in, true));
             } else {
                 RCK(e->graph_full.capture(x, [&] { return generate_encode(e, own, x); }));
+                RCK(e->graph_full.bind(e, own, F_in, false));
                 RCK(e->graph_decode.capture(x, [&] { return generate_decode(e, own, x, false); }));
+                RCK(e->graph_decode.bind(e, own, 0, true));
             }
             e->full_slot = {key, true}; e->graph_is_split = split;
         } else {
@@ -1016,11 +1101,13 @@
         if (split) dec = &e->graph_decode;
     }
     RCK(replay(e, rq, x, enc, dec));
-    const size_t nout = (size_t)rq.Q * (size_t)keep_best(*rq.sp);
-    HIPCK(hipMemcpyAsync(rq.tokens, e->out_tokens, nout * rq.sp->max_steps * sizeof(long long), hipMemcpyDefault, x));
-    HIPCK(hipMemcpyAsync(rq.logprob, e->out_lp, nout * sizeof(float), hipMemcpyDefault, x));
-    HIPCK(hipMemcpyAsync(rq.info, e->out_info, 4 * sizeof(int), hipMemcpyDefault, x));
-    if (rq.sent != e->out_sent) HIPCK(hipMemcpyAsync(rq.sent, e->out_sent, (size_t)rq.Q * 2 * sizeof(int), hipMemcpyDefault, x));
+    if (staged) {
+        const size_t nout = (size_t)rq.Q * (size_t)keep_best(*rq.sp);
+        HIPCK(hipMemcpyAsync(rq.tokens, e->out_tokens, nout * rq.sp->max_steps * sizeof(long long), hipMemcpyDefault, x));
+        HIPCK(hipMemcpyAsync(rq.logprob, e->out_lp, nout * sizeof(float), hipMemcpyDefault, x));
+        HIPCK(hipMemcpyAsync(rq.info, e->out_info, 4 * sizeof(int), hipMemcpyDefault, x));
+        if (rq.sent != e->out_sent) HIPCK(hipMemcpyAsync(rq.sent, e->out_sent, (size_t)rq.Q * 2 * sizeof(int), hipMemcpyDefault, x));
+    }
     if (x != s) {
         HIPCK(hipEventRecord(e->fence_out, x));
         HIPCK(hipStreamWaitEvent(s, e->fence_out, 0));
@@ -1063,8 +1150,11 @@
     RCK(constrain_check(e, "generate", sp, B, &constrained));
     hipStream_t s = (hipStream_t)stream;
     if (frames) RCK(ragged_prepare(e, frames, F, B, s));
-    RCK(fill_uniform_sentences(e, B, (const long long*)prefix, P, s));
-    const Request rq{frames, F, B, B, P, P, false, sp, (long long*)tokens_out, logprob_out, info_out, e->out_sent};
+    const bool plain = e->pol.decode_open && sp->kind != GITMI_SEARCH_TRIE && !constrained;
+    if (plain) e->img_identity = true;
+    else RCK(fill_uniform_sentences(e, B, (const long long*)prefix, P, s));
+    const Request rq{frames, F, B, B, P, P, false, sp, (long long*)tokens_out, logprob_out, info_out, e->out_sent,
+                     (const long long*)prefix, plain};
     return generate_run(e, rq, s, constrained);
 }
 
diff --git a/generativeimage2text_amd/csrc/engine_state.h b/generativeimage2text_amd/csrc/engine_state.h
--- a/generativeimage2text_amd/csrc/engine_state.h
+++ b/generativeimage2text_amd/csrc/engine_state.h
@@ -55,15 +55,31 @@
 };
 struct GraphSlot { GraphKey key{}; bool valid = false; };
 
+struct Request;
+
+struct PatchedNode {
+    hipGraphNode_t node = nullptr;
+    hipKernelNodeParams params{};
+    std::vector<void*> args;
+    int first = 0, n = 0;
+    const void* vals[4] = {nullptr, nullptr, nullptr, nullptr};
+    hipError_t set(hipGraphExec_t exec, const void* const* v);
+};
+
 struct CapturedGraph {
     hipGraph_t graph = nullptr;
     hipGraphExec_t exec = nullptr;
+    std::vector<PatchedNode> frames_in;
+    std::vector<PatchedNode> results;
+    std::vector<PatchedNode> opens;
     void reset() {
         if (exec) hipGraphExecDestroy(exec);
         if (graph) hipGraphDestroy(graph);
         exec = nullptr, graph = nullptr;
+        frames_in.clear(); results.clear(); opens.clear();
     }
     int capture(hipStream_t s, const std::function<int()>& fn);
+    int bind(const gitmi_engine* e, const Request& rq, int F_in, bool with_results);
     hipError_t launch(hipStream_t s) const { return hipGraphLaunch(exec, s); }
 };
 
@@ -74,6 +90,8 @@
     const gitmi_search* sp;
     long long* tokens; float* logprob; int32_t* info;
     int32_t* sent;
+    const long long* open_prefix = nullptr;
+    bool plain = false;
 };
 
 struct ModelWeights {
@@ -111,6 +129,7 @@
     int vocab_wgs = -1;
     int gemm_tall = 1;
     int dgemm_rows = 0;
+    bool decode_open = true;
     int decode_skip = 0;
 };
 
diff --git a/generativeimage2text_amd/csrc/engine_weights.hip b/generativeimage2text_amd/csrc/engine_weights.hip
--- a/generativeimage2text_amd/csrc/engine_weights.hip
+++ b/generativeimage2text_amd/csrc/engine_weights.hip
@@ -209,9 +209,8 @@
     HIPCK(hipStreamCreateWithFlags(&e->own_stream, hipStreamNonBlocking));
     HIPCK(hipEventCreateWithFlags(&e->fence_in, hipEventDisableTiming));
     HIPCK(hipEventCreateWithFlags(&e->fence_out, hipEventDisableTiming));
-    e->frame_stage.resize(c.max_frames);
-    for (int f = 0; f < c.max_frames; ++f)
-        RCK(dev_alloc_t(e, &e->frame_stage[f], (size_t)c.max_batch * 3 * e->max_pixels));
+    e->frame_stage.resize(1);
+    RCK(dev_alloc_t(e, &e->frame_stage[0], (size_t)c.max_batch * 3 * e->max_pixels));
     RCK(dev_alloc_t(e, &e->rg_meta, (size_t)c.max_batch));
     RCK(dev_alloc_t(e, &e->rg_ntok, (size_t)c.max_batch));
     return 0;
diff --git a/generativeimage2text_amd/csrc/gitmi_common.h b/generativeimage2text_amd/csrc/gitmi_common.h
--- a/generativeimage2text_amd/csrc/gitmi_common.h
+++ b/generativeimage2text_amd/csrc/gitmi_common.h
@@ -128,6 +128,55 @@
 __device__ __forceinline__ size_t frag_tile(int rt, int ks, int ksteps, int lane) {
     return (((size_t)rt * ksteps + ks) * 64 + lane) * 8;
 }
+
+template <typename TOut>
+__device__ __forceinline__ void embed_ln_row(int row, int tok, int pos, const float* __restrict__ words,
+                                             const float* __restrict__ positions, const float* __restrict__ gamma,
+                                             const float* __restrict__ beta, float eps, float* __restrict__ h_f,
+                                             TOut* __restrict__ h_t, int D, int vocab, int frag, float* s_part) {
+    const int tid = threadIdx.x, lane = tid & 63, wave = tid >> 6;
+    tok = tok < 0 ? 0 : (tok >= vocab ? vocab - 1 : tok);
+    const int c = tid * 4;
+    const bool on = c < D;
+    f32x4_t a = {0.f, 0.f, 0.f, 0.f}, g4 = a, b4 = a;
+    if (on) {
+        const f32x4_t w4 = *reinterpret_cast<const f32x4_t*>(words + (size_t)tok * D + c);
+        const f32x4_t p4 = *reinterpret_cast<const f32x4_t*>(positions + (size_t)pos * D + c);
+        g4 = *reinterpret_cast<const f32x4_t*>(gamma + c);
+        b4 = *reinterpret_cast<const f32x4_t*>(beta + c);
+#pragma unroll
+        for (int r = 0; r < 4; ++r) a[r] = w4[r] + p4[r];
+    }
+    float sum = wave_sum(a[0] + a[1] + a[2] + a[3]);
+    if (lane == 0) s_part[wave] = sum;
+    __syncthreads();
+    const float mean = (s_part[0] + s_part[1] + s_part[2] + s_part[3]) / (float)D;
+    float q = 0.f;
+    if (on) {
+#pragma unroll
+        for (int r = 0; r < 4; ++r) { const float d = a[r] - mean; q += d * d; }
+    }
+    q = wave_sum(q);
+    if (lane == 0) s_part[4 + wave] = q;
+    __syncthreads();
+    const float rstd = rsqrtf((s_part[4] + s_part[5] + s_part[6] + s_part[7]) / (float)D + eps);
+    if (on) {
+        float o[4];
+#pragma unroll
+        for (int r = 0; r < 4; ++r) o[r] = (a[r] - mean) * rstd * g4[r] + b4[r];
+        *reinterpret_cast<f32x4_t*>(h_f + (size_t)row * D + c) = f32x4_t{o[0], o[1], o[2], o[3]};
+        if constexpr (sizeof(TOut) == 4) {
+            *reinterpret_cast<f32x4_t*>(h_t + (size_t)row * D + c) = f32x4_t{o[0], o[1], o[2], o[3]};
+        } else {
+            uint2 t;
+            t.x = pack2bf(o[0], o[1]);
+            t.y = pack2bf(o[2], o[3]);
+            const size_t off = frag ? frag_offset(row, c, D >> 5) : (size_t)row * D + c;
+            *reinterpret_cast<uint2*>(h_t + off) = t;
+        }
+    }
+}
+
 
 __device__ __forceinline__ float rep_penalize(float x, float rp) { return x < 0.f ? x * rp : x / rp; }
 constexpr int HIST_SLOTS = 2048;
diff --git a/generativeimage2text_amd/csrc/kernels_norm.hip b/generativeimage2text_amd/csrc/kernels_norm.hip
--- a/generativeimage2text_amd/csrc/kernels_norm.hip
+++ b/generativeimage2text_amd/csrc/kernels_norm.hip
@@ -463,49 +463,8 @@
                                                        float* __restrict__ h_f, TOut* __restrict__ h_t, int R,
                                                        int D, int vocab, int frag) {
     __shared__ float s_part[8];
-    const int tid = threadIdx.x, lane = tid & 63, wave = tid >> 6;
     const int row = blockIdx.x;
-    int tok = ids[(size_t)row * ld_ids + pos];
-    tok = tok < 0 ? 0 : (tok >= vocab ? vocab - 1 : tok);
-    const int c = tid * 4;
-    const bool on = c < D;
-    f32x4_t a = {0.f, 0.f, 0.f, 0.f}, g4 = a, b4 = a;
-    if (on) {
-        const f32x4_t w4 = *reinterpret_cast<const f32x4_t*>(words + (size_t)tok * D + c);
-        const f32x4_t p4 = *reinterpret_cast<const f32x4_t*>(positions + (size_t)pos * D + c);
-        g4 = *reinterpret_cast<const f32x4_t*>(gamma + c);
-        b4 = *reinterpret_cast<const f32x4_t*>(beta + c);
-#pragma unroll
-        for (int r = 0; r < 4; ++r) a[r] = w4[r] + p4[r];
-    }
-    float sum = wave_sum(a[0] + a[1] + a[2] + a[3]);
-    if (lane == 0) s_part[wave] = sum;
-    __syncthreads();
-    const float mean = (s_part[0] + s_part[1] + s_part[2] + s_part[3]) / (float)D;
-    float q = 0.f;
-    if (on) {
-#pragma unroll
-        for (int r = 0; r < 4; ++r) { const float d = a[r] - mean; q += d * d; }
-    }
-    q = wave_sum(q);
-    if (lane == 0) s_part[4 + wave] = q;
-    __syncthreads();
-    const float rstd = rsqrtf((s_part[4] + s_part[5] + s_part[6] + s_part[7]) / (float)D + eps);
-    if (on) {
-        float o[4];
-#pragma unroll
-        for (int r = 0; r < 4; ++r) o[r] = (a[r] - mean) * rstd * g4[r] + b4[r];
-        *reinterpret_cast<f32x4_t*>(h_f + (size_t)row * D + c) = f32x4_t{o[0], o[1], o[2], o[3]};
-        if constexpr (sizeof(TOut) == 4) {
-            *reinterpret_cast<f32x4_t*>(h_t + (size_t)row * D + c) = f32x4_t{o[0], o[1], o[2], o[3]};
-        } else {
-            uint2 t;
-            t.x = pack2bf(o[0], o[1]);
-            t.y = pack2bf(o[2], o[3]);
-            const size_t off = frag ? frag_offset(row, c, D >> 5) : (size_t)row * D + c;
-            *reinterpret_cast<uint2*>(h_t + off) = t;
-        }
-    }
+    embed_ln_row<TOut>(row, ids[(size_t)row * ld_ids + pos], pos, words, positions, gamma, beta, eps, h_f, h_t, D, vocab, frag, s_part);
 }
 
 template <typename TOut>
@@ -668,6 +627,9 @@
     return hipGetLastError();
 }
 
+static bool im2col_is_p16(const float* img, int W, int p, int K, int Kpad) {
+    return p == 16 && K == 3 * 256 && Kpad == K && (W & 3) == 0 && ((uintptr_t)img & 15) == 0;
+}
 hipError_t launch_im2col(const float* img, void* out, bool out_f32, int B, int H, int W, int p, int K, int Kpad,
                          hipStream_t s) {
     const int gh = H / p, gw = W / p;
@@ -675,13 +637,19 @@
     if (out_f32)
         hipLaunchKernelGGL(im2col_kernel<float>, dim3(grid_for(total, 256)), dim3(256), 0, s, img, (float*)out, B,
                            3, H, W, p, gh, gw, K, Kpad);
-    else if (p == 16 && K == 3 * 256 && Kpad == K && (W & 3) == 0 && ((uintptr_t)img & 15) == 0)
+    else if (im2col_is_p16(img, W, p, K, Kpad))
         hipLaunchKernelGGL(im2col_p16_kernel, dim3(grid_for(total / 8, 256)), dim3(256), 0, s, img, (bf16_t*)out, B, 3, H, W,
                            gh, gw, Kpad);
     else
         hipLaunchKernelGGL(im2col_kernel<bf16_t>, dim3(grid_for(total, 256)), dim3(256), 0, s, img, (bf16_t*)out,
                            B, 3, H, W, p, gh, gw, K, Kpad);
     return hipGetLastError();
+}
+const void* im2col_kernel_func(const float* img, bool out_f32, int W, int p, int K, int Kpad, int* nargs) {
+    const bool p16 = !out_f32 && im2col_is_p16(img, W, p, K, Kpad);
+    *nargs = p16 ? 9 : 11;
+    if (out_f32) return (const void*)im2col_kernel<float>;
+    return p16 ? (const void*)im2col_p16_kernel : (const void*)im2col_kernel<bf16_t>;
 }
 
 hipError_t launch_pos_bicubic(const float* pos, float* out, int g, int gh, int gw, int D, hipStream_t s) {
diff --git a/generativeimage2text_amd/csrc/kernels_search.hip b/generativeimage2text_amd/csrc/kernels_search.hip
--- a/generativeimage2text_amd/csrc/kernels_search.hip
+++ b/generativeimage2text_amd/csrc/kernels_search.hip
@@ -775,24 +775,53 @@
     }
 }
 
+__device__ __forceinline__ long long start_token(const long long* __restrict__ prefix, int ldp, int shared, int sos, int b, int s) {
+    return prefix ? prefix[(shared ? 0 : (size_t)b * ldp) + s] : (long long)sos;
+}
+__device__ __forceinline__ void search_init_id(const SearchState& st, int i, int r, int tok) {
+    st.ids[0][i] = tok;
+    st.kv_src[0][i] = r;
+}
+__device__ __forceinline__ void search_init_row(const SearchState& st, int r) {
+    st.score[0][r] = (st.kind == 1 && r % st.k > 0) ? -1e9f : 0.f;
+}
+__device__ __forceinline__ void search_init_sentence(const SearchState& st, int b) {
+    st.done[b] = 0; st.hyp_n[b] = 0; st.hyp_cnt[b] = 0; st.hyp_worst[b] = 1e9; st.stop[b] = 0; st.early[b] = 0;
+}
+__device__ __forceinline__ void search_init_once(const SearchState& st) {
+    if (threadIdx.x < 4) st.info[threadIdx.x] = 0;
+    for (int len = threadIdx.x; len <= st.T; len += blockDim.x) st.len_norm[len] = length_norm(len, st.length_penalty);
+}
+
 __global__ void search_init_kernel(SearchState st) {
     const int R = st.B * st.k;
     for (int i = blockIdx.x * blockDim.x + threadIdx.x; i < R * st.T; i += gridDim.x * blockDim.x) {
         const int r = i / st.T, s = i % st.T;
         const int b = r / st.k;
-        st.ids[0][i] = s < st.plen[b] ? (int)st.start[(size_t)b * st.ld_start + s] : st.eos;
-        st.kv_src[0][i] = r;
+        search_init_id(st, i, r, s < st.plen[b] ? (int)st.start[(size_t)b * st.ld_start + s] : st.eos);
     }
     if (blockIdx.x == 0) {
-        for (int r = threadIdx.x; r < R; r += blockDim.x) {
-            st.score[0][r] = (st.kind == 1 && r % st.k > 0) ? -1e9f : 0.f;
-        }
-        for (int b = threadIdx.x; b < st.B; b += blockDim.x) {
-            st.done[b] = 0; st.hyp_n[b] = 0; st.hyp_cnt[b] = 0; st.hyp_worst[b] = 1e9; st.stop[b] = 0; st.early[b] = 0;
-        }
-        if (threadIdx.x < 4) st.info[threadIdx.x] = 0;
-        for (int len = threadIdx.x; len <= st.T; len += blockDim.x) st.len_norm[len] = length_norm(len, st.length_penalty);
-    }
+        for (int r = threadIdx.x; r < R; r += blockDim.x) search_init_row(st, r);
+        for (int b = threadIdx.x; b < st.B; b += blockDim.x) search_init_sentence(st, b);
+        search_init_once(st);
+    }
+}
+
+template <typename TOut>
+__global__ __launch_bounds__(256) void decode_open_kernel(SearchState st, long long* __restrict__ start, int* __restrict__ plen,
+                                                          const long long* __restrict__ prefix, int sos, int P, EmbedArgs em) {
+    __shared__ float s_part[8];
+    const int r = blockIdx.x, b = r / st.k;
+    if (r % st.k == 0) {
+        for (int s = threadIdx.x; s < P; s += blockDim.x) start[(size_t)b * st.ld_start + s] = start_token(prefix, 0, 1, sos, b, s);
+        if (threadIdx.x == 0) { plen[b] = P; search_init_sentence(st, b); }
+    }
+    for (int s = threadIdx.x; s < st.T; s += blockDim.x)
+        search_init_id(st, r * st.T + s, r, s < P ? (int)start_token(prefix, 0, 1, sos, b, s) : st.eos);
+    if (threadIdx.x == 0) search_init_row(st, r);
+    if (r == 0) search_init_once(st);
+    embed_ln_row<TOut>(r, (int)start_token(prefix, 0, 1, sos, b, 0), 0, em.words, em.positions, em.gamma, em.beta, em.eps, em.h_f,
+                       reinterpret_cast<TOut*>(em.h_t), em.D, em.vocab, em.frag, s_part);
 }
 
 __global__ void search_finish_kernel(SearchState st, int cur, int cur_len, long long* __restrict__ tokens_out,
@@ -876,7 +905,7 @@
                                   int shared, int sos, int B, int P) {
     for (int i = blockIdx.x * blockDim.x + threadIdx.x; i < B * P; i += gridDim.x * blockDim.x) {
         const int b = i / P, s = i % P;
-        start[(size_t)b * ld + s] = prefix ? prefix[(shared ? 0 : (size_t)b * ldp) + s] : (long long)sos;
+        start[(size_t)b * ld + s] = start_token(prefix, ldp, shared, sos, b, s);
     }
 }
 
@@ -975,12 +1004,25 @@
     hipLaunchKernelGGL(search_init_kernel, dim3(16), dim3(256), 0, s, st);
     return hipGetLastError();
 }
+hipError_t launch_decode_open(const SearchState& st, long long* start, int* plen, const long long* prefix, int sos, int P,
+                              const EmbedArgs& em, bool t_is_f32, hipStream_t s) {
+    if (start != st.start || plen != st.plen || P < 1 || P > st.T || P > st.ld_start || st.B < 1 || st.k < 1) return hipErrorInvalidValue;
+    if (!em.words || em.D > 1024 || (em.D & 3) || (em.frag && (t_is_f32 || (em.D & 31)))) return hipErrorInvalidValue;
+    const dim3 grid(st.B * st.k), block(256);
+    if (t_is_f32) hipLaunchKernelGGL(decode_open_kernel<float>, grid, block, 0, s, st, start, plen, prefix, sos, P, em);
+    else hipLaunchKernelGGL(decode_open_kernel<bf16_t>, grid, block, 0, s, st, start, plen, prefix, sos, P, em);
+    return hipGetLastError();
+}
+const void* decode_open_kernel_func(bool t_is_f32) {
+    return t_is_f32 ? (const void*)decode_open_kernel<float> : (const void*)decode_open_kernel<bf16_t>;
+}
 hipError_t launch_search_finish(const SearchState& st, int cur, int cur_len, long long* tokens_out,
                                 float* logprob_out, int* info_out, int* sent_out, hipStream_t s) {
     hipLaunchKernelGGL(search_finish_kernel, dim3(1), dim3(256), 0, s, st, cur, cur_len, tokens_out, logprob_out,
                        info_out, sent_out);
     return hipGetLastError();
 }
+const void* search_finish_kernel_func() { return (const void*)search_finish_kernel; }
 hipError_t launch_search_rows(const SearchState& st, int cur, int cur_len, long long* out, hipStream_t s) {
     hipLaunchKernelGGL(search_rows_kernel, dim3(64), dim3(256), 0, s, st, cur, cur_len, out);
     return hipGetLastError();
diff --git a/generativeimage2text_amd/csrc/launchers.h b/generativeimage2text_amd/csrc/launchers.h
--- a/generativeimage2text_amd/csrc/launchers.h
+++ b/generativeimage2text_amd/csrc/launchers.h
@@ -90,6 +90,7 @@
                             int rows, int D, int map_n_in, int map_n_out, int map_off, hipStream_t s);
 hipError_t launch_im2col(const float* img, void* out, bool out_f32, int B, int H, int W, int p, int K, int Kpad,
                          hipStream_t s);
+const void* im2col_kernel_func(const float* img, bool out_f32, int W, int p, int K, int Kpad, int* nargs);
 hipError_t launch_pos_bicubic(const float* pos, float* out, int g, int gh, int gw, int D, hipStream_t s);
 hipError_t launch_ragged_stage(const float* src, float* dst, size_t slot, int4* meta, int* ntok, int B, int p, size_t max_pixels,
                                int Nmax, hipStream_t s);
@@ -247,8 +248,14 @@
 hipError_t launch_search_step(const SearchState& st, int src, int cur_len, const StepCands& in, const EmbedArgs& em,
                               bool t_is_f32, hipStream_t s);
 hipError_t launch_search_init(const SearchState& st, hipStream_t s);
+hipError_t launch_decode_open(const SearchState& st, long long* start, int* plen, const long long* prefix, int sos, int P,
+                              const EmbedArgs& em, bool t_is_f32, hipStream_t s);
+constexpr int DECODE_OPEN_PREFIX_ARG = 3, DECODE_OPEN_NARGS = 7;
+const void* decode_open_kernel_func(bool t_is_f32);
 hipError_t launch_search_finish(const SearchState& st, int cur, int cur_len, long long* tokens_out,
                                 float* logprob_out, int* info_out, int* sent_out, hipStream_t s);
+constexpr int SEARCH_FINISH_OUT_ARG = 3, SEARCH_FINISH_NARGS = 7;
+const void* search_finish_kernel_func();
 hipError_t launch_search_rows(const SearchState& st, int cur, int cur_len, long long* out, hipStream_t s);
 hipError_t launch_fill_start(long long* start, int ld, const long long* prefix, int ldp, int shared, int sos, int B, int P,
                              hipStream_t s);
```

Result: no change. 11750 captions/s (-0.1%).
